# calclavia/tal-asrd

Measured on AMD Instinct MI355X. Metric: audio frames/sec (16 kHz, 10 ms hop) end-to-end log-mel -> TDS encoder -> diarization head, higher is better.
Workload: dtype f32 (dense layers: 3 x f16 MFMA hi/lo split, f32 accumulate); 1 GPU; 1 x 3600 s 16 kHz clip per GPU, each a whole-episode B=1 call (BASELINE.json configs[2]; SDModel path of tal/baseline/reconcile.py:76-85: log-mel -> TDS 80-800-1120-1440 -> 128-d feat + argmax over 6008 speakers); weights=synthetic deterministic, audio_resident_in_hbm=True

## Files before the change

include/tal_asrd.h:

```cpp
#ifndef TAL_ASRD_H
#define TAL_ASRD_H

#include <stddef.h>
#include <stdint.h>

#ifdef __cplusplus
extern "C" {
#endif

#define TAL_OK 0
#define TAL_EINVAL (-1)
#define TAL_ENOMEM (-2)
#define TAL_EHIP (-3)

#define TAL_MAX_STAGES 4
#define TAL_MAX_DEPTH 8

int tal_version(void);
const char* tal_last_error(void);

int tal_set_option(const char* name, int value);
int tal_get_option(const char* name, int* value);
const char* tal_option_name(int index);

int64_t tal_logmel_num_frames(int64_t L);
size_t tal_logmel_plan_bytes(void);
int tal_logmel_plan_init(const float* window, const float* fb, void* plan, void* stream);
size_t tal_logmel_workspace_bytes(int B, int64_t L);
int tal_logmel_fwd(const void* plan, const float* audio, int B, int64_t L, float eps,
                   int subtract_mean, float* out, float* mean_out, double* sum_out,
                   void* workspace, size_t workspace_bytes, void* stream);
int tal_logmel_f16_fwd(const void* plan, const void* audio_f16, int B, int64_t L, float eps,
                       int subtract_mean, float* out, float* mean_out, double* sum_out,
                       void* workspace, size_t workspace_bytes, void* stream);
int tal_subtract_scalar(float* x, int64_t n, const float* mean, void* stream);

int64_t tal_logmel_frames(int64_t L, int hop);
size_t tal_logmel_general_plan_bytes(int n_fft, int n_mels);
int tal_logmel_general_plan_init(const float* window, int n_fft, int hop, const float* fb, int n_mels, void* plan, void* stream);
size_t tal_logmel_general_workspace_bytes(int n_fft, int hop, int B, int64_t L);
int tal_logmel_general_fwd(const void* plan, int n_fft, int hop, int n_mels, const void* audio, int audio_is_f16, int B, int64_t L,
                           float eps, int subtract_mean, float* out, float* mean_out, double* sum_out, void* workspace,
                           size_t workspace_bytes, void* stream);

#define TAL_RESAMPLE_F32 0
#define TAL_RESAMPLE_F16 1
#define TAL_RESAMPLE_I16 2
int64_t tal_resample_num_samples(int64_t n_in, int orig, int new_rate);
size_t tal_resample_plan_bytes(int orig, int new_rate, int width);
int tal_resample_plan_build_host(int orig, int new_rate, int width, float* w, int32_t* first, int* taps);
int tal_resample_plan_init(void* plan, int orig, int new_rate, int width, void* stream);
int tal_resample_fwd(const void* plan, int orig, int new_rate, int width, const void* x, int x_dtype, int B, int64_t L_in,
                     int64_t x_pitch, const int64_t* lengths, float* y, int64_t y_pitch, void* stream);

int tal_linear_fwd(const float* x, const float* w, const float* b, const float* res, float alpha,
                   int mode, int64_t M, int N, int K, float* y, void* stream);
size_t tal_linear_workspace_bytes(int64_t M, int N, int K);
int tal_linear_ws_fwd(const float* x, const float* w, const float* b, const float* res, float alpha,
                      int mode, int64_t M, int N, int K, float* y, void* workspace,
                      size_t workspace_bytes, void* stream);

int tal_split_f16x3_fwd(const float* x, void* out, int64_t rows, int K, void* stream);
int tal_linear_f16x3_fwd(const void* x_split, const void* w_split, const float* b, const float* res, float alpha,
                         int mode, int64_t M, int N, int K, void* y, int out_split, void* workspace,
                         size_t workspace_bytes, void* stream);
int tal_linear_f16x3_guarded_fwd(const void* x_split, const void* w_split, const float* b, const void* res, int res_split,
                                 float alpha, int mode, int64_t M, int N, int K, void* y, int out_split,
                                 int* range_flag, void* workspace, size_t workspace_bytes, void* stream);

#define TAL_GCONV_MAX_K 63
int tal_pack_gconv_weight(const float* w_ref, float* w_packed, int c_out, int c_in_per_group,
                          int ksize, int groups, void* stream);
int tal_gconv_s2_fwd(const float* x, const float* w_packed, const float* bias, int B, int64_t T_in,
                     int C_in, int C_out, int groups, float* y, void* stream);
int tal_gconv_res_fwd(const float* x, const float* w_packed, const float* bias, float alpha, int B,
                      int64_t T, int C, int groups, float* y, void* stream);
int tal_gconv_s2_k_fwd(const float* x, const float* w_packed, const float* bias, int B, int64_t T_in, int C_in, int C_out,
                       int groups, int ksize, float* y, void* stream);
int tal_gconv_res_k_fwd(const float* x, const float* w_packed, const float* bias, float alpha, int B, int64_t T, int C,
                        int groups, int ksize, float* y, void* stream);

size_t tal_gconv_f16x3_weight_bytes(int C_in, int C_out, int groups, int stride);
int tal_pack_gconv_f16x3_weight(const float* w_ref, void* w_frag, int C_in, int C_out, int groups, int stride,
                                void* stream);
int tal_gconv_res_f16x3_fwd(const float* x, const void* w_frag, const float* bias, float alpha, int B,
                            int64_t T, int C, int groups, float* y, void* y_split, void* stream);
int tal_gconv_s2_f16x3_fwd(const float* x, const void* w_frag, const float* bias, int B, int64_t T_in,
                           int C_in, int C_out, int groups, float* y, void* stream);
int tal_gconv_res_split_fwd(const void* x_split, const void* w_frag, const float* bias, float alpha, int B,
                            int64_t T, int C, int groups, void* y_split, void* stream);
int tal_gconv_s2_split_fwd(const void* x, int x_is_split, const void* w_frag, const float* bias, int B,
                           int64_t T_in, int C_in, int C_out, int groups, void* y_split, void* stream);

typedef struct tal_tds_block_w {
    const float* conv_w;
    const float* conv_b;
    const float* fc0_w;
    const float* fc0_b;
    const float* fc3_w;
    const float* fc3_b;
    float resweight;
    int32_t _pad;
    const void* fc0_w_split;
    const void* fc3_w_split;
    const void* conv_w_frag;
} tal_tds_block_w;

typedef struct tal_tds_desc {
    int32_t n_stages;
    int32_t groups;
    int32_t channels[TAL_MAX_STAGES + 1];
    int32_t depths[TAL_MAX_STAGES];
    const float* down_w[TAL_MAX_STAGES];
    const float* down_b[TAL_MAX_STAGES];
    tal_tds_block_w blocks[TAL_MAX_STAGES][TAL_MAX_DEPTH];
    const void* down_w_frag[TAL_MAX_STAGES];
    int32_t flags;
    int32_t ksize;
} tal_tds_desc;
#define TAL_TDS_EXACT_F32 1
#define TAL_TDS_OUT_SPLIT 2

int64_t tal_tds_out_len(const tal_tds_desc* d, int64_t T);
size_t tal_tds_workspace_bytes(const tal_tds_desc* d, int B, int64_t T);
size_t tal_tds_status_offset(const tal_tds_desc* d, int B, int64_t T);
int tal_tds_out_split(const tal_tds_desc* d, int B, int64_t T);
int tal_tds_fwd(const tal_tds_desc* d, const float* x, int B, int64_t T, float* y,
                void* workspace, size_t workspace_bytes, void* stream);
int tal_tds_premean_ok(const tal_tds_desc* d, const float* x);
int tal_tds_premean_fwd(const tal_tds_desc* d, const float* x, const float* x_mean, int B, int64_t T, float* y,
                        void* workspace, size_t workspace_bytes, void* stream);

int tal_tds_halo(const tal_tds_desc* d, int64_t* left, int64_t* right, int64_t* stride);
size_t tal_tds_tiled_workspace_bytes(const tal_tds_desc* d, int64_t T, int64_t out_tile);
size_t tal_tds_tiled_status_offset(const tal_tds_desc* d, int64_t T, int64_t out_tile);
int tal_tds_tiled_fwd(const tal_tds_desc* d, const float* x, int64_t T, float* y, int64_t out_tile,
                      void* workspace, size_t workspace_bytes, void* stream);

size_t tal_sd_head_workspace_bytes(int64_t M, int S);
int tal_sd_head_fwd(const float* x, int64_t M, int C, const float* w_embed, const float* b_embed, int E,
                    const float* w_logit, const float* b_logit, int S, float* feat, float* logits,
                    int32_t* ids, void* workspace, size_t workspace_bytes, void* stream);
int tal_sd_head_split_fwd(const void* x_split, int64_t M, int C, const void* w_embed_split, const float* b_embed, int E,
                          const float* w_logit, const float* b_logit, int S, float* feat, float* logits,
                          int32_t* ids, void* workspace, size_t workspace_bytes, void* stream);
int tal_argmax_rows(const float* x, int64_t M, int N, int32_t* ids, void* stream);

#define TAL_TOPK_MAX 16
size_t tal_spk_topk_workspace_bytes(int64_t M, int S, int E, int k);
int tal_spk_topk_fwd(const float* feat, int64_t M, int E, const float* w_logit, const float* b_logit, int S, int k,
                     int32_t* ids, float* logp, float* lse, void* workspace, size_t workspace_bytes, void* stream);
int tal_topk_lse_rows(const float* x, int64_t M, int N, int k, int32_t* ids, float* logp, float* lse, void* stream);

size_t tal_xent_rows_workspace_bytes(int64_t M, int N, int E);
int tal_xent_rows_fwd(const float* feat, int64_t M, int64_t ldf, int E, const float* w, const float* bias, int N,
                      const int64_t* target, float* nll, float* lse, int32_t* top1, void* workspace, size_t workspace_bytes,
                      void* stream);
int tal_xent_lse_rows(const float* x, int64_t M, int N, const int64_t* target, float* nll, float* lse, int32_t* top1, void* stream);

size_t tal_soft_embed_workspace_bytes(int64_t M, int N, int E, int D);
int tal_soft_embed_fwd(const float* feat, int64_t M, int64_t ldf, int E, const float* w, const float* bias, int N,
                       const float* values, int D, float* out, float* lse, void* workspace, size_t workspace_bytes, void* stream);
size_t tal_soft_embed_rows_workspace_bytes(int64_t M, int N, int D);
int tal_soft_embed_rows(const float* x, int64_t M, int N, const float* values, int D, float* out, float* lse, void* workspace,
                        size_t workspace_bytes, void* stream);

int tal_embed_tokens_fwd(const int64_t* tokens, int B, int U, const float* emb, int V, int E0,
                         const float* proj, int D, const float* pe, int max_len, float* out,
                         void* stream);
int tal_add_positional_fwd(const float* x, int B, int U, int D, const float* pe, int max_len,
                           float* out, void* stream);

typedef struct tal_decoder_layer_w {
    const float* sa_in_w;
    const float* sa_in_b;
    const float* sa_out_w;
    const float* sa_out_b;
    const float* ca_in_w;
    const float* ca_in_b;
    const float* ca_out_w;
    const float* ca_out_b;
    const float* lin1_w;
    const float* lin1_b;
    const float* lin2_w;
    const float* lin2_b;
    float resweight;
    float resweight_src;
    const float* fold_sa_w;
    const float* fold_sa_b;
    const float* fold_ca_w;
    const float* fold_ca_b;
} tal_decoder_layer_w;

int64_t tal_pad4(int64_t n);
int tal_cross_kv_fwd(const tal_decoder_layer_w* w, const float* mem, int B, int S, int E,
                     float* k, float* vt, void* stream);
size_t tal_decoder_layer_workspace_bytes(int B, int U, int S, int E, int H, int FF);
int tal_decoder_layer_fwd(const tal_decoder_layer_w* w, const float* tgt, int B, int U,
                          const float* mem, int S, int E, int H, int FF, const float* tgt_mask,
                          const uint8_t* mem_kpm, const float* k_cache, const float* vt_cache,
                          float* out, float* xattn_avg, void* workspace, size_t workspace_bytes,
                          void* stream);
int tal_decoder_stack_fwd(const tal_decoder_layer_w* layers, int n_layers, const float* tgt, int B,
                          int U, const float* mem, int S, int E, int H, int FF, const float* tgt_mask,
                          const uint8_t* mem_kpm, const float* const* k_cache,
                          const float* const* vt_cache, float* out, float* xattn_avg, void* workspace,
                          size_t workspace_bytes, void* stream);
int tal_lm_head_fwd(const float* h, int64_t M, int64_t ldh, int D, const float* proj_t, int E0,
                    const float* emb, int V, float* logits, void* workspace, size_t workspace_bytes,
                    void* stream);
size_t tal_lm_xent_workspace_bytes(int64_t M, int D, int E0, int V);
int tal_lm_xent_fwd(const float* h, int64_t M, int64_t ldh, int D, const float* proj_t, int E0, const float* emb, int V,
                    const int64_t* target, float* nll, float* lse, int32_t* top1, void* workspace, size_t workspace_bytes,
                    void* stream);
size_t tal_lm_soft_embed_workspace_bytes(int64_t M, int D, int E0, int V, int col_begin);
int tal_lm_soft_embed_fwd(const float* h, int64_t M, int64_t ldh, int D, const float* proj_t, int E0, const float* emb, int V,
                          int col_begin, float* out, float* lse, void* workspace, size_t workspace_bytes, void* stream);
int tal_transpose_fwd(const float* x, int R, int Cc, float* y, void* stream);
int tal_log_softmax_rows(const float* x, int64_t M, int N, float* out, void* stream);
int tal_greedy_pick_fwd(const float* logits, int V, const float* attn_rows, int n_layers,
                        int64_t layer_stride, int S, float* out, int64_t* token_out, void* stream);
typedef struct tal_greedy_ctx {
    const tal_decoder_layer_w* layers;
    int32_t n_layers, E, H, FF, V, E0, S, max_len;
    const float* emb;
    const float* proj;
    const float* proj_t;
    const float* pe;
    const float* const* k_cache;
    const float* const* vt_cache;
    const uint8_t* mem_kpm;
    int64_t* tokens;
    void* workspace;
    size_t workspace_bytes;
    float* picked_dev;
    float* picked_host;
    uint32_t* tickets;
    float* picked_host_dev;
    uint32_t seq;
    uint32_t needs_reset;
    int64_t k_pitch;
    const float* const* kv_all;
    const uint8_t* kpm_all;
    int64_t enc_frames, kv_pitch;
    const float* pick_bias;
    uint32_t no_fold;
    uint32_t _pad2;
} tal_greedy_ctx;
size_t tal_greedy_step_workspace_bytes(int U_max, int S, int E, int H, int FF, int V, int E0, int n_layers);
int tal_greedy_step_fwd(tal_greedy_ctx* c, int64_t history_start, int64_t n_gen, int sync, void* stream);
int tal_greedy_step_poll(tal_greedy_ctx* c, int wait_ms);
int tal_greedy_group_ok(const tal_greedy_ctx* c, int64_t history_start, int64_t n_gen);
int tal_window_vt_fwd(const float* const* kv_all, int n_layers, int64_t frame0, int S, int E, int64_t kv_pitch,
                      float* const* vt, void* stream);
int tal_greedy_set_window(tal_greedy_ctx* c, int64_t frame0, void* stream);
int tal_greedy_step_multi_fwd(tal_greedy_ctx* const* ctxs, const int64_t* history_start, const int64_t* n_gen, int G,
                              void* stream);
typedef struct tal_unaligned_state {
    int64_t* gen;
    int64_t gen_cap, n;
    int64_t history_start;
    int64_t chunk_start;
    int64_t encoder_len;
    int64_t eos, it, max_iters;
    int64_t* rec_chunk_start;
    float* rec_attn;
    int32_t* rec_len;
    int64_t rec_cap, n_rec;
    int32_t rec_stride;
    int32_t chunk_size, max_positions, stall_patience, rep_n;
    int32_t skip_frames;
    int32_t shift_frames;
    float del_prct;
    double thresh_prct;
    double highest_progress;
    int32_t num_no_improve, window_time;
    int32_t flags;
    int32_t gen_pinned;
} tal_unaligned_state;
#define TAL_UNALIGNED_WINDOW_MOVED 1
#define TAL_UNALIGNED_PREFIX_REWRITTEN 2
#define TAL_UNALIGNED_DONE 4
#define TAL_UNALIGNED_GROW 8
#define TAL_UNALIGNED_ALONE 16
int tal_unaligned_consume(tal_unaligned_state* st, int64_t token, const float* attn, int S);
int tal_unaligned_group_run(tal_unaligned_state* const* st, tal_greedy_ctx* const* ctxs, const int64_t* dev_cap, int G,
                            int max_steps, void* stream);
int64_t tal_ngram_repeat_count(const int64_t* row, int64_t len, int n);
int tal_beam_topk(const float* logprobs, const float* row_score, const uint8_t* row_done, int B,
                  int cur_beam, int V, int k, float* out_val, int64_t* out_idx, void* stream);
typedef struct tal_beam_ctx {
    int32_t B, beam, L0, length, V, num_speakers;
    void* workspace;
    size_t workspace_bytes;
    uint32_t* done_host;
    uint32_t* done_host_dev;
    uint32_t* ctl;
    float* scores;
    uint8_t* done;
    int32_t* rec_step;
    float* rec_score;
    int64_t* rec_tokens;
    int64_t* tokens[2];
    float* sel_val;
    int64_t* sel_idx;
    float* part_val;
    int64_t* part_idx;
    float* spk_hist;
    int32_t* parent;
    size_t state_bytes;
    uint32_t seq;
    uint32_t _pad;
} tal_beam_ctx;
size_t tal_beam_workspace_bytes(int B, int beam, int L0, int length, int V, int num_speakers);
int tal_beam_init_fwd(tal_beam_ctx* c, const int64_t* generated, void* stream);
int tal_beam_select_fwd(tal_beam_ctx* c, int step, int cur_beam, const float* logits, const float* bias, int nl, void* stream);
int tal_beam_advance_fwd(tal_beam_ctx* c, int step, int cur_beam, int64_t terminate_token, const float* spk_logits, void* stream);
int tal_beam_gather_spk_fwd(const tal_beam_ctx* c, const int32_t* pairs, int n, float* out, void* stream);

int tal_attn_pool_fwd(const float* attn, const int64_t* chunk_start, const float* feat, int64_t T,
                      int E, int N, int S, int half_mode, float* out, void* stream);
int tal_attn_vote_fwd(const float* attn, const int64_t* chunk_start, const int32_t* ids, int64_t T,
                      int N, int S, int32_t* out_id, float* out_weight, void* stream);
int tal_attn_vote_groups_fwd(const float* attn, const int64_t* chunk_start, const int32_t* ids, int64_t T,
                             int S, const int64_t* group_offsets, int G, int num_ids, int half_mode,
                             int32_t* out_id, double* out_weight, void* stream);
int tal_majority_vote_fwd(const int32_t* ids, int64_t T, const int64_t* ranges, int G, int num_ids,
                          int32_t* out_id, double* out_count, void* stream);

size_t tal_gru_cell_workspace_bytes(int B, int H);
int tal_gru_cell_fwd(const float* x, const float* h, int B, int In, int H, const float* w_ih,
                     const float* w_hh, const float* b_ih, const float* b_hh, float* h_out,
                     void* workspace, size_t workspace_bytes, void* stream);

#define TAL_EDIT_TILE_ROWS 64
#ifndef TAL_EDIT_TILE_COLS
#define TAL_EDIT_TILE_COLS 128
#endif
#define TAL_EDIT_TAG_EQUAL 0
#define TAL_EDIT_TAG_REPLACE 1
#define TAL_EDIT_TAG_INSERT 2
#define TAL_EDIT_TAG_DELETE 3
#define TAL_EDIT_TAG_NONE 255
void tal_edit_align_tile(int* rows, int* cols);
size_t tal_edit_align_workspace_bytes(int P, const int64_t* a_off, const int64_t* b_off, int want_path);
int tal_edit_align_plan(int P, const int64_t* a_off, const int64_t* b_off, int want_path, int64_t* desc,
                        size_t* workspace_bytes, int64_t* path_bytes, int* launches);
int tal_edit_align_fwd(const int64_t* desc_host, const int64_t* desc_dev, int P, const int32_t* a, const int32_t* b,
                       const int32_t* a_lab, const int32_t* b_lab, int Ka, int Kb, int64_t* stats, uint8_t* path,
                       int64_t* counts, void* workspace, size_t workspace_bytes, void* stream);

int tal_prof_enable(int on);
int tal_prof_reset(void);
int tal_prof_collect(int cls, double* total_ms, int64_t* launches, double* total_work);

#ifdef __cplusplus
}
#endif
#endif
```

tal_asrd_amd/_native.py:

```python
import ctypes as C
import os

_HERE = os.path.dirname(os.path.abspath(__file__))
LIB_PATH = os.environ.get("TAL_ASRD_LIB", os.path.join(_HERE, "libtal_asrd_hip.so"))

TAL_MAX_STAGES = 4
TAL_MAX_DEPTH = 8
TAL_TDS_EXACT_F32 = 1
TAL_TDS_OUT_SPLIT = 2
TAL_GCONV_MAX_K = 63
TAL_GROUP_MAX = 16
TAL_TOPK_MAX = 16

c_float_p = C.c_void_p


class TdsBlockW(C.Structure):
    _fields_ = [("conv_w", C.c_void_p), ("conv_b", C.c_void_p), ("fc0_w", C.c_void_p), ("fc0_b", C.c_void_p),
                ("fc3_w", C.c_void_p), ("fc3_b", C.c_void_p), ("resweight", C.c_float), ("_pad", C.c_int32),
                ("fc0_w_split", C.c_void_p), ("fc3_w_split", C.c_void_p), ("conv_w_frag", C.c_void_p)]


class TdsDesc(C.Structure):
    _fields_ = [("n_stages", C.c_int32), ("groups", C.c_int32),
                ("channels", C.c_int32 * (TAL_MAX_STAGES + 1)), ("depths", C.c_int32 * TAL_MAX_STAGES),
                ("down_w", C.c_void_p * TAL_MAX_STAGES), ("down_b", C.c_void_p * TAL_MAX_STAGES),
                ("blocks", (TdsBlockW * TAL_MAX_DEPTH) * TAL_MAX_STAGES),
                ("down_w_frag", C.c_void_p * TAL_MAX_STAGES), ("flags", C.c_int32), ("ksize", C.c_int32)]


class DecoderLayerW(C.Structure):
    _fields_ = [(n, C.c_void_p) for n in ("sa_in_w", "sa_in_b", "sa_out_w", "sa_out_b", "ca_in_w", "ca_in_b",
                                          "ca_out_w", "ca_out_b", "lin1_w", "lin1_b", "lin2_w", "lin2_b")] + \
               [("resweight", C.c_float), ("resweight_src", C.c_float)] + \
               [(n, C.c_void_p) for n in ("fold_sa_w", "fold_sa_b", "fold_ca_w", "fold_ca_b")]


class GreedyCtx(C.Structure):
    _fields_ = [("layers", C.c_void_p), ("n_layers", C.c_int32), ("E", C.c_int32), ("H", C.c_int32), ("FF", C.c_int32),
                ("V", C.c_int32), ("E0", C.c_int32), ("S", C.c_int32), ("max_len", C.c_int32),
                ("emb", C.c_void_p), ("proj", C.c_void_p), ("proj_t", C.c_void_p), ("pe", C.c_void_p),
                ("k_cache", C.c_void_p), ("vt_cache", C.c_void_p), ("mem_kpm", C.c_void_p), ("tokens", C.c_void_p),
                ("workspace", C.c_void_p), ("workspace_bytes", C.c_size_t), ("picked_dev", C.c_void_p),
                ("picked_host", C.c_void_p), ("tickets", C.c_void_p), ("picked_host_dev", C.c_void_p),
                ("seq", C.c_uint32), ("needs_reset", C.c_uint32), ("k_pitch", C.c_int64), ("kv_all", C.c_void_p), ("kpm_all", C.c_void_p),
                ("enc_frames", C.c_int64), ("kv_pitch", C.c_int64), ("pick_bias", C.c_void_p),
                ("no_fold", C.c_uint32), ("_pad2", C.c_uint32)]


class UnalignedState(C.Structure):
    _fields_ = [("gen", C.c_void_p), ("gen_cap", C.c_int64), ("n", C.c_int64), ("history_start", C.c_int64), ("chunk_start", C.c_int64),
                ("encoder_len", C.c_int64), ("eos", C.c_int64), ("it", C.c_int64), ("max_iters", C.c_int64),
                ("rec_chunk_start", C.c_void_p), ("rec_attn", C.c_void_p), ("rec_len", C.c_void_p), ("rec_cap", C.c_int64),
                ("n_rec", C.c_int64), ("rec_stride", C.c_int32), ("chunk_size", C.c_int32), ("max_positions", C.c_int32),
                ("stall_patience", C.c_int32), ("rep_n", C.c_int32), ("skip_frames", C.c_int32), ("shift_frames", C.c_int32),
                ("del_prct", C.c_float), ("thresh_prct", C.c_double), ("highest_progress", C.c_double),
                ("num_no_improve", C.c_int32), ("window_time", C.c_int32), ("flags", C.c_int32), ("gen_pinned", C.c_int32)]


class BeamCtx(C.Structure):
    _fields_ = [(n, C.c_int32) for n in ("B", "beam", "L0", "length", "V", "num_speakers")] + \
               [("workspace", C.c_void_p), ("workspace_bytes", C.c_size_t), ("done_host", C.c_void_p), ("done_host_dev", C.c_void_p)] + \
               [(n, C.c_void_p) for n in ("ctl", "scores", "done", "rec_step", "rec_score", "rec_tokens")] + \
               [("tokens", C.c_void_p * 2)] + \
               [(n, C.c_void_p) for n in ("sel_val", "sel_idx", "part_val", "part_idx", "spk_hist", "parent")] + \
               [("state_bytes", C.c_size_t), ("seq", C.c_uint32), ("_pad", C.c_uint32)]


UNALIGNED_WINDOW_MOVED, UNALIGNED_PREFIX_REWRITTEN, UNALIGNED_DONE, UNALIGNED_GROW, UNALIGNED_ALONE = 1, 2, 4, 8, 16

_i, _i64, _sz, _f, _p = C.c_int, C.c_int64, C.c_size_t, C.c_float, C.c_void_p
SIGNATURES = {
    "tal_version": (_i, []),
    "tal_last_error": (C.c_char_p, []),
    "tal_set_option": (_i, [C.c_char_p, _i]),
    "tal_get_option": (_i, [C.c_char_p, C.POINTER(C.c_int)]),
    "tal_option_name": (C.c_char_p, [_i]),
    "tal_logmel_num_frames": (_i64, [_i64]),
    "tal_logmel_plan_bytes": (_sz, []),
    "tal_logmel_plan_init": (_i, [_p, _p, _p, _p]),
    "tal_logmel_workspace_bytes": (_sz, [_i, _i64]),
    "tal_logmel_fwd": (_i, [_p, _p, _i, _i64, _f, _i, _p, _p, _p, _p, _sz, _p]),
    "tal_logmel_f16_fwd": (_i, [_p, _p, _i, _i64, _f, _i, _p, _p, _p, _p, _sz, _p]),
    "tal_subtract_scalar": (_i, [_p, _i64, _p, _p]),
    "tal_logmel_frames": (_i64, [_i64, _i]),
    "tal_logmel_general_plan_bytes": (_sz, [_i, _i]),
    "tal_logmel_general_plan_init": (_i, [_p, _i, _i, _p, _i, _p, _p]),
    "tal_logmel_general_workspace_bytes": (_sz, [_i, _i, _i, _i64]),
    "tal_logmel_general_fwd": (_i, [_p, _i, _i, _i, _p, _i, _i, _i64, _f, _i, _p, _p, _p, _p, _sz, _p]),
    "tal_resample_num_samples": (_i64, [_i64, _i, _i]),
    "tal_resample_plan_bytes": (_sz, [_i, _i, _i]),
    "tal_resample_plan_build_host": (_i, [_i, _i, _i, _p, _p, C.POINTER(C.c_int)]),
    "tal_resample_plan_init": (_i, [_p, _i, _i, _i, _p]),
    "tal_resample_fwd": (_i, [_p, _i, _i, _i, _p, _i, _i, _i64, _i64, _p, _p, _i64, _p]),
    "tal_linear_fwd": (_i, [_p, _p, _p, _p, _f, _i, _i64, _i, _i, _p, _p]),
    "tal_linear_workspace_bytes": (_sz, [_i64, _i, _i]),
    "tal_split_f16x3_fwd": (_i, [_p, _p, _i64, _i, _p]),
    "tal_linear_f16x3_fwd": (_i, [_p, _p, _p, _p, _f, _i, _i64, _i, _i, _p, _i, _p, _sz, _p]),
    "tal_linear_ws_fwd": (_i, [_p, _p, _p, _p, _f, _i, _i64, _i, _i, _p, _p, _sz, _p]),
    "tal_linear_f16x3_guarded_fwd": (_i, [_p, _p, _p, _p, _i, _f, _i, _i64, _i, _i, _p, _i, _p, _p, _sz, _p]),
    "tal_pack_gconv_weight": (_i, [_p, _p, _i, _i, _i, _i, _p]),
    "tal_gconv_s2_fwd": (_i, [_p, _p, _p, _i, _i64, _i, _i, _i, _p, _p]),
    "tal_gconv_res_fwd": (_i, [_p, _p, _p, _f, _i, _i64, _i, _i, _p, _p]),
    "tal_gconv_s2_k_fwd": (_i, [_p, _p, _p, _i, _i64, _i, _i, _i, _i, _p, _p]),
    "tal_gconv_res_k_fwd": (_i, [_p, _p, _p, _f, _i, _i64, _i, _i, _i, _p, _p]),
    "tal_gconv_f16x3_weight_bytes": (C.c_size_t, [_i, _i, _i, _i]),
    "tal_pack_gconv_f16x3_weight": (_i, [_p, _p, _i, _i, _i, _i, _p]),
    "tal_gconv_s2_f16x3_fwd": (_i, [_p, _p, _p, _i, _i64, _i, _i, _i, _p, _p]),
    "tal_gconv_res_f16x3_fwd": (_i, [_p, _p, _p, _f, _i, _i64, _i, _i, _p, _p, _p]),
    "tal_gconv_res_split_fwd": (_i, [_p, _p, _p, _f, _i, _i64, _i, _i, _p, _p]),
    "tal_gconv_s2_split_fwd": (_i, [_p, _i, _p, _p, _i, _i64, _i, _i, _i, _p, _p]),
    "tal_tds_out_len": (_i64, [C.POINTER(TdsDesc), _i64]),
    "tal_tds_workspace_bytes": (_sz, [C.POINTER(TdsDesc), _i, _i64]),
    "tal_tds_status_offset": (_sz, [C.POINTER(TdsDesc), _i, _i64]),
    "tal_tds_fwd": (_i, [C.POINTER(TdsDesc), _p, _i, _i64, _p, _p, _sz, _p]),
    "tal_tds_out_split": (_i, [C.POINTER(TdsDesc), _i, _i64]),
    "tal_tds_premean_ok": (_i, [C.POINTER(TdsDesc), _p]),
    "tal_tds_premean_fwd": (_i, [C.POINTER(TdsDesc), _p, _p, _i, _i64, _p, _p, _sz, _p]),
    "tal_tds_halo": (_i, [C.POINTER(TdsDesc), C.POINTER(C.c_int64), C.POINTER(C.c_int64), C.POINTER(C.c_int64)]),
    "tal_tds_tiled_workspace_bytes": (_sz, [C.POINTER(TdsDesc), _i64, _i64]),
    "tal_tds_tiled_status_offset": (_sz, [C.POINTER(TdsDesc), _i64, _i64]),
    "tal_tds_tiled_fwd": (_i, [C.POINTER(TdsDesc), _p, _i64, _p, _i64, _p, _sz, _p]),
    "tal_sd_head_workspace_bytes": (_sz, [_i64, _i]),
    "tal_sd_head_fwd": (_i, [_p, _i64, _i, _p, _p, _i, _p, _p, _i, _p, _p, _p, _p, _sz, _p]),
    "tal_sd_head_split_fwd": (_i, [_p, _i64, _i, _p, _p, _i, _p, _p, _i, _p, _p, _p, _p, _sz, _p]),
    "tal_argmax_rows": (_i, [_p, _i64, _i, _p, _p]),
    "tal_spk_topk_workspace_bytes": (_sz, [_i64, _i, _i, _i]),
    "tal_spk_topk_fwd": (_i, [_p, _i64, _i, _p, _p, _i, _i, _p, _p, _p, _p, _sz, _p]),
    "tal_topk_lse_rows": (_i, [_p, _i64, _i, _i, _p, _p, _p, _p]),
    "tal_xent_rows_workspace_bytes": (_sz, [_i64, _i, _i]),
    "tal_xent_rows_fwd": (_i, [_p, _i64, _i64, _i, _p, _p, _i, _p, _p, _p, _p, _p, _sz, _p]),
    "tal_xent_lse_rows": (_i, [_p, _i64, _i, _p, _p, _p, _p, _p]),
    "tal_soft_embed_workspace_bytes": (_sz, [_i64, _i, _i, _i]),
    "tal_soft_embed_fwd": (_i, [_p, _i64, _i64, _i, _p, _p, _i, _p, _i, _p, _p, _p, _sz, _p]),
    "tal_soft_embed_rows_workspace_bytes": (_sz, [_i64, _i, _i]),
    "tal_soft_embed_rows": (_i, [_p, _i64, _i, _p, _i, _p, _p, _p, _sz, _p]),
    "tal_embed_tokens_fwd": (_i, [_p, _i, _i, _p, _i, _i, _p, _i, _p, _i, _p, _p]),
    "tal_add_positional_fwd": (_i, [_p, _i, _i, _i, _p, _i, _p, _p]),
    "tal_pad4": (_i64, [_i64]),
    "tal_cross_kv_fwd": (_i, [C.POINTER(DecoderLayerW), _p, _i, _i, _i, _p, _p, _p]),
    "tal_decoder_layer_workspace_bytes": (_sz, [_i, _i, _i, _i, _i, _i]),
    "tal_decoder_layer_fwd": (_i, [C.POINTER(DecoderLayerW), _p, _i, _i, _p, _i, _i, _i, _i, _p, _p, _p, _p, _p, _p,
                                   _p, _sz, _p]),
    "tal_decoder_stack_fwd": (_i, [_p, _i, _p, _i, _i, _p, _i, _i, _i, _i, _p, _p, _p, _p, _p, _p, _p, _sz, _p]),
    "tal_lm_head_fwd": (_i, [_p, _i64, _i64, _i, _p, _i, _p, _i, _p, _p, _sz, _p]),
    "tal_lm_xent_workspace_bytes": (_sz, [_i64, _i, _i, _i]),
    "tal_lm_xent_fwd": (_i, [_p, _i64, _i64, _i, _p, _i, _p, _i, _p, _p, _p, _p, _p, _sz, _p]),
    "tal_lm_soft_embed_workspace_bytes": (_sz, [_i64, _i, _i, _i, _i]),
    "tal_lm_soft_embed_fwd": (_i, [_p, _i64, _i64, _i, _p, _i, _p, _i, _i, _p, _p, _p, _sz, _p]),
    "tal_transpose_fwd": (_i, [_p, _i, _i, _p, _p]),
    "tal_greedy_step_workspace_bytes": (_sz, [_i, _i, _i, _i, _i, _i, _i, _i]),
    "tal_greedy_step_fwd": (_i, [C.POINTER(GreedyCtx), _i64, _i64, _i, _p]),
    "tal_greedy_step_poll": (_i, [C.POINTER(GreedyCtx), _i]),
    "tal_greedy_group_ok": (_i, [C.POINTER(GreedyCtx), _i64, _i64]),
    "tal_window_vt_fwd": (_i, [_p, _i, _i64, _i, _i, _i64, _p, _p]),
    "tal_greedy_set_window": (_i, [C.POINTER(GreedyCtx), _i64, _p]),
    "tal_greedy_step_multi_fwd": (_i, [C.POINTER(C.POINTER(GreedyCtx)), C.POINTER(C.c_int64), C.POINTER(C.c_int64), _i, _p]),
    "tal_unaligned_consume": (_i, [C.POINTER(UnalignedState), _i64, _p, _i]),
    "tal_unaligned_group_run": (_i, [C.POINTER(C.POINTER(UnalignedState)), C.POINTER(C.POINTER(GreedyCtx)), C.POINTER(C.c_int64), _i, _i, _p]),
    "tal_ngram_repeat_count": (_i64, [_p, _i64, _i]),
    "tal_greedy_pick_fwd": (_i, [_p, _i, _p, _i, _i64, _i, _p, _p, _p]),
    "tal_log_softmax_rows": (_i, [_p, _i64, _i, _p, _p]),
    "tal_beam_topk": (_i, [_p, _p, _p, _i, _i, _i, _i, _p, _p, _p]),
    "tal_beam_workspace_bytes": (_sz, [_i, _i, _i, _i, _i, _i]),
    "tal_beam_init_fwd": (_i, [C.POINTER(BeamCtx), _p, _p]),
    "tal_beam_select_fwd": (_i, [C.POINTER(BeamCtx), _i, _i, _p, _p, _i, _p]),
    "tal_beam_advance_fwd": (_i, [C.POINTER(BeamCtx), _i, _i, _i64, _p, _p]),
    "tal_beam_gather_spk_fwd": (_i, [C.POINTER(BeamCtx), _p, _i, _p, _p]),
    "tal_attn_pool_fwd": (_i, [_p, _p, _p, _i64, _i, _i, _i, _i, _p, _p]),
    "tal_attn_vote_groups_fwd": (_i, [_p, _p, _p, _i64, _i, _p, _i, _i, _i, _p, _p, _p]),
    "tal_majority_vote_fwd": (_i, [_p, _i64, _p, _i, _i, _p, _p, _p]),
    "tal_attn_vote_fwd": (_i, [_p, _p, _p, _i64, _i, _i, _p, _p, _p]),
    "tal_gru_cell_workspace_bytes": (_sz, [_i, _i]),
    "tal_gru_cell_fwd": (_i, [_p, _p, _i, _i, _i, _p, _p, _p, _p, _p, _p, _sz, _p]),
    "tal_edit_align_tile": (None, [C.POINTER(C.c_int), C.POINTER(C.c_int)]),
    "tal_edit_align_workspace_bytes": (_sz, [_i, _p, _p, _i]),
    "tal_edit_align_plan": (_i, [_i, _p, _p, _i, _p, C.POINTER(C.c_size_t), C.POINTER(C.c_int64), C.POINTER(C.c_int)]),
    "tal_edit_align_fwd": (_i, [_p, _p, _i, _p, _p, _p, _p, _i, _i, _p, _p, _p, _p, _sz, _p]),
    "tal_prof_enable": (_i, [_i]),
    "tal_prof_reset": (_i, []),
    "tal_prof_collect": (_i, [_i, C.POINTER(C.c_double), C.POINTER(C.c_int64), C.POINTER(C.c_double)]),
}

_lib = None


class NativeError(RuntimeError):
    pass


def lib():
    global _lib
    if _lib is None:
        if not os.path.exists(LIB_PATH):
            raise NativeError(
                "tal_asrd_amd: %s is missing -- run `python -c 'import __graft_entry__ as g; g.build()'` "
                "(hipcc --offload-arch=gfx950).  There is no CPU/PyTorch fallback for the hot path." % LIB_PATH)
        l = C.CDLL(LIB_PATH)
        for name, (res, args) in SIGNATURES.items():
            fn = getattr(l, name)
            fn.restype = res
            fn.argtypes = args
        pending = []
        for item in filter(None, (x.strip() for x in os.environ.get("TAL_OPTIONS", "").split(","))):
            name, _, val = item.partition("=")
            name = name.strip()
            try:
                value = int(val) if val.strip() else 1
            except ValueError:
                raise NativeError("TAL_OPTIONS: %r is not name=integer" % item) from None
            probe = C.c_int()
            if l.tal_get_option(name.encode(), C.byref(probe)) != 0:
                raise NativeError("TAL_OPTIONS: unknown option %r" % name)
            pending.append((name, value))
        for name, value in pending:
            if l.tal_set_option(name.encode(), value) != 0:
                raise NativeError("TAL_OPTIONS: tal_set_option(%s, %d) failed: %s" % (name, value, l.tal_last_error().decode()))
        _lib = l
    return _lib


def set_option(name, value=1):
    check(lib().tal_set_option(name.encode(), int(value)), "tal_set_option(%s)" % name)


def get_option(name):
    v = C.c_int()
    check(lib().tal_get_option(name.encode(), C.byref(v)), "tal_get_option(%s)" % name)
    return v.value


def check(rc, what=""):
    if rc != 0:
        msg = lib().tal_last_error()
        raise NativeError("%s failed (rc=%d): %s" % (what or "tal call", rc, msg.decode() if msg else ""))


def ptr(t):
    return None if t is None else C.c_void_p(t.data_ptr())


def stream_handle():
    import torch
    return C.c_void_p(torch.cuda.current_stream().cuda_stream)


def require_cuda(t, what):
    if not t.is_cuda:
        raise NativeError("%s: the hot path only runs on the GPU (HIP kernels); got a %s tensor and there is "
                          "deliberately no CPU fallback" % (what, t.device))
```

tal_asrd_amd/csrc/api.hip:

```cpp
#include <string.h>

#include <atomic>

#include "common.h"

namespace tal {

static thread_local char g_err[512] = "";

void set_error(const char* fmt, ...) {
    va_list ap;
    va_start(ap, fmt);
    vsnprintf(g_err, sizeof(g_err), fmt, ap);
    va_end(ap);
}

static const char* const g_opt_names[OPT_COUNT] = {
    "tds_exact_f32", "tds_fp32_activations", "gconv_fuse_split", "gconv_c1_generic", "head_no_astationary", "gemm_global_loads",
    "gemm_no_splitk4", "gemm_no_glds", "gemm_no_splitk_tail", "gemm_no_w64", "logmel_no_fold", "decode_no_small", "decode_small_rows", "gemm_no_row_split", "gemm_no_n96", "gemm_s64_below", "gconv_short_below", "gconv_no_shift18", "gconv_grid_xyz", "gemm_w64_stagger", "gemm_s64_order", "decode_wide_gemm", "gemm_s64_rows", "decode_persist", "decode_persist_wgs", "logmel_mfma", "gru_unfused", "decode_no_fold", "gconv_c1_fuse", "decode_fold_rows", "gconv_long_tt", "logmel_general", "gconv_general", "head_topk_form", "head_topk_grid", "xent_form", "xent_grid", "soft_embed_form", "soft_embed_grid"};
static std::atomic<int> g_opt[OPT_COUNT] = {{0}, {0}, {0}, {0}, {0}, {0}, {0}, {0}, {0}, {0}, {0}, {0}, {256}, {0}, {0}, {2}, {4}, {0}, {0}, {0}, {0}, {0}, {0}, {0}, {32}, {0}, {0}, {0}, {0}, {64}, {0}, {0}, {0}, {0}, {0}, {0}, {0}, {0}, {0}};
int opt(Option o) { return g_opt[o].load(std::memory_order_relaxed); }

int device_cus() {
    static std::atomic<int> table[64];
    int dev = 0;
    if (hipGetDevice(&dev) != hipSuccess || dev < 0 || dev >= 64) dev = 0;
    int cus = table[dev].load(std::memory_order_relaxed);
    if (!cus) {
        hipDeviceProp_t p;
        if (hipGetDeviceProperties(&p, dev) == hipSuccess) cus = p.multiProcessorCount;
        if (cus <= 0) cus = 256;
        table[dev].store(cus, std::memory_order_relaxed);
    }
    return cus;
}

static const int PROF_MAX = 8192;
static std::atomic<bool> g_prof_on{false};
static std::atomic<int> g_prof_n{0};
static hipEvent_t g_prof_ev[PROF_MAX][2];
static std::atomic<int> g_prof_have[PROF_MAX];
static int g_prof_cls[PROF_MAX];
static double g_prof_work[PROF_MAX];

ProfScope::ProfScope(int cls, double work, hipStream_t stream) : slot(-1), s(stream) {
    if (!g_prof_on.load(std::memory_order_relaxed)) return;
    const int mine = g_prof_n.fetch_add(1, std::memory_order_relaxed);
    if (mine >= PROF_MAX) return;
    g_prof_cls[mine] = -1;
    if (!g_prof_have[mine].load(std::memory_order_acquire)) {
        if (hipEventCreate(&g_prof_ev[mine][0]) != hipSuccess || hipEventCreate(&g_prof_ev[mine][1]) != hipSuccess)
            return;
        g_prof_have[mine].store(1, std::memory_order_release);
    }
    slot = mine;
    g_prof_cls[slot] = cls;
    g_prof_work[slot] = work;
    (void)hipEventRecord(g_prof_ev[slot][0], s);
}
ProfScope::~ProfScope() {
    if (slot >= 0) (void)hipEventRecord(g_prof_ev[slot][1], s);
}

__global__ __launch_bounds__(256) void argmax_rows_kernel(const float* __restrict__ x, int64_t M, int N,
                                                         int32_t* __restrict__ ids) {
    const int lane = threadIdx.x & 63;
    const int64_t row = (int64_t)blockIdx.x * 4 + (threadIdx.x >> 6);
    if (row >= M) return;
    const float* xr = x + row * N;
    float best = -INFINITY;
    int bi = 0x7fffffff;
    for (int i = lane; i < N; i += 64) {
        const float v = xr[i];
        if (v > best || (v == best && i < bi)) {
            best = v;
            bi = i;
        }
    }
#pragma unroll
    for (int off = 32; off > 0; off >>= 1) {
        const float ov = __shfl_xor(best, off, 64);
        const int oi = __shfl_xor(bi, off, 64);
        if (ov > best || (ov == best && oi < bi)) {
            best = ov;
            bi = oi;
        }
    }
    if (lane == 0) ids[row] = bi == 0x7fffffff ? 0 : bi;
}

__global__ __launch_bounds__(256) void argmax_partials_kernel(const float* __restrict__ pv,
                                                             const int32_t* __restrict__ pi, int64_t M, int P, int ld,
                                                             int32_t* __restrict__ ids) {
    const int lane = threadIdx.x & 63;
    const int64_t row = (int64_t)blockIdx.x * 4 + (threadIdx.x >> 6);
    if (row >= M) return;
    float best = -INFINITY;
    int bi = 0x7fffffff;
    for (int p = lane; p < P; p += 64) {
        const float v = pv[row * ld + p];
        const int idx = pi[row * ld + p];
        if (v > best || (v == best && idx < bi)) {
            best = v;
            bi = idx;
        }
    }
#pragma unroll
    for (int off = 32; off > 0; off >>= 1) {
        const float ov = __shfl_xor(best, off, 64);
        const int oi = __shfl_xor(bi, off, 64);
        if (ov > best || (ov == best && oi < bi)) {
            best = ov;
            bi = oi;
        }
    }
    if (lane == 0) ids[row] = bi == 0x7fffffff ? 0 : bi;
}

__global__ __launch_bounds__(256) void argmax_row_block_kernel(const float* __restrict__ x, int N,
                                                              int32_t* __restrict__ ids) {
    __shared__ float bv[4];
    __shared__ int bix[4];
    const float* xr = x + (int64_t)blockIdx.x * N;
    const int lane = threadIdx.x & 63, w = threadIdx.x >> 6;
    float best = -INFINITY;
    int bi = 0x7fffffff;
    for (int i = threadIdx.x; i < N; i += 256) {
        const float v = xr[i];
        if (v > best || (v == best && i < bi)) {
            best = v;
            bi = i;
        }
    }
#pragma unroll
    for (int off = 32; off > 0; off >>= 1) {
        const float ov = __shfl_xor(best, off, 64);
        const int oi = __shfl_xor(bi, off, 64);
        if (ov > best || (ov == best && oi < bi)) {
            best = ov;
            bi = oi;
        }
    }
    if (lane == 0) {
        bv[w] = best;
        bix[w] = bi;
    }
    __syncthreads();
    if (threadIdx.x == 0) {
        for (int q = 1; q < 4; ++q)
            if (bv[q] > best || (bv[q] == best && bix[q] < bi)) {
                best = bv[q];
                bi = bix[q];
            }
        ids[blockIdx.x] = bi == 0x7fffffff ? 0 : bi;
    }
}

int launch_argmax_rows(const float* x, int64_t M, int N, int32_t* ids, hipStream_t s) {
    TAL_CHECK_ARG(x && ids && N > 0 && M >= 0, "tal_argmax_rows: bad argument");
    if (M == 0) return TAL_OK;
    ProfScope prof(PROF_OTHER, (double)M * N * 4.0, s);
    if (M <= 512 && N >= 2048)
        hipLaunchKernelGGL(argmax_row_block_kernel, dim3((unsigned)M), dim3(256), 0, s, x, N, ids);
    else
        hipLaunchKernelGGL(argmax_rows_kernel, dim3((unsigned)cdiv(M, 4)), dim3(256), 0, s, x, M, N, ids);
    TAL_CHECK_LAUNCH("tal_argmax_rows");
    return TAL_OK;
}

static int64_t conv_out_len(int64_t t, int k) { return t < k ? 0 : (t - k) / 2 + 1; }

}

using namespace tal;

extern "C" int tal_version(void) { return 501;  }

extern "C" int64_t tal_ngram_repeat_count(const int64_t* row, int64_t len, int n) {
    if (!row || n <= 0 || len - n <= 0) return 0;
    const int64_t starts = len - n;
    int64_t covered_until = 0, count = 0;
    for (int64_t j = 0; j < starts; ++j) {
        bool seen = false;
        for (int64_t i = 0; i < j && !seen; ++i) {
            if (row[i] != row[j]) continue;
            bool eq = true;
            for (int k = 1; k < n && eq; ++k) eq = row[i + k] == row[j + k];
            seen = eq;
        }
        if (seen) {
            const int64_t lo = j > covered_until ? j : covered_until;
            if (j + n > lo) count += j + n - lo;
            covered_until = j + n;
        }
    }
    return count;
}

extern "C" const char* tal_last_error(void) { return g_err; }

static int find_option(const char* name) {
    if (!name) return -1;
    for (int i = 0; i < OPT_COUNT; ++i)
        if (strcmp(name, g_opt_names[i]) == 0) return i;
    return -1;
}

extern "C" int tal_set_option(const char* name, int value) {
    const int i = find_option(name);
    TAL_CHECK_ARG(i >= 0, "tal_set_option: unknown option '%s'", name ? name : "(null)");
    TAL_CHECK_ARG(i != OPT_DECODE_SMALL_ROWS || value >= 0, "tal_set_option: decode_small_rows must be >= 0");
    TAL_CHECK_ARG(i != OPT_HEAD_TOPK_FORM || (value >= 0 && value <= 2), "tal_set_option: head_topk_form is 0 (auto), 1 (generic) or 2 (fused)");
    TAL_CHECK_ARG(i != OPT_HEAD_TOPK_GRID || value >= 0, "tal_set_option: head_topk_grid must be >= 0");
    TAL_CHECK_ARG(i != OPT_XENT_FORM || (value >= 0 && value <= 2), "tal_set_option: xent_form is 0 (auto), 1 (generic) or 2 (fused)");
    TAL_CHECK_ARG(i != OPT_XENT_GRID || value >= 0, "tal_set_option: xent_grid must be >= 0");
    TAL_CHECK_ARG(i != OPT_SOFT_EMBED_FORM || (value >= 0 && value <= 2), "tal_set_option: soft_embed_form is 0 (auto), 1 (generic) or 2 (fused)");
    TAL_CHECK_ARG(i != OPT_SOFT_EMBED_GRID || value >= 0, "tal_set_option: soft_embed_grid must be >= 0");
    g_opt[i].store(value, std::memory_order_relaxed);
    return TAL_OK;
}

extern "C" int tal_get_option(const char* name, int* value) {
    const int i = find_option(name);
    TAL_CHECK_ARG(i >= 0 && value, "tal_get_option: unknown option '%s'", name ? name : "(null)");
    *value = g_opt[i].load(std::memory_order_relaxed);
    return TAL_OK;
}

extern "C" const char* tal_option_name(int index) { return index >= 0 && index < OPT_COUNT ? g_opt_names[index] : nullptr; }

extern "C" int tal_prof_enable(int on) {
    g_prof_on = on != 0;
    return TAL_OK;
}

extern "C" int tal_prof_reset(void) {
    g_prof_n = 0;
    return TAL_OK;
}

extern "C" int tal_prof_collect(int cls, double* total_ms, int64_t* launches, double* total_work) {
    TAL_CHECK_ARG(cls >= 0 && cls < PROF_NCLASS && total_ms && launches && total_work, "tal_prof_collect: bad argument");
    double ms = 0.0, work = 0.0;
    int64_t n = 0;
    const int n_used = g_prof_n.load() < PROF_MAX ? g_prof_n.load() : PROF_MAX;
    for (int i = 0; i < n_used; ++i) {
        if (g_prof_cls[i] != cls) continue;
        if (hipEventSynchronize(g_prof_ev[i][1]) != hipSuccess) {
            set_error("tal_prof_collect: event sync failed");
            return TAL_EHIP;
        }
        float t = 0.f;
        if (hipEventElapsedTime(&t, g_prof_ev[i][0], g_prof_ev[i][1]) != hipSuccess) {
            set_error("tal_prof_collect: cannot read the event pair of launch %d", i);
            return TAL_EHIP;
        }
        ms += t;
        work += g_prof_work[i];
        ++n;
    }
    *total_ms = ms;
    *launches = n;
    *total_work = work;
    return TAL_OK;
}

extern "C" int tal_linear_fwd(const float* x, const float* w, const float* b, const float* res, float alpha, int mode,
                              int64_t M, int N, int K, float* y, void* stream) {
    return launch_linear(x, w, b, res, alpha, mode, M, N, K, y, (hipStream_t)stream);
}

extern "C" size_t tal_linear_workspace_bytes(int64_t M, int N, int K) {
    return gemm_wants_scratch(M, N, K) ? gemm_splitk_ws_bytes() : 0;
}

extern "C" int tal_linear_ws_fwd(const float* x, const float* w, const float* b, const float* res, float alpha, int mode,
                                 int64_t M, int N, int K, float* y, void* workspace, size_t workspace_bytes,
                                 void* stream) {
    TAL_CHECK_ARG(workspace || workspace_bytes == 0, "tal_linear_ws_fwd: null workspace with %zu bytes", workspace_bytes);
    return launch_linear_ws(x, w, b, res, alpha, mode, M, N, K, y, (float*)workspace, workspace_bytes, (hipStream_t)stream);
}

extern "C" int tal_gconv_s2_fwd(const float* x, const float* w_packed, const float* bias, int B, int64_t T_in,
                                int C_in, int C_out, int groups, float* y, void* stream) {
    return launch_gconv_s2(x, w_packed, bias, B, T_in, C_in, C_out, groups, y, (hipStream_t)stream);
}

extern "C" int tal_gconv_res_fwd(const float* x, const float* w_packed, const float* bias, float alpha, int B,
                                 int64_t T, int C, int groups, float* y, void* stream) {
    return launch_gconv_res(x, w_packed, bias, alpha, B, T, C, groups, y, (hipStream_t)stream);
}

extern "C" size_t tal_gconv_f16x3_weight_bytes(int C_in, int C_out, int groups, int stride) {
    return gconv_f16x3_weight_bytes(C_in, C_out, groups, stride);
}

extern "C" int tal_pack_gconv_f16x3_weight(const float* w_ref, void* w_frag, int C_in, int C_out, int groups, int stride, void* stream) {
    return launch_pack_gconv_f16x3(w_ref, w_frag, C_in, C_out, groups, stride, (hipStream_t)stream);
}

extern "C" int tal_gconv_res_f16x3_fwd(const float* x, const void* w_frag, const float* bias, float alpha, int B,
                                       int64_t T, int C, int groups, float* y, void* y_split, void* stream) {
    return launch_gconv_res_f16x3(x, w_frag, bias, alpha, B, T, C, groups, y, y_split, (hipStream_t)stream);
}

extern "C" int tal_gconv_s2_f16x3_fwd(const float* x, const void* w_frag, const float* bias, int B, int64_t T_in, int C_in,
                                      int C_out, int groups, float* y, void* stream) {
    return launch_gconv_s2_f16x3(x, w_frag, bias, B, T_in, C_in, C_out, groups, y, (hipStream_t)stream);
}

extern "C" int tal_gconv_res_split_fwd(const void* x_split, const void* w_frag, const float* bias, float alpha, int B, int64_t T,
                                       int C, int groups, void* y_split, void* stream) {
    TAL_CHECK_ARG(C % 32 == 0, "tal_gconv_res_split_fwd: the split form needs C %% 32 == 0 (C=%d)", C);
    return launch_gconv_res_f16x3(reinterpret_cast<const float*>(x_split), w_frag, bias, alpha, B, T, C, groups, nullptr, y_split,
                                  (hipStream_t)stream, nullptr, true);
}

extern "C" int tal_gconv_s2_split_fwd(const void* x, int x_is_split, const void* w_frag, const float* bias, int B, int64_t T_in,
                                      int C_in, int C_out, int groups, void* y_split, void* stream) {
    TAL_CHECK_ARG(C_out % 32 == 0 && (!x_is_split || C_in % 32 == 0), "tal_gconv_s2_split_fwd: the split form needs channels %% 32 == 0");
    return launch_gconv_s2_f16x3(reinterpret_cast<const float*>(x), w_frag, bias, B, T_in, C_in, C_out, groups, nullptr, (hipStream_t)stream,
                                 nullptr, x_is_split != 0, y_split);
}

extern "C" int tal_argmax_rows(const float* x, int64_t M, int N, int32_t* ids, void* stream) {
    return launch_argmax_rows(x, M, N, ids, (hipStream_t)stream);
}

static int tds_ksize(const tal_tds_desc* d) { return d->ksize == 0 ? 21 : d->ksize; }
static bool tds_general(const tal_tds_desc* d) { return tds_ksize(d) != 21 || opt(OPT_GCONV_GENERAL) != 0; }

static int check_desc(const tal_tds_desc* d) {
    TAL_CHECK_ARG(d, "tal_tds: null descriptor");
    TAL_CHECK_ARG(d->n_stages >= 1 && d->n_stages <= TAL_MAX_STAGES, "tal_tds: n_stages=%d", d->n_stages);
    TAL_CHECK_ARG(d->groups > 0, "tal_tds: groups=%d", d->groups);
    TAL_CHECK_ARG(d->ksize >= 0 && d->ksize <= TAL_GCONV_MAX_K, "tal_tds: ksize=%d outside 1..%d (0: 21)", d->ksize, TAL_GCONV_MAX_K);
    for (int i = 0; i <= d->n_stages; ++i)
        TAL_CHECK_ARG(d->channels[i] > 0 && d->channels[i] % d->groups == 0, "tal_tds: channels[%d]=%d", i, d->channels[i]);
    for (int i = 0; i < d->n_stages; ++i) {
        TAL_CHECK_ARG(d->depths[i] >= 0 && d->depths[i] <= TAL_MAX_DEPTH, "tal_tds: depths[%d]=%d", i, d->depths[i]);
        TAL_CHECK_ARG(d->channels[i + 1] % 4 == 0 || d->depths[i] == 0, "tal_tds: channels[%d]=%d must be a multiple of 4 for the pointwise layers", i + 1, d->channels[i + 1]);
        TAL_CHECK_ARG(tds_ksize(d) % 2 == 1 || d->depths[i] == 0, "tal_tds: ksize=%d is even but depths[%d]=%d: a TDSBlock needs an odd kernel size",
                      d->ksize, i, d->depths[i]);
        if (tds_ksize(d) != 21) {
            TAL_CHECK_ARG(!d->down_w_frag[i], "tal_tds: down_w_frag[%d] set with ksize=%d (fragments exist for k = 21 only)", i, d->ksize);
            for (int j = 0; j < d->depths[i]; ++j)
                TAL_CHECK_ARG(!d->blocks[i][j].conv_w_frag, "tal_tds: blocks[%d][%d].conv_w_frag set with ksize=%d (fragments exist for k = 21 only)",
                              i, j, d->ksize);
        }
    }
    return TAL_OK;
}

extern "C" int64_t tal_tds_out_len(const tal_tds_desc* d, int64_t T) {
    if (!d) return -1;
    const int k = tds_ksize(d);
    for (int i = 0; i < d->n_stages; ++i) T = conv_out_len(T, k);
    return T;
}

static size_t tds_buf_floats(const tal_tds_desc* d, int B, int64_t T) {
    size_t mx = 0;
    for (int i = 0; i < d->n_stages; ++i) {
        T = conv_out_len(T, tds_ksize(d));
        const size_t n = (size_t)B * (size_t)T * (size_t)d->channels[i + 1];
        if (n > mx) mx = n;
    }
    return (mx + 63) & ~(size_t)63;
}

__global__ void clear_status_kernel(int* __restrict__ status, int y_form = 0) { status[threadIdx.x] = threadIdx.x == 1 ? y_form : 0; }

extern "C" size_t tal_tds_status_offset(const tal_tds_desc* d, int B, int64_t T) {
    if (!d || B <= 0 || T <= 0) return 0;
    return 4 * tds_buf_floats(d, B, T) * sizeof(float) + gemm_splitk_ws_bytes();
}

extern "C" size_t tal_tds_workspace_bytes(const tal_tds_desc* d, int B, int64_t T) {
    if (!d || B <= 0 || T <= 0) return 0;
    return tal_tds_status_offset(d, B, T) + 64;
}

static bool tds_s2_mfma_ok(const tal_tds_desc* d, int B, int i, int64_t Tin, int ks, bool general, bool force_f32) {
    return !force_f32 && !general && d->down_w_frag[i] && (int64_t)B * conv_out_len(Tin, ks) > 64 &&
           gconv_has_mfma(d->channels[i], d->channels[i + 1], d->groups, 2) && gconv_f16x3_fits(Tin, d->channels[i]);
}
static bool tds_blocks_split_ok(const tal_tds_desc* d, int B, int i, int64_t Tin, int ks, bool general, bool fp32_only) {
    if (fp32_only || general || d->depths[i] == 0) return false;
    const int c = d->channels[i + 1];
    const int64_t To = conv_out_len(Tin, ks);
    if ((int64_t)B * To <= 128 || c % 160 != 0 || c % 32 != 0 || !gconv_f16x3_fits(To, c) || !gconv_has_mfma(c, c, d->groups, 1)) return false;
    for (int j = 0; j < d->depths[i]; ++j)
        if (!d->blocks[i][j].fc0_w_split || !d->blocks[i][j].fc3_w_split || !d->blocks[i][j].conv_w_frag) return false;
    return true;
}

static int tds_launch_resize(const tal_tds_desc* d, int i, const float* cur, bool cur_split, const float* x_mean, int B, int64_t Tc, int ks, bool general,
                             bool s2_mfma, bool allsplit, float* a, hipStream_t s, int* range_flag) {
    const int cin = d->channels[i], c = d->channels[i + 1];
    if (general) return launch_gconv_s2_k(cur, d->down_w[i], d->down_b[i], B, Tc, cin, c, d->groups, ks, a, s);
    if (s2_mfma)
        return launch_gconv_s2_f16x3(cur, d->down_w_frag[i], d->down_b[i], B, Tc, cin, c, d->groups, allsplit ? nullptr : a, s, range_flag, cur_split,
                                     allsplit ? a : nullptr);
    return launch_gconv_s2(cur, d->down_w[i], d->down_b[i], B, Tc, cin, c, d->groups, allsplit ? nullptr : a, s, allsplit ? a : nullptr,
                           allsplit ? range_flag : nullptr, i == 0 ? x_mean : nullptr);
}

static int tds_launch_dense(const tal_tds_block_w& bw, bool f16x3, bool allsplit, const float* xin, const float* x1, float* h, float* outp, bool out_split,
                            int64_t M, int c, float* skws, hipStream_t s, int* range_flag) {
    const size_t skb = gemm_splitk_ws_bytes();
    int rc;
    if (f16x3) {
        rc = launch_linear_f16x3(xin, bw.fc0_w_split, bw.fc0_b, nullptr, 0.f, 1, M, c, c, h, 1, skws, skb, s, range_flag);
        if (rc) return rc;
        return launch_linear_f16x3(h, bw.fc3_w_split, bw.fc3_b, x1, bw.resweight, 2, M, c, c, outp, out_split ? 1 : 0, skws, skb, s,
                                   allsplit ? range_flag : nullptr, allsplit ? 1 : 0);
    }
    rc = launch_linear_ws(xin, bw.fc0_w, bw.fc0_b, nullptr, 0.f, 1, M, c, c, h, skws, skb, s);
    if (rc) return rc;
    return launch_linear_ws(h, bw.fc3_w, bw.fc3_b, x1, bw.resweight, 2, M, c, c, outp, skws, skb, s);
}

static int tds_walk(const tal_tds_desc* d, const float* x, const float* x_mean, int B, int64_t T, float* y, void* workspace, hipStream_t s,
                    bool launch, bool* y_split) {
    const size_t nf = tds_buf_floats(d, B, T);
    float* buf[4];
    for (int q = 0; q < 4; ++q) buf[q] = reinterpret_cast<float*>(workspace) + q * nf;
    float* skws = reinterpret_cast<float*>(workspace) + 4 * nf;
    int* range_flag = reinterpret_cast<int*>(reinterpret_cast<char*>(workspace) + tal_tds_status_offset(d, B, T));
    const bool force_f32 = opt(OPT_TDS_EXACT_F32) != 0 || (d->flags & TAL_TDS_EXACT_F32) != 0;
    const bool fp32_only = force_f32 || opt(OPT_TDS_FP32_ACTIVATIONS) != 0;
    const int ks = tds_ksize(d);
    const bool general = tds_general(d);
    const float* cur = x;
    bool cur_split = false;
    int ia = -1;
    int64_t Tc = T;
    bool s2_mfma = tds_s2_mfma_ok(d, B, 0, T, ks, general, force_f32), blocks_split = tds_blocks_split_ok(d, B, 0, T, ks, general, fp32_only);
    for (int i = 0; i < d->n_stages; ++i) {
        const int cin = d->channels[i], c = d->channels[i + 1];
        const int64_t To = conv_out_len(Tc, ks);
        const bool last_stage = i == d->n_stages - 1;
        const int64_t M = (int64_t)B * To;
        const bool allsplit = blocks_split && (s2_mfma ? (!cur_split || cin % 32 == 0) : (!cur_split && gconv_s2_can_split(cin, c, d->groups, cur)));
        const bool next_s2_mfma = !last_stage && tds_s2_mfma_ok(d, B, i + 1, To, ks, general, force_f32);
        const bool next_blocks_split = !last_stage && tds_blocks_split_ok(d, B, i + 1, To, ks, general, fp32_only);
        const bool next_split = c % 32 == 0 && next_s2_mfma && next_blocks_split;
        const int io = (ia + 1) % 4;
        float* a = (last_stage && d->depths[i] == 0) ? y : buf[io];
        const bool c1_fused = allsplit && i == 0 && !s2_mfma && opt(OPT_GCONV_C1_FUSE) && !opt(OPT_GCONV_C1_GENERIC) &&
                              gconv_c1_res_fusable(cin, c, d->groups, cur);
        if (launch && !c1_fused) {
            TAL_CHECK_ARG(allsplit || !cur_split, "tal_tds_fwd: internal: stage %d would read a split activation through an fp32 kernel", i);
            const int rc = tds_launch_resize(d, i, cur, cur_split, x_mean, B, Tc, ks, general, s2_mfma, allsplit, a, s, range_flag);
            if (rc) return rc;
        }
        ia = io;
        cur_split = allsplit;
        for (int j = 0; j < d->depths[i]; ++j) {
            const tal_tds_block_w& bw = d->blocks[i][j];
            const bool last_block = j == d->depths[i] - 1;
            float* outp = (last_stage && last_block) ? y : buf[ia];
            const bool out_split = allsplit && (!last_block || next_split || (last_stage && (d->flags & TAL_TDS_OUT_SPLIT) != 0));
            if (launch) {
                TAL_CHECK_ARG(bw.conv_w && bw.conv_b && bw.fc0_w && bw.fc0_b && bw.fc3_w && bw.fc3_b, "tal_tds_fwd: null weight in block %d.%d", i, j);
                float* x1 = buf[(ia + 1) % 4];
                float* h = buf[(ia + 2) % 4];
                float* x1s = buf[(ia + 3) % 4];
                int rc;
                if (allsplit) {
                    if (c1_fused && j == 0)
                        rc = launch_gconv_c1_res_f16x3(cur, d->down_w[i], d->down_b[i], x_mean, bw.conv_w_frag, bw.conv_b, bw.resweight, B, Tc, d->groups, x1, s, range_flag);
                    else
                        rc = launch_gconv_res_f16x3(a, bw.conv_w_frag, bw.conv_b, bw.resweight, B, To, c, d->groups, nullptr, x1, s, range_flag, true);
                    if (!rc) rc = tds_launch_dense(bw, true, true, x1, x1, h, outp, out_split, M, c, skws, s, range_flag);
                } else {
                    const bool f16x3 = !force_f32 && bw.fc0_w_split && bw.fc3_w_split && M > 128 && c % 160 == 0;
                    const bool conv_mfma = !force_f32 && !general && M > 64 && bw.conv_w_frag && gconv_has_mfma(c, c, d->groups, 1) && gconv_f16x3_fits(To, c);
                    const bool fuse_split = opt(OPT_GCONV_FUSE_SPLIT) != 0;
                    if (general)
                        rc = launch_gconv_res_k(a, bw.conv_w, bw.conv_b, bw.resweight, B, To, c, d->groups, ks, x1, s);
                    else if (conv_mfma)
                        rc = launch_gconv_res_f16x3(a, bw.conv_w_frag, bw.conv_b, bw.resweight, B, To, c, d->groups, x1, (fuse_split && f16x3) ? x1s : nullptr, s,
                                                    range_flag);
                    else
                        rc = launch_gconv_res(a, bw.conv_w, bw.conv_b, bw.resweight, B, To, c, d->groups, x1, s);
                    if (!rc && f16x3 && !(conv_mfma && fuse_split)) rc = launch_split_f16x3(x1, x1s, M, c, s, range_flag);
                    if (!rc) rc = tds_launch_dense(bw, f16x3, false, f16x3 ? x1s : x1, x1, h, outp, false, M, c, skws, s, range_flag);
                }
                if (rc) return rc;
            }
            a = outp;
            cur_split = out_split;
        }
        cur = a;
        Tc = To;
        s2_mfma = next_s2_mfma;
        blocks_split = next_blocks_split;
    }
    *y_split = cur_split;
    return TAL_OK;
}

static int tds_fwd_impl(const tal_tds_desc* d, const float* x, const float* x_mean, int B, int64_t T, float* y, void* workspace,
                        size_t workspace_bytes, void* stream) {
    int rc = check_desc(d);
    if (rc) return rc;
    TAL_CHECK_ARG(x && y && workspace, "tal_tds_fwd: null pointer");
    TAL_CHECK_ARG(B > 0 && tal_tds_out_len(d, T) > 0, "tal_tds_fwd: T=%lld too short for %d stride-2 k=%d stages", (long long)T, d->n_stages, tds_ksize(d));
    if (workspace_bytes < tal_tds_workspace_bytes(d, B, T)) {
        set_error("tal_tds_fwd: workspace %zu < %zu bytes", workspace_bytes, tal_tds_workspace_bytes(d, B, T));
        return TAL_ENOMEM;
    }
    hipStream_t s = (hipStream_t)stream;
    bool y_split_out = false;
    if (d->flags & TAL_TDS_OUT_SPLIT) tds_walk(d, x, x_mean, B, T, y, workspace, s, false, &y_split_out);
    int* status = reinterpret_cast<int*>(reinterpret_cast<char*>(workspace) + tal_tds_status_offset(d, B, T));
    clear_status_kernel<<<1, 16, 0, s>>>(status, y_split_out ? 1 : 0);
    if (hipGetLastError() != hipSuccess) {
        set_error("tal_tds_fwd: cannot clear the status word");
        return TAL_EHIP;
    }
    return tds_walk(d, x, x_mean, B, T, y, workspace, s, true, &y_split_out);
}

extern "C" int tal_tds_out_split(const tal_tds_desc* d, int B, int64_t T) {
    if (check_desc(d) || B <= 0 || tal_tds_out_len(d, T) <= 0 || !(d->flags & TAL_TDS_OUT_SPLIT)) return 0;
    float* const aligned = reinterpret_cast<float*>(static_cast<uintptr_t>(16));
    bool y_split = false;
    tds_walk(d, aligned, nullptr, B, T, aligned, aligned, nullptr, false, &y_split);
    return y_split ? 1 : 0;
}

extern "C" int tal_tds_fwd(const tal_tds_desc* d, const float* x, int B, int64_t T, float* y, void* workspace,
                           size_t workspace_bytes, void* stream) {
    return tds_fwd_impl(d, x, nullptr, B, T, y, workspace, workspace_bytes, stream);
}

extern "C" int tal_tds_premean_ok(const tal_tds_desc* d, const float* x) {
    if (check_desc(d) || d->n_stages < 1 || tds_general(d)) return 0;
    return gconv_s2_can_fold_mean(d->channels[0], d->channels[1], d->groups, x) ? 1 : 0;
}

extern "C" int tal_tds_premean_fwd(const tal_tds_desc* d, const float* x, const float* x_mean, int B, int64_t T, float* y, void* workspace,
                                   size_t workspace_bytes, void* stream) {
    int rc = check_desc(d);
    if (rc) return rc;
    TAL_CHECK_ARG(x_mean, "tal_tds_premean_fwd: null mean pointer");
    TAL_CHECK_ARG(tal_tds_premean_ok(d, x), "tal_tds_premean_fwd: the first resize conv of this stack (%d -> %d channels, %d groups) has no mean-folding "
                  "kernel: subtract the mean (tal_subtract_scalar) and call tal_tds_fwd", d->channels[0], d->channels[1], d->groups);
    return tds_fwd_impl(d, x, x_mean, B, T, y, workspace, workspace_bytes, stream);
}

extern "C" int tal_tds_halo(const tal_tds_desc* d, int64_t* left, int64_t* right, int64_t* stride) {
    int rc = check_desc(d);
    if (rc) return rc;
    const int k = tds_ksize(d);
    int64_t lo = 0, hi = 0, st = 1;
    for (int i = d->n_stages - 1; i >= 0; --i) {
        lo -= (int64_t)d->depths[i] * (k / 2);
        hi += (int64_t)d->depths[i] * (k / 2);
        lo = 2 * lo;
        hi = 2 * hi + k - 1;
        st *= 2;
    }
    if (left) *left = -lo;
    if (right) *right = hi;
    if (stride) *stride = st;
    return TAL_OK;
}

namespace {
struct TilePlan { int64_t in_start, in_stop, out_start, out_stop, skip; };
TilePlan plan_tile(int64_t T, int64_t t_out, int64_t out_tile, int64_t k, int64_t left, int64_t right, int64_t stride) {
    TilePlan p;
    p.out_start = k * out_tile;
    p.out_stop = p.out_start + out_tile < t_out ? p.out_start + out_tile : t_out;
    const int64_t a = stride * (p.out_start - (left + stride - 1) / stride);
    p.in_start = a > 0 ? a : 0;
    const int64_t b = stride * (p.out_stop - 1) + right + 1;
    p.in_stop = b < T ? b : T;
    p.skip = p.out_start - p.in_start / stride;
    return p;
}
__global__ void or_status_kernel(const int* __restrict__ tile_flag, int* __restrict__ call_flag) {
    if (threadIdx.x == 0 && *tile_flag) atomicOr(call_flag, *tile_flag);
}
size_t up256(size_t n) { return (n + 255) & ~(size_t)255; }
}

static int tiled_layout(const tal_tds_desc* d, int64_t T, int64_t out_tile, size_t* slice_out_bytes, size_t* tds_bytes, int64_t* max_slice) {
    int64_t left, right, stride;
    int rc = tal_tds_halo(d, &left, &right, &stride);
    if (rc) return rc;
    const int64_t t_out = tal_tds_out_len(d, T);
    TAL_CHECK_ARG(t_out > 0 && out_tile > 0, "tal_tds_tiled: T=%lld too short or out_tile=%lld not positive", (long long)T, (long long)out_tile);
    int64_t longest = 0;
    const int64_t n_tiles = cdiv(t_out, out_tile);
    for (int64_t k = 0; k < n_tiles; ++k) {
        const TilePlan p = plan_tile(T, t_out, out_tile, k, left, right, stride);
        if (p.in_stop - p.in_start > longest) longest = p.in_stop - p.in_start;
    }
    *max_slice = longest;
    *slice_out_bytes = up256((size_t)tal_tds_out_len(d, longest) * d->channels[d->n_stages] * sizeof(float));
    *tds_bytes = up256(tal_tds_workspace_bytes(d, 1, longest));
    return TAL_OK;
}

extern "C" size_t tal_tds_tiled_status_offset(const tal_tds_desc* d, int64_t T, int64_t out_tile) {
    size_t a, b;
    int64_t m;
    if (!d || tiled_layout(d, T, out_tile, &a, &b, &m)) return 0;
    return a + b;
}

extern "C" size_t tal_tds_tiled_workspace_bytes(const tal_tds_desc* d, int64_t T, int64_t out_tile) {
    const size_t off = tal_tds_tiled_status_offset(d, T, out_tile);
    return off ? off + 64 : 0;
}

extern "C" int tal_tds_tiled_fwd(const tal_tds_desc* d, const float* x, int64_t T, float* y, int64_t out_tile, void* workspace,
                                 size_t workspace_bytes, void* stream) {
    TAL_CHECK_ARG(x && y && workspace && d, "tal_tds_tiled_fwd: null pointer");
    tal_tds_desc fp32_out = *d;
    fp32_out.flags &= ~(uint32_t)TAL_TDS_OUT_SPLIT;
    d = &fp32_out;
    size_t so, tb;
    int64_t longest;
    int rc = tiled_layout(d, T, out_tile, &so, &tb, &longest);
    if (rc) return rc;
    if (workspace_bytes < so + tb + 64) {
        set_error("tal_tds_tiled_fwd: workspace %zu < %zu bytes", workspace_bytes, so + tb + 64);
        return TAL_ENOMEM;
    }
    hipStream_t s = (hipStream_t)stream;
    int64_t left, right, stride;
    tal_tds_halo(d, &left, &right, &stride);
    const int64_t t_out = tal_tds_out_len(d, T), n_tiles = cdiv(t_out, out_tile);
    const int c_in = d->channels[0], c_out = d->channels[d->n_stages];
    char* base = reinterpret_cast<char*>(workspace);
    float* slice_out = reinterpret_cast<float*>(base);
    void* tds_ws = base + so;
    int* call_flag = reinterpret_cast<int*>(base + so + tb);
    clear_status_kernel<<<1, 16, 0, s>>>(call_flag);
    if (hipGetLastError() != hipSuccess) {
        set_error("tal_tds_tiled_fwd: cannot clear the status word");
        return TAL_EHIP;
    }
    for (int64_t k = 0; k < n_tiles; ++k) {
        const TilePlan p = plan_tile(T, t_out, out_tile, k, left, right, stride);
        const int64_t Ts = p.in_stop - p.in_start;
        const bool direct = n_tiles == 1;
        rc = tal_tds_fwd(d, x + p.in_start * c_in, 1, Ts, direct ? y : slice_out, tds_ws, tb, stream);
        if (rc) return rc;
        const int* tile_flag = reinterpret_cast<const int*>(reinterpret_cast<char*>(tds_ws) + tal_tds_status_offset(d, 1, Ts));
        hipLaunchKernelGGL(or_status_kernel, dim3(1), dim3(64), 0, s, tile_flag, call_flag);
        TAL_CHECK_LAUNCH("tal_tds_tiled_fwd(status)");
        if (!direct && hipMemcpyAsync(y + p.out_start * c_out, slice_out + p.skip * c_out, (size_t)(p.out_stop - p.out_start) * c_out * sizeof(float),
                                      hipMemcpyDeviceToDevice, s) != hipSuccess) {
            set_error("tal_tds_tiled_fwd: copy of tile %lld failed", (long long)k);
            return TAL_EHIP;
        }
    }
    return TAL_OK;
}

extern "C" int tal_split_f16x3_fwd(const float* x, void* out, int64_t rows, int K, void* stream) {
    return launch_split_f16x3(x, out, rows, K, (hipStream_t)stream);
}

extern "C" int tal_linear_f16x3_fwd(const void* x_split, const void* w_split, const float* b, const float* res, float alpha,
                                    int mode, int64_t M, int N, int K, void* y, int out_split, void* workspace,
                                    size_t workspace_bytes, void* stream) {
    TAL_CHECK_ARG(workspace || workspace_bytes == 0, "tal_linear_f16x3_fwd: null workspace with %zu bytes", workspace_bytes);
    return launch_linear_f16x3(x_split, w_split, b, res, alpha, mode, M, N, K, y, out_split, (float*)workspace, workspace_bytes,
                               (hipStream_t)stream);
}

extern "C" int tal_linear_f16x3_guarded_fwd(const void* x_split, const void* w_split, const float* b, const void* res, int res_split,
                                            float alpha, int mode, int64_t M, int N, int K, void* y, int out_split,
                                            int* range_flag, void* workspace, size_t workspace_bytes, void* stream) {
    TAL_CHECK_ARG(workspace || workspace_bytes == 0, "tal_linear_f16x3_guarded_fwd: null workspace with %zu bytes", workspace_bytes);
    return launch_linear_f16x3(x_split, w_split, b, reinterpret_cast<const float*>(res), alpha, mode, M, N, K, y, out_split,
                               (float*)workspace, workspace_bytes, (hipStream_t)stream, range_flag, res_split);
}

static int sd_head_part_ld(int S) {
    const int64_t a = cdiv(S, 32), b = 4 * cdiv(S, 128);
    return (int)(a > b ? a : b);
}

static size_t sd_head_partials_bytes(int64_t M, int S) { return (size_t)(M > 0 ? M : 1) * (size_t)sd_head_part_ld(S) * 8; }

extern "C" size_t tal_sd_head_workspace_bytes(int64_t M, int S) {
    const size_t partials = ((sd_head_partials_bytes(M, S) + 255) & ~(size_t)255) + (size_t)S * 128 * 4 + 64;
    const int64_t tiles = cdiv(M > 0 ? M : 1, 128);
    const size_t slices = tiles <= 128 ? (size_t)tiles * 8 * 128 * 160 * sizeof(float) : 0;
    return partials > slices ? partials : slices;
}

static int sd_head_after_feat(int64_t M, int E, const float* w_logit, const float* b_logit, int S, float* feat, float* logits,
                              int32_t* ids, void* workspace, size_t workspace_bytes, hipStream_t s);

extern "C" int tal_sd_head_fwd(const float* x, int64_t M, int C, const float* w_embed, const float* b_embed, int E,
                               const float* w_logit, const float* b_logit, int S, float* feat, float* logits,
                               int32_t* ids, void* workspace, size_t workspace_bytes, void* stream) {
    TAL_CHECK_ARG(x && w_embed && w_logit && feat, "tal_sd_head_fwd: null pointer");
    TAL_CHECK_ARG(M >= 0 && C > 0 && E > 0 && S > 0, "tal_sd_head_fwd: bad shape");
    hipStream_t s = (hipStream_t)stream;
    int rc = workspace && workspace_bytes >= tal_sd_head_workspace_bytes(M, S) && M > 512
                 ? launch_linear_ws(x, w_embed, b_embed, nullptr, 0.f, 0, M, E, C, feat, reinterpret_cast<float*>(workspace), workspace_bytes, s)
                 : launch_linear(x, w_embed, b_embed, nullptr, 0.f, 0, M, E, C, feat, s);
    if (rc) return rc;
    return sd_head_after_feat(M, E, w_logit, b_logit, S, feat, logits, ids, workspace, workspace_bytes, s);
}

extern "C" int tal_sd_head_split_fwd(const void* x_split, int64_t M, int C, const void* w_embed_split, const float* b_embed, int E,
                                     const float* w_logit, const float* b_logit, int S, float* feat, float* logits,
                                     int32_t* ids, void* workspace, size_t workspace_bytes, void* stream) {
    TAL_CHECK_ARG(x_split && w_embed_split && w_logit && feat, "tal_sd_head_split_fwd: null pointer");
    TAL_CHECK_ARG(M > 128 && C > 0 && C % 32 == 0 && E > 0 && S > 0, "tal_sd_head_split_fwd: needs M > 128 rows and C %% 32 == 0 (M=%lld, C=%d)", (long long)M, C);
    hipStream_t s = (hipStream_t)stream;
    const bool ws_ok = workspace && workspace_bytes >= tal_sd_head_workspace_bytes(M, S);
    int rc = launch_linear_f16x3(x_split, w_embed_split, b_embed, nullptr, 0.f, 0, M, E, C, feat, 0, ws_ok ? reinterpret_cast<float*>(workspace) : nullptr,
                                 ws_ok ? workspace_bytes : 0, s);
    if (rc) return rc;
    return sd_head_after_feat(M, E, w_logit, b_logit, S, feat, logits, ids, workspace, workspace_bytes, s);
}

static int sd_head_after_feat(int64_t M, int E, const float* w_logit, const float* b_logit, int S, float* feat, float* logits,
                              int32_t* ids, void* workspace, size_t workspace_bytes, hipStream_t s) {
    int rc;
    if (!logits && !ids) return TAL_OK;
    if (logits) {
        rc = launch_linear(feat, w_logit, b_logit, nullptr, 0.f, 0, M, S, E, logits, s);
        if (rc) return rc;
        return ids ? launch_argmax_rows(logits, M, S, ids, s) : TAL_OK;
    }
    TAL_CHECK_ARG(workspace, "tal_sd_head_fwd: ids without logits needs a workspace");
    if (workspace_bytes < sd_head_partials_bytes(M, S)) {
        set_error("tal_sd_head_fwd: workspace %zu < %zu bytes", workspace_bytes, sd_head_partials_bytes(M, S));
        return TAL_ENOMEM;
    }
    if (M == 0) return TAL_OK;
    if (b_logit && head_argmax_applicable(M, S, E)) {
        const int P = head_argmax_partials(M, S);
        float* pv = reinterpret_cast<float*>(workspace);
        int32_t* pi = reinterpret_cast<int32_t*>(pv + (size_t)M * P);
        const bool head_f32 = opt(OPT_TDS_EXACT_F32) != 0;
        void* wsplit = nullptr;
        int* guard = nullptr;
        const size_t used = ((size_t)M * P * 8 + 255) & ~(size_t)255;
        if (!head_f32 && E % 32 == 0 && (reinterpret_cast<uintptr_t>(w_logit) & 15) == 0 && used + (size_t)S * E * 4 + 64 <= workspace_bytes) {
            wsplit = reinterpret_cast<char*>(workspace) + used;
            guard = reinterpret_cast<int*>(reinterpret_cast<char*>(workspace) + used + (size_t)S * E * 4);
            clear_status_kernel<<<1, 16, 0, s>>>(guard);
            TAL_CHECK_LAUNCH("tal_sd_head_fwd(status)");
            rc = launch_split_f16x3(w_logit, wsplit, S, E, s, guard);
            if (rc) return rc;
        }
        rc = launch_head_argmax(feat, w_logit, wsplit, b_logit, M, S, pv, pi, s, guard);
        if (rc) return rc;
        ProfScope prof(PROF_OTHER, (double)M * P * 8.0, s);
        hipLaunchKernelGGL(argmax_partials_kernel, dim3((unsigned)cdiv(M, 4)), dim3(256), 0, s, pv, pi, M, P, P, ids);
        TAL_CHECK_LAUNCH("tal_sd_head_fwd(argmax)");
        return TAL_OK;
    }
    const int ld = sd_head_part_ld(S);
    GemmArgs g = {};
    g.A = feat; g.W = w_logit; g.bias = b_logit;
    g.M = M; g.N = S; g.K = E;
    g.lda = E; g.ldw = E; g.ldy = S; g.nb2 = 1;
    g.part_val = reinterpret_cast<float*>(workspace);
    g.part_idx = reinterpret_cast<int32_t*>(g.part_val + (size_t)M * ld);
    g.part_ld = ld;
    rc = launch_gemm(g, 4, 1, s);
    if (rc) return rc;
    {
        ProfScope prof(PROF_OTHER, (double)M * ld * 8.0, s);
        hipLaunchKernelGGL(argmax_partials_kernel, dim3((unsigned)cdiv(M, 4)), dim3(256), 0, s, g.part_val, g.part_idx, M,
                           gemm_mode4_partials(M, S), ld, ids);
    }
    TAL_CHECK_LAUNCH("tal_sd_head_fwd(argmax)");
    return TAL_OK;
}
```

tal_asrd_amd/csrc/common.h:

```cpp
#pragma once
#include <hip/hip_runtime.h>
#include <stdint.h>
#include <stdio.h>
#include <stdarg.h>
#include <stdlib.h>

#include "../../include/tal_asrd.h"
#include "gemm_plan.h"
#include "gconv_plan.h"

namespace tal {

void set_error(const char* fmt, ...);

#define TAL_CHECK_ARG(cond, ...)                 \
    do {                                         \
        if (!(cond)) {                           \
            tal::set_error(__VA_ARGS__);         \
            return TAL_EINVAL;                   \
        }                                        \
    } while (0)

#define TAL_CHECK_LAUNCH(what)                                                        \
    do {                                                                              \
        hipError_t e__ = hipGetLastError();                                           \
        if (e__ != hipSuccess) {                                                      \
            tal::set_error("%s: launch failed: %s", what, hipGetErrorString(e__));    \
            return TAL_EHIP;                                                          \
        }                                                                             \
    } while (0)

typedef float f32x4 __attribute__((ext_vector_type(4)));
typedef float f32x16 __attribute__((ext_vector_type(16)));
typedef _Float16 f16x8 __attribute__((ext_vector_type(8)));
typedef _Float16 f16x4 __attribute__((ext_vector_type(4)));

__device__ __forceinline__ void split_f16x3(float x, _Float16& hi, _Float16& lo) {
    hi = (_Float16)fminf(fmaxf(x, -65504.f), 65504.f);
    lo = (_Float16)fminf(fmaxf((x - (float)hi) * 2048.f, -65504.f), 65504.f);
}

__device__ __forceinline__ void st_agent(float* p, float v) {
    __hip_atomic_store(reinterpret_cast<unsigned*>(p), __float_as_uint(v), __ATOMIC_RELAXED, __HIP_MEMORY_SCOPE_AGENT);
}
__device__ __forceinline__ float ld_agent(const float* p) {
    return __uint_as_float(__hip_atomic_load(reinterpret_cast<const unsigned*>(p), __ATOMIC_RELAXED, __HIP_MEMORY_SCOPE_AGENT));
}
template <int N>
__device__ __forceinline__ void ld_agent_x4(const float* p, size_t stride, f32x4 (&v)[N]) {
#pragma unroll
    for (int i = 0; i < N; ++i) asm volatile("global_load_dwordx4 %0, %1, off sc1" : "=&v"(v[i]) : "v"(p + i * stride) : "memory");
    asm volatile("s_waitcnt vmcnt(0)" ::: "memory");
#pragma unroll
    for (int i = 0; i < N; ++i) asm volatile("" : "+v"(v[i]));
}
__device__ __forceinline__ unsigned take_ticket(unsigned* word) {
    asm volatile("s_waitcnt vmcnt(0)" ::: "memory");
    return __hip_atomic_fetch_add(word, 1u, __ATOMIC_RELAXED, __HIP_MEMORY_SCOPE_AGENT);
}
__device__ __forceinline__ void reset_ticket(unsigned* word) {
    __hip_atomic_store(word, 0u, __ATOMIC_RELAXED, __HIP_MEMORY_SCOPE_AGENT);
}

__device__ __forceinline__ float amax4(float a, const f32x4& v) {
    return fmaxf(fmaxf(a, fmaxf(fabsf(v.x), fabsf(v.y))), fmaxf(fabsf(v.z), fabsf(v.w)));
}
__device__ __forceinline__ void note_range(float amax, int* flag) {
    if (flag && !(amax <= 65504.f)) atomicOr(flag, 1);
}
__device__ __forceinline__ float amax_nan(float a, float v) {
    const unsigned ua = __float_as_uint(a), uv = __float_as_uint(v) & 0x7fffffffu;
    return __uint_as_float(ua > uv ? ua : uv);
}
__device__ __forceinline__ float amax4_nan(float a, const f32x4& v) {
    return amax_nan(amax_nan(a, v.x), amax_nan(amax_nan(0.f, v.y), amax_nan(amax_nan(0.f, v.z), v.w)));
}

typedef float f32x2p __attribute__((ext_vector_type(2)));
typedef _Float16 f16x2p __attribute__((ext_vector_type(2)));
__device__ __forceinline__ void split_f16x3_pair(float a, float b, f16x2p& hi, f16x2p& lo) {
    const f32x2p x = {a, b};
    hi = __builtin_convertvector(x, f16x2p);
    const f32x2p hf = __builtin_convertvector(hi, f32x2p);
    lo = __builtin_convertvector((x - hf) * 2048.f, f16x2p);
}

enum Option {
    OPT_TDS_EXACT_F32 = 0,
    OPT_TDS_FP32_ACTIVATIONS,
    OPT_GCONV_FUSE_SPLIT,
    OPT_GCONV_C1_GENERIC,
    OPT_HEAD_NO_ASTATIONARY,
    OPT_GEMM_GLOBAL_LOADS,
    OPT_GEMM_NO_SPLITK4,
    OPT_GEMM_NO_GLDS,
    OPT_GEMM_NO_SPLITK_TAIL,
    OPT_GEMM_NO_W64,
    OPT_LOGMEL_NO_FOLD,
    OPT_DECODE_NO_SMALL,
    OPT_DECODE_SMALL_ROWS,
    OPT_GEMM_NO_ROW_SPLIT,
    OPT_GEMM_NO_N96,
    OPT_GEMM_S64_BELOW,
    OPT_GCONV_SHORT_BELOW,
    OPT_GCONV_NO_SHIFT18,
    OPT_GCONV_GRID_XYZ,
    OPT_GEMM_W64_STAGGER,
    OPT_GEMM_S64_ORDER,
    OPT_DECODE_WIDE_GEMM,
    OPT_GEMM_S64_ROWS,
    OPT_DECODE_PERSIST,
    OPT_DECODE_PERSIST_WGS,
    OPT_LOGMEL_MFMA,
    OPT_GRU_UNFUSED,
    OPT_DECODE_NO_FOLD,
    OPT_GCONV_C1_FUSE,
    OPT_DECODE_FOLD_ROWS,
    OPT_GCONV_LONG_TT,
    OPT_LOGMEL_GENERAL,
    OPT_GCONV_GENERAL,
    OPT_HEAD_TOPK_FORM,
    OPT_HEAD_TOPK_GRID,
    OPT_XENT_FORM,
    OPT_XENT_GRID,
    OPT_SOFT_EMBED_FORM,
    OPT_SOFT_EMBED_GRID,
    OPT_COUNT
};
int opt(Option o);
int device_cus();

__device__ __forceinline__ unsigned xcd_logical_block(unsigned nb, unsigned bid) {
    const unsigned xcd = bid & 7u, q = nb >> 3, r = nb & 7u;
    return (xcd < r ? xcd * (q + 1) : r * (q + 1) + (xcd - r) * q) + (bid >> 3);
}

__device__ __forceinline__ int wave_id() { return __builtin_amdgcn_readfirstlane((int)(threadIdx.x >> 6)); }

enum ProfClass { PROF_GEMM = 0, PROF_GCONV_RES = 1, PROF_GCONV_S2 = 2, PROF_LOGMEL = 3, PROF_OTHER = 4, PROF_NCLASS = 5 };
struct ProfScope {
    int slot;
    hipStream_t s;
    ProfScope(int cls, double work, hipStream_t stream);
    ~ProfScope();
};

struct GemmArgs {
    const float* A;
    const float* W;
    const float* bias;
    const float* res;
    float* Y;
    int64_t M;
    int N, K;
    int64_t lda, ldw, ldy, ldres;
    int nb2;
    int64_t a_s1, a_s2, w_s1, w_s2, y_s1, y_s2, r_s1, r_s2, bias_s2;
    float alpha;
    int scale_cols;
    int tiles_n;
    unsigned tiles_n_magic;
    float* part_val;
    int32_t* part_idx;
    int part_ld;
    int tile_base, split, tail_tiles;
    float* splitk_ws;
    size_t splitk_ws_bytes;
    int f16x3, out_split;
    int res_split;
    int* range_flag;
    int stagger_ticks, stagger_blocks;
    int n_major, tiles_m;
    unsigned tiles_m_magic;
};
int launch_gemm(GemmArgs g, int mode, int nbatch, hipStream_t s);
void launch_gemm_w64(const GemmArgs& g, int mode, const GemmStep& st, hipStream_t s);
void launch_gemm_s64(const GemmArgs& g, int mode, const GemmStep& st, hipStream_t s);
int gemm_mode4_partials(int64_t M, int N);
inline int launch_linear_ld(const float* a, int64_t lda, const float* w, const float* bias, int64_t M, int N, int K, float* y, int64_t ldy,
                            hipStream_t s) {
    GemmArgs g = {};
    g.A = a; g.W = w; g.bias = bias; g.Y = y; g.M = M; g.N = N; g.K = K;
    g.lda = lda; g.ldw = K; g.ldy = ldy; g.ldres = ldy; g.nb2 = 1;
    return launch_gemm(g, 0, 1, s);
}

inline size_t lm_proj_bytes(int64_t M, int E0) { return ((size_t)M * E0 * sizeof(float) + 15) & ~(size_t)15; }
template <class Check, class Stage>
int lm_head_project(const char* who, const float* h, int64_t M, int64_t ldh, int D, const float* proj_t, int E0, void* workspace,
                    size_t workspace_bytes, hipStream_t s, Check check, Stage stage) {
    const size_t head = lm_proj_bytes(M, E0);
    if (!workspace || workspace_bytes < head) {
        set_error("%s: workspace %zu < %zu bytes", who, workspace ? workspace_bytes : (size_t)0, head);
        return TAL_ENOMEM;
    }
    float* t = reinterpret_cast<float*>(workspace);
    size_t need = 0;
    int rc = check(t, need);
    if (rc) return rc;
    if (workspace_bytes < head + need) {
        set_error("%s: workspace %zu < %zu bytes", who, workspace_bytes, head + need);
        return TAL_ENOMEM;
    }
    rc = launch_linear_ld(h, ldh, proj_t, nullptr, M, E0, D, t, E0, s);
    if (rc) return rc;
    return stage(t, reinterpret_cast<char*>(workspace) + head, workspace_bytes - head);
}

int launch_linear(const float* x, const float* w, const float* b, const float* res, float alpha, int mode,
                  int64_t M, int N, int K, float* y, hipStream_t s);
int launch_linear_ws(const float* x, const float* w, const float* b, const float* res, float alpha, int mode,
                     int64_t M, int N, int K, float* y, float* ws, size_t ws_bytes, hipStream_t s);
size_t gemm_splitk_ws_bytes();
int launch_split_f16x3(const float* x, void* out, int64_t rows, int K, hipStream_t s, int* range_flag = nullptr);
int launch_linear_f16x3(const void* xs, const void* wsplit, const float* b, const float* res, float alpha, int mode, int64_t M,
                        int N, int K, void* y, int out_split, float* ws, size_t ws_bytes, hipStream_t s, int* range_flag = nullptr,
                        int res_split = 0);
int launch_gconv_s2(const float* x, const float* wp, const float* bias, int B, int64_t T_in, int C_in, int C_out,
                    int groups, float* y, hipStream_t s, void* y_split = nullptr, int* range_flag = nullptr, const float* in_mean = nullptr);
bool gconv_s2_can_split(int C_in, int C_out, int groups, const float* x);
bool gconv_s2_can_fold_mean(int C_in, int C_out, int groups, const float* x);
int launch_gconv_res(const float* x, const float* wp, const float* bias, float alpha, int B, int64_t T, int C,
                     int groups, float* y, hipStream_t s);
int launch_gconv_s2_k(const float* x, const float* wp, const float* bias, int B, int64_t T_in, int C_in, int C_out, int groups,
                      int ks, float* y, hipStream_t s);
int launch_gconv_res_k(const float* x, const float* wp, const float* bias, float alpha, int B, int64_t T, int C, int groups, int ks,
                       float* y, hipStream_t s);
size_t gconv_f16x3_weight_bytes(int C_in, int C_out, int groups, int stride);
GconvCall gconv_call(int entry, int B, int64_t T_in, int C_in, int C_out, int groups, int ks, const void* x);
int gconv_refused(const GconvCall& c, int why);
template <auto KERN, class... Args>
int gconv_launch_planned(const GconvLaunch& p, dim3 grid, const char* what, hipStream_t s, Args... args) {
    static bool reserved = false;
    if (p.lds_reserve > 0 && !reserved) {
        if (hipFuncSetAttribute(reinterpret_cast<const void*>(KERN), hipFuncAttributeMaxDynamicSharedMemorySize, (int)p.lds_reserve) != hipSuccess) {
            set_error("%s: cannot reserve %zu bytes of LDS", what, p.lds_reserve);
            return TAL_EHIP;
        }
        reserved = true;
    }
    if (p.prof == GCP_NONE) {
        hipLaunchKernelGGL(KERN, grid, dim3(p.block), p.lds, s, args...);
    } else {
        ProfScope prof(p.prof, p.work, s);
        hipLaunchKernelGGL(KERN, grid, dim3(p.block), p.lds, s, args...);
    }
    TAL_CHECK_LAUNCH(what);
    return TAL_OK;
}
bool gconv_c1_res_fusable(int C_in, int C_out, int groups, const float* mel);
int launch_gconv_c1_res_f16x3(const float* mel, const float* w1, const float* b1, const float* in_mean, const void* w_frag, const float* bias,
                              float alpha, int B, int64_t T_mel, int groups, void* y_split, hipStream_t s, int* range_flag);
int launch_pack_gconv_f16x3(const float* w_ref, void* w_frag, int C_in, int C_out, int groups, int stride, hipStream_t s);
int launch_gconv_s2_f16x3(const float* x, const void* w_frag, const float* bias, int B, int64_t T_in, int C_in, int C_out, int groups,
                          float* y, hipStream_t s, int* range_flag = nullptr, bool x_split = false, void* y_split = nullptr);
int launch_gconv_res_f16x3(const float* x, const void* w_frag, const float* bias, float alpha, int B, int64_t T, int C, int groups,
                           float* y, void* y_split, hipStream_t s, int* range_flag = nullptr, bool x_split = false);
int launch_argmax_rows(const float* x, int64_t M, int N, int32_t* ids, hipStream_t s);
int launch_logmel_mean(const double* partial, int64_t nparts, double count, float* mean_out, double* sum_out, float* mean_ws,
                       int subtract_mean, float* x, int64_t n, hipStream_t s, const char* what);
bool head_argmax_applicable(int64_t M, int S, int E);
int head_argmax_partials(int64_t M, int S);
int launch_head_argmax(const float* feat, const float* w, const void* w_split, const float* b, int64_t M, int S, float* part_val,
                       int32_t* part_idx, hipStream_t s, int* range_flag = nullptr);

struct SkinnyArgs {
    const float* A;
    const float* W;
    const float* bias;
    const float* res;
    float* Y;
    int M, N, K;
    int64_t lda, ldw, ldy, ldres;
    float alpha;
    int scale_cols;
    float* Yt;
    int vt_begin, U;
    int64_t ldt, vt_bs;
    int ksplit;
    float* sk_part;
    unsigned* sk_tickets;
    const float* A2;
    int64_t lda2;
    int K1;
    int relu_begin;
    int k1_cols;
};

struct AttnArgs {
    const float* q;
    const float* k;
    const float* vt;
    const float* vbias;
    const float* mask;
    const uint8_t* kpm;
    float* ctx;
    float* probs;
    int64_t ldq, q_bs, ldk, k_bs, ldvt, vt_bs, ldc, c_bs;
    int U, S, H, prob_row0;
};

constexpr int TAL_GROUP_MAX = 16;
template <typename T>
struct ArgPack {
    T a[TAL_GROUP_MAX];
    int n;
};

constexpr int TAL_GREEDY_TICKETS = 256;
constexpr int PS_BAR = 252, PS_DONE = 253, PS_ERR = 254;
constexpr int TAL_PS_MAX_SESS = 8, TAL_PS_MAX_LAYERS = 6;
struct PsModel {
    tal_decoder_layer_w layer[TAL_PS_MAX_LAYERS];
    int n_layers, E, H, FF, V, K0;
    float qscale;
    const float *emb, *proj, *proj_t, *pe;
};
struct PsSession {
    const int64_t* tokens;
    int64_t* token_out;
    int U, S;
    float *h0, *h1, *qkv, *vt, *ctx, *x1, *x2, *ff, *probs, *sk_part, *pick_part, *out;
    unsigned* tickets;
    const float* k_cache[TAL_PS_MAX_LAYERS];
    const float* vt_cache[TAL_PS_MAX_LAYERS];
    const uint8_t* kpm;
    int64_t k_pitch;
    unsigned host_seq;
};
struct PsArgs {
    PsModel m;
    PsSession s[TAL_PS_MAX_SESS];
    int n, G;
};
static_assert(sizeof(PsArgs) <= 3800, "the one-launch step's arguments travel by value in the kernel argument segment");
int launch_greedy_persist(const PsArgs& a, hipStream_t s);

bool skinny_gemm_applicable(const SkinnyArgs& g);
int launch_skinny_gemm(const SkinnyArgs& g, int mode, hipStream_t s);
bool attn_small_applicable(int U, int S, int hd);
int launch_attn_small(const AttnArgs& g, int B, int hd, hipStream_t s);
size_t attn_split_scratch_floats(int B, int U, int S, int H, int hd);
int attn_split_tickets(int B, int U, int H);
int launch_attn_split(const AttnArgs& g, int B, int hd, float* scratch, unsigned* tickets, hipStream_t s);
int launch_head_average(const float* probs, float* avg, int B, int H, int U, int S, hipStream_t s);
int launch_skinny_gemm_multi(const SkinnyArgs* g, int G, int mode, hipStream_t s);
int launch_attn_small_multi(const AttnArgs* g, int G, int hd, hipStream_t s);
int launch_attn_split_multi(const AttnArgs* g, float* const* scratch, unsigned* const* tickets, int G, int hd, hipStream_t s);

}
```

tal_asrd_amd/models.py:

```python
import collections
import math

import torch
import torch.nn as nn

from . import _native as N
from . import ops
from . import tiling
from .modules import PositionalEncoding, weight_init

DEFAULT_SR = 16000
KERNEL_SIZE = 21


def _check_kernel_size(who, kernel_size, blocks):
    if isinstance(kernel_size, bool) or not isinstance(kernel_size, int) or not 1 <= kernel_size <= N.TAL_GCONV_MAX_K:
        raise N.NativeError("%s: kernel_size=%r outside 1..%d (the grouped-conv kernels' range)" % (who, kernel_size, N.TAL_GCONV_MAX_K))
    if blocks and kernel_size % 2 == 0:
        raise N.NativeError("%s: kernel_size=%d is even: the reference's TDSBlock residual add fails for it (its conv pads k // 2 "
                            "and returns T + 1 frames)" % (who, kernel_size))


def _htk_filterbank(n_freqs, n_mels, sample_rate, f_min=0.0, f_max=None):
    f_max = float(sample_rate // 2) if f_max is None else float(f_max)
    freqs = torch.linspace(0, sample_rate // 2, n_freqs)
    lo = 2595.0 * math.log10(1.0 + f_min / 700.0)
    hi = 2595.0 * math.log10(1.0 + f_max / 700.0)
    edges_mel = torch.linspace(lo, hi, n_mels + 2)
    edges_hz = 700.0 * (10.0 ** (edges_mel / 2595.0) - 1.0)
    width = edges_hz[1:] - edges_hz[:-1]
    dist = edges_hz.unsqueeze(0) - freqs.unsqueeze(1)
    falling = (-1.0 * dist[:, :-2]) / width[:-1]
    rising = dist[:, 2:] / width[1:]
    return torch.clamp(torch.min(falling, rising), min=0.0)


_EPOCH_ATTR = "_tal_param_epoch"
_hook_installed = [False]


def _note_parameter_registration(module, name, param):
    cell = module.__dict__.get(_EPOCH_ATTR)
    if cell is not None:
        cell[0] += 1


def _note_module_registration(module, name, child):
    cell = module.__dict__.get(_EPOCH_ATTR)
    if cell is not None and child is not None:
        for m in child.modules():
            m.__dict__[_EPOCH_ATTR] = cell
        cell[0] += 1


def _install_hooks():
    if not _hook_installed[0]:
        torch.nn.modules.module.register_module_parameter_registration_hook(_note_parameter_registration)
        torch.nn.modules.module.register_module_module_registration_hook(_note_module_registration)
        _hook_installed[0] = True


def _adopt(root):
    _install_hooks()
    cell = root.__dict__.get(_EPOCH_ATTR)
    if cell is None:
        cell = [0]
    for m in root.modules():
        m.__dict__[_EPOCH_ATTR] = cell
    return cell


def param_epoch(root):
    _install_hooks()
    cell = root.__dict__.get(_EPOCH_ATTR)
    if cell is None:
        cell = _adopt(root)
    return cell[0]


class _Spectrogram(nn.Module):
    def __init__(self, n_fft):
        super().__init__()
        self.register_buffer("window", torch.hann_window(n_fft))


class _MelScale(nn.Module):
    def __init__(self, n_mels, sample_rate, n_freqs):
        super().__init__()
        self.register_buffer("fb", _htk_filterbank(n_freqs, n_mels, sample_rate))


class MelSpectrogram(nn.Module):

    def __init__(self, sample_rate, n_mels, n_fft, win_length, hop_length):
        super().__init__()
        if win_length != n_fft:
            raise N.NativeError("MelSpectrogram: the HIP front-end takes win_length == n_fft (tal/asr/models.py:24-32), got %d and %d"
                                % (win_length, n_fft))
        err = ops.logmel_shape_error(n_fft, hop_length, n_mels)
        if err:
            raise N.NativeError("MelSpectrogram(sample_rate=%s): the HIP front-end limit is violated: %s" % (sample_rate, err))
        self.hop_length = hop_length
        self.spectrogram = _Spectrogram(n_fft)
        self.mel_scale = _MelScale(n_mels, sample_rate, n_fft // 2 + 1)


class LogMelSpec(nn.Module):

    def __init__(self, sr=DEFAULT_SR, n_mels=80, eps=1e-6):
        super().__init__()
        self.mel_transform = MelSpectrogram(sample_rate=sr, n_mels=n_mels, n_fft=int(25 / 1000 * sr),
                                            win_length=int(25 / 1000 * sr), hop_length=int(10 / 1000 * sr))
        self.eps = eps
        self.sample_rate = sr
        self._plan = None
        self._plan_key = None

    def plan(self):
        win, fb = self.mel_transform.spectrogram.window, self.mel_transform.mel_scale.fb
        key = (win.data_ptr(), win._version, fb.data_ptr(), fb._version)
        if self._plan is None or self._plan_key != key:
            self._plan = ops.logmel_plan(win, fb, hop=self.mel_transform.hop_length)
            self._plan_key = key
        return self._plan

    @torch.no_grad()
    def forward(self, audio: torch.Tensor):
        N.require_cuda(audio, "LogMelSpec.forward")
        return ops.logmel(self.plan(), audio, eps=self.eps, subtract_mean=True)

    def forward_unsubtracted(self, audio: torch.Tensor):
        N.require_cuda(audio, "LogMelSpec.forward_unsubtracted")
        out, mean, _ = ops.logmel(self.plan(), audio, eps=self.eps, subtract_mean=False, return_stats=True)
        return out, mean


class Resample(nn.Module):

    def __init__(self, orig_freq=DEFAULT_SR, new_freq=DEFAULT_SR):
        super().__init__()
        ops.resample_plan_bytes(orig_freq, new_freq)
        self.orig_freq, self.new_freq = int(orig_freq), int(new_freq)
        self._plans = {}

    def plan(self, device):
        if device not in self._plans:
            self._plans[device] = ops.resample_plan(self.orig_freq, self.new_freq, device)
        return self._plans[device]

    def num_samples(self, n_in):
        return ops.resample_num_samples(n_in, self.orig_freq, self.new_freq)

    @torch.no_grad()
    def forward(self, waveform: torch.Tensor, lengths=None):
        N.require_cuda(waveform, "Resample.forward")
        return ops.resample(self.plan(waveform.device), waveform, lengths=lengths)

    def extra_repr(self):
        return "orig_freq=%d, new_freq=%d" % (self.orig_freq, self.new_freq)


class _Resampled:

    def _resampler(self, sample_rate):
        own = self.logmelspec.sample_rate
        if sample_rate is None or sample_rate == own:
            return None
        cache = self.__dict__.setdefault("_resamplers", {})
        if sample_rate not in cache:
            cache[sample_rate] = Resample(sample_rate, own)
        return cache[sample_rate]

    def _resample_batch(self, x, audio_lens, sample_rate):
        rs = self._resampler(sample_rate)
        if rs is None:
            return x, audio_lens
        if audio_lens is None:
            return rs(x), None
        return rs(x, lengths=audio_lens), rs.num_samples(audio_lens)


class Linear(nn.Linear):
    def forward(self, x):
        return ops.linear(x, self.weight, self.bias)


class PointwiseConv1d(nn.Conv1d):

    def forward(self, x):
        return ops.linear(x, self.weight, self.bias)


class GroupedConv1d(nn.Conv1d):

    def __init__(self, *a, **kw):
        super().__init__(*a, **kw)
        self._packed = None
        self._packed_key = None

    def packed(self):
        key = (self.weight.data_ptr(), self.weight._version, self.weight.device)
        if self._packed is None or self._packed_key != key:
            self._packed = ops.pack_gconv_weight(self.weight.detach(), self.groups)
            self._packed_key = key
        return self._packed

    def forward(self, x):
        if self.stride[0] != 2 or self.padding[0] != 0:
            raise N.NativeError("GroupedConv1d.forward: only the stride-2 / pad-0 resize conv is exposed directly")
        return ops.gconv_s2(x, self.packed(), self.bias, self.out_channels, self.groups, ksize=self.kernel_size[0])


class TDSBlock(nn.Module):

    def __init__(self, hidden, kernel_size, groups, dropout=0.1):
        super().__init__()
        _check_kernel_size("TDSBlock", kernel_size, True)
        self.conv = nn.Sequential(
            GroupedConv1d(hidden, hidden, kernel_size=kernel_size, stride=1, groups=groups,
                          padding=kernel_size // 2),
            nn.ReLU(), nn.Dropout(dropout))
        self.fc = nn.Sequential(
            PointwiseConv1d(hidden, hidden, kernel_size=1, stride=1), nn.ReLU(), nn.Dropout(dropout),
            PointwiseConv1d(hidden, hidden, kernel_size=1, stride=1), nn.Dropout(dropout))
        self.resweight = nn.Parameter(torch.Tensor([0]))

    def forward_time_major(self, x):
        rw = float(self.resweight.detach())
        g = self.conv[0]
        x = ops.gconv_res(x, g.packed(), g.bias, rw, g.groups, ksize=g.kernel_size[0])
        h = ops.linear(x, self.fc[0].weight, self.fc[0].bias, mode=1)
        return ops.linear(h, self.fc[3].weight, self.fc[3].bias, mode=2, res=x, alpha=rw)

    def forward(self, x):
        return self.forward_time_major(x.permute(0, 2, 1).contiguous()).permute(0, 2, 1).contiguous()


class TDS(nn.Module):

    def __init__(self, input_size, sizes, depths, kernel_size=21, dropout=0.1):
        super().__init__()
        _check_kernel_size("TDS", kernel_size, any(int(d) > 0 for d in depths))
        if len(sizes) - 1 > N.TAL_MAX_STAGES or max(depths) > N.TAL_MAX_DEPTH:
            raise N.NativeError("TDS: at most %d stages of depth %d" % (N.TAL_MAX_STAGES, N.TAL_MAX_DEPTH))
        self.kernel_size = kernel_size
        self.extract_block_id = 1
        self.sizes = sizes
        self.depths = list(depths)
        self.max_item_frames = tiling.max_item_frames(list(sizes))
        self.tile_frames = 32768
        self.input_size = input_size
        self.blocks = nn.Sequential(*[
            nn.Sequential(
                GroupedConv1d(sizes[i - 1], sizes[i], kernel_size=kernel_size, stride=2, groups=input_size),
                nn.Sequential(*[TDSBlock(sizes[i], kernel_size, input_size, dropout=dropout)
                                for _ in range(depths[i - 1])]))
            for i in range(1, len(sizes))])
        self._plist = None
        self._plist_epoch = -1
        _adopt(self)
        self._descs = {}
        self._packs = {}
        self._desc_key = None

    def _apply(self, fn, *a, **kw):
        self._plist = None
        return super()._apply(fn, *a, **kw)


    def _param_key(self):
        epoch = param_epoch(self)
        if self._plist is None or self._plist_epoch != epoch:
            self._plist = list(self.parameters())
            self._plist_epoch = epoch
        return tuple((p.data_ptr(), p._version) for p in self._plist)

    def _stage_pack(self, s):
        if s in self._packs:
            return self._packs[s]
        down, chain = self.blocks[s][0], self.blocks[s][1]
        c = self.sizes[s + 1]
        def in_range(w):
            return bool(torch.isfinite(w).all()) and float(w.abs().max()) <= 65504.0
        frags = self.kernel_size == KERNEL_SIZE
        pack = {"down_w": down.packed(),
                "down_frag": ops.pack_gconv_f16x3_weight(down.weight.detach(), down.groups, stride=2)
                if frags and in_range(down.weight.detach()) else None,
                "blocks": []}
        rws = torch.stack([blk.resweight.detach().reshape(()) for blk in chain]).cpu().tolist() if len(chain) else []
        for blk, rw in zip(chain, rws):
            g = blk.conv[0]
            b = {"conv_w": g.packed(), "rw": float(rw), "fc0_split": None, "fc3_split": None, "conv_frag": None}
            if c % 160 == 0 and in_range(blk.fc[0].weight.detach()) and in_range(blk.fc[3].weight.detach()):
                b["fc0_split"] = ops.split_f16x3(blk.fc[0].weight.detach().reshape(c, c))
                b["fc3_split"] = ops.split_f16x3(blk.fc[3].weight.detach().reshape(c, c))
            if frags and in_range(g.weight.detach()):
                b["conv_frag"] = ops.pack_gconv_f16x3_weight(g.weight.detach(), g.groups)
            pack["blocks"].append(b)
        self._packs[s] = pack
        return pack

    def _descriptor(self, first=0, last=None):
        last = len(self.sizes) - 1 if last is None else last
        key = self._param_key()
        if key != self._desc_key:
            self._descs, self._packs, self._desc_key = {}, {}, key
        if (first, last) in self._descs:
            return self._descs[(first, last)]
        d = N.TdsDesc()
        d.n_stages = last - first
        d.groups = self.input_size
        d.ksize = self.kernel_size
        for s in range(first, last + 1):
            d.channels[s - first] = self.sizes[s]
        for s in range(first, last):
            i = s - first
            down, chain = self.blocks[s][0], self.blocks[s][1]
            pack = self._stage_pack(s)
            d.depths[i] = len(chain)
            d.down_w[i] = pack["down_w"].data_ptr()
            d.down_b[i] = down.bias.data_ptr()
            if pack["down_frag"] is not None:
                d.down_w_frag[i] = pack["down_frag"].data_ptr()
            for j, (blk, b) in enumerate(zip(chain, pack["blocks"])):
                g = blk.conv[0]
                bw = d.blocks[i][j]
                bw.conv_w, bw.conv_b = b["conv_w"].data_ptr(), g.bias.data_ptr()
                bw.fc0_w, bw.fc0_b = blk.fc[0].weight.data_ptr(), blk.fc[0].bias.data_ptr()
                bw.fc3_w, bw.fc3_b = blk.fc[3].weight.data_ptr(), blk.fc[3].bias.data_ptr()
                bw.resweight = b["rw"]
                if b["fc0_split"] is not None:
                    bw.fc0_w_split, bw.fc3_w_split = b["fc0_split"].data_ptr(), b["fc3_split"].data_ptr()
                if b["conv_frag"] is not None:
                    bw.conv_w_frag = b["conv_frag"].data_ptr()
        self._descs[(first, last)] = d
        return d

    def _needs_tiles(self, x, first, last):
        return first == 0 and last == len(self.sizes) - 1 and x.shape[0] == 1 and x.shape[1] > self.max_item_frames

    def forward_time_major(self, x, first=0, last=None):
        N.require_cuda(x, "TDS.forward")
        last = len(self.sizes) - 1 if last is None else last
        if first == last:
            return x
        if self._needs_tiles(x, first, last):
            return ops.tds_forward_tiled(self._descriptor(first, last), x, self.sizes[last], self.tile_frames)
        return ops.tds_forward(self._descriptor(first, last), x, self.sizes[last])

    def forward_then(self, x, tail, x_mean=None, split_ok=False):
        N.require_cuda(x, "TDS.forward")
        desc = self._descriptor(0, len(self.sizes) - 1)
        if x_mean is not None and (self._needs_tiles(x, 0, len(self.sizes) - 1) or not ops.tds_premean_ok(desc, x)):
            x, x_mean = ops.subtract_scalar_(x, x_mean), None
        if self._needs_tiles(x, 0, len(self.sizes) - 1):
            y = self.forward_time_major(x)
            return tail(y, False) if split_ok else tail(y)
        y, chk = ops.tds_forward(desc, x, self.sizes[-1], defer=True, x_mean=x_mean, out_split=split_ok)
        out = tail(y, chk.y_split) if split_ok else tail(y)
        if chk.flagged():
            y = chk.rerun_exact()
            out = tail(y, False) if split_ok else tail(y)
        return out

    def extract(self, x):
        y = self.forward_time_major(x.permute(0, 2, 1).contiguous(), 0, self.extract_block_id)
        return y.permute(0, 2, 1).contiguous()

    def aggregate(self, x):
        y = self.forward_time_major(x.permute(0, 2, 1).contiguous(), self.extract_block_id, len(self.sizes) - 1)
        return y.permute(0, 2, 1).contiguous()

    def forward(self, x):
        return self.forward_time_major(x.permute(0, 2, 1).contiguous()).permute(0, 2, 1).contiguous()


def padding_mask(audio_lens, t_out, device):
    lens = audio_lens.detach().cpu().to(torch.int64)
    scaled = lens // (lens.max() // int(t_out))
    mask = torch.zeros(lens.numel(), int(t_out), dtype=torch.bool)
    for i, l in enumerate(scaled.tolist()):
        mask[i, l:] = 1
    return mask.to(device)


def _check_encoder_mels(n_mels, who):
    if (10 * n_mels) % 4 != 0:
        raise N.NativeError("%s(n_mels=%d): the encoder's pointwise layers need C %% 4 == 0, and C = 10 * n_mels = %d is not "
                            "(n_mels must be even)" % (who, n_mels, 10 * n_mels))


class SDModel(_Resampled, nn.Module):

    def __init__(self, num_speakers=6008, n_mels=80, dropout=0.2, embed_size=128):
        super().__init__()
        self.num_speakers = num_speakers
        _check_encoder_mels(n_mels, "SDModel")
        tds_sizes = [n_mels, 10 * n_mels, 14 * n_mels, 18 * n_mels]
        tds_depths = [2, 3, 6]
        self.logmelspec = LogMelSpec(n_mels=n_mels)
        self.encoder = TDS(n_mels, tds_sizes, tds_depths, dropout=dropout)
        self.dropout = nn.Dropout(dropout)
        self.spk_embed_proj = Linear(tds_sizes[-1], embed_size)
        self.spk_logit_proj = Linear(embed_size, num_speakers)
        self.apply(weight_init())
        self.eval()

    def get_encoder_params(self):
        return list(self.encoder.parameters())

    def extract_features(self, x, specaug=True):
        return self.logmelspec(x)

    def encode_features(self, x: torch.Tensor, audio_lens: torch.LongTensor = None, sample_rate=None):
        rs = self._resampler(sample_rate)
        if rs is not None and audio_lens is not None:
            audio_lens = rs.num_samples(audio_lens)
        x = self.encoder.forward_time_major(x)
        mask = None if audio_lens is None else padding_mask(audio_lens, x.size(1), x.device)
        return {"encoder_out": x, "encoder_padding_mask": mask}

    def encode(self, x: torch.Tensor, audio_lens: torch.LongTensor = None, sample_rate=None):
        x, audio_lens = self._resample_batch(x, audio_lens, sample_rate)
        return self.encode_features(self.extract_features(x), audio_lens)

    def decode(self, encoder_out, past=None, causal_mask=True):
        _, logits, _ = ops.sd_head(encoder_out["encoder_out"], self.spk_embed_proj.weight, self.spk_embed_proj.bias,
                                   self.spk_logit_proj.weight, self.spk_logit_proj.bias,
                                   want_logits=True, want_ids=False)
        return logits

    def forward(self, x, audio_lens):
        encoder_out = self.encode(x, audio_lens)
        return self.decode(encoder_out), encoder_out

    @torch.no_grad()
    def speaker_ids(self, x_wav, want_logits=False, sample_rate=None):
        rs = self._resampler(sample_rate)
        if rs is not None:
            x_wav = rs(x_wav)
        mel, mean = self.logmelspec.forward_unsubtracted(x_wav)
        return self.speaker_ids_from_logmel(mel, mean, want_logits=want_logits)

    @torch.no_grad()
    def speaker_ids_from_logmel(self, mel, mean, want_logits=False):
        def head(enc_out, enc_split=False):
            return ops.sd_head(enc_out, self.spk_embed_proj.weight, self.spk_embed_proj.bias, self.spk_logit_proj.weight,
                               self.spk_logit_proj.bias, want_logits=want_logits, want_ids=True, x_split=enc_split,
                               w_embed_split=self._embed_split() if enc_split else None)
        feat, logits, ids = self.encoder.forward_then(mel, head, x_mean=mean, split_ok=self._embed_split() is not None)
        return (feat, ids, logits) if want_logits else (feat, ids)

    @torch.no_grad()
    def speaker_topk(self, x_wav, k=4, sample_rate=None):
        rs = self._resampler(sample_rate)
        if rs is not None:
            x_wav = rs(x_wav)
        mel, mean = self.logmelspec.forward_unsubtracted(x_wav)
        return self.speaker_topk_from_logmel(mel, mean, k=k)

    @torch.no_grad()
    def speaker_topk_from_logmel(self, mel, mean, k=4):
        def head(enc_out, enc_split=False):
            feat, _, _ = ops.sd_head(enc_out, self.spk_embed_proj.weight, self.spk_embed_proj.bias, self.spk_logit_proj.weight,
                                     self.spk_logit_proj.bias, want_logits=False, want_ids=False, x_split=enc_split,
                                     w_embed_split=self._embed_split() if enc_split else None)
            return (feat,) + ops.spk_topk(feat, self.spk_logit_proj.weight, self.spk_logit_proj.bias, k)
        return self.encoder.forward_then(mel, head, x_mean=mean, split_ok=self._embed_split() is not None)

    @torch.no_grad()
    def speaker_soft_embeds(self, x_wav, sample_rate=None):
        rs = self._resampler(sample_rate)
        if rs is not None:
            x_wav = rs(x_wav)
        mel, mean = self.logmelspec.forward_unsubtracted(x_wav)
        return self.speaker_soft_embeds_from_logmel(mel, mean)

    @torch.no_grad()
    def speaker_soft_embeds_from_logmel(self, mel, mean):
        def head(enc_out, enc_split=False):
            feat, _, _ = ops.sd_head(enc_out, self.spk_embed_proj.weight, self.spk_embed_proj.bias, self.spk_logit_proj.weight,
                                     self.spk_logit_proj.bias, want_logits=False, want_ids=False, x_split=enc_split,
                                     w_embed_split=self._embed_split() if enc_split else None)
            return (feat,) + ops.soft_embed(feat, self.spk_logit_proj.weight, self.spk_logit_proj.bias, None, want_lse=True)
        return self.encoder.forward_then(mel, head, x_mean=mean, split_ok=self._embed_split() is not None)

    def _embed_split(self):
        w = self.spk_embed_proj.weight
        key = (w.data_ptr(), w._version, w.device)
        if getattr(self, "_embed_split_key", None) != key:
            wd = w.detach()
            ok = w.is_cuda and w.shape[1] % 32 == 0 and bool(torch.isfinite(wd).all()) and float(wd.abs().max()) <= 65504.0
            self._embed_split_t = ops.split_f16x3(wd.contiguous()) if ok else None
            self._embed_split_key = key
        return self._embed_split_t

    @torch.no_grad()
    def speaker_ids_stream(self, host_clips, sample_rate=None):
        dev = self.spk_embed_proj.weight.device
        taken = (torch.float32, torch.float16) + ((torch.int16,) if self._resampler(sample_rate) is not None else ())
        copy_stream = torch.cuda.Stream(device=dev)
        compute = torch.cuda.current_stream(dev)
        if not hasattr(self, "_stream_bufs"):
            self._stream_bufs = [None, None]
        bufs, free_ev = self._stream_bufs, [None, None]

        def upload(clip, slot):
            if clip.dtype not in taken:
                raise N.NativeError("speaker_ids_stream: clips must be float32 or float16 waveforms (or int16 PCM together with "
                                    "sample_rate=), got %s" % clip.dtype)
            nbytes = clip.numel() * clip.element_size()
            if bufs[slot] is None or bufs[slot].numel() < nbytes:
                if free_ev[slot] is not None:
                    free_ev[slot].synchronize()
                bufs[slot] = torch.empty(nbytes + nbytes // 8, dtype=torch.uint8, device=dev)
                free_ev[slot] = None
            view = bufs[slot][:nbytes].view(clip.dtype).view(clip.shape)
            if free_ev[slot] is not None:
                copy_stream.wait_event(free_ev[slot])
            else:
                copy_stream.wait_stream(compute)
            with torch.cuda.stream(copy_stream):
                view.copy_(clip, non_blocking=True)
                done = torch.cuda.Event()
                done.record(copy_stream)
            return view, done, slot

        it = iter(host_clips)
        first = next(it, None)
        if first is None:
            return
        pending = upload(first, 0)
        i = 0
        while pending is not None:
            x, done, slot = pending
            nxt = next(it, None)
            pending = upload(nxt, (i + 1) & 1) if nxt is not None else None
            compute.wait_event(done)
            out = self.speaker_ids(x, sample_rate=sample_rate)
            ev = torch.cuda.Event()
            ev.record(compute)
            free_ev[slot] = ev
            i += 1
            yield out


class ModRZTXDecoderLayer(nn.Module):

    def __init__(self, d_model, nhead, dim_feedforward=2048, dropout=0.1, activation="relu"):
        super().__init__()
        if activation != "relu":
            raise N.NativeError("ModRZTXDecoderLayer: only the ReLU FFN is built (tal/asr/models.py:125)")
        self.self_attn = nn.MultiheadAttention(d_model, nhead, dropout=dropout)
        self.multihead_attn = nn.MultiheadAttention(d_model, nhead, dropout=dropout)
        self.linear1 = Linear(d_model, dim_feedforward)
        self.dropout = nn.Dropout(dropout)
        self.linear2 = Linear(dim_feedforward, d_model)
        self.dropout1 = nn.Dropout(dropout)
        self.dropout2 = nn.Dropout(dropout)
        self.dropout3 = nn.Dropout(dropout)
        self.resweight = nn.Parameter(torch.Tensor([0]))
        self.resweight_src = nn.Parameter(torch.Tensor([0]))
        self.nhead = nhead
        self.src_attn_weights = None
        _adopt(self)

    def forward(self, tgt, memory, tgt_mask=None, memory_mask=None, tgt_key_padding_mask=None,
                memory_key_padding_mask=None):
        from .decoder import decoder_layer_forward
        return decoder_layer_forward(self, tgt, memory, tgt_mask, memory_mask, tgt_key_padding_mask,
                                     memory_key_padding_mask)


ScoreResult = collections.namedtuple("ScoreResult", ["lm_nll", "spk_nll", "lm_top1", "spk_top1"])


class ASRModel(_Resampled, nn.Module):

    def __init__(self, model_type="2x", num_speakers=0, n_mels=80, vocab_size=10000, n_head=4, max_positions=512,
                 dropout=0.2, embed_size=64, spk_embed=128, use_speaker_head=False):
        super().__init__()
        self.embed_size = embed_size
        self.num_speakers = num_speakers
        self.max_positions = max_positions
        self.use_speaker_head = use_speaker_head
        self.model_type = model_type
        self.n_head = n_head
        _check_encoder_mels(n_mels, "ASRModel")
        tds_sizes = [n_mels, 10 * n_mels, 14 * n_mels, 18 * n_mels]
        tds_depths = [2, 3, 6]
        if model_type == "1x":
            d_hidden, n_layers = 256, 4
        elif model_type == "2x":
            d_hidden, n_layers = 512, 4
        else:
            raise Exception("Invalid model type")
        self.pos_dec_encoder = PositionalEncoding(d_hidden, max_len=max_positions, dropout=dropout)
        self.logmelspec = LogMelSpec(n_mels=n_mels)
        self.encoder = TDS(n_mels, tds_sizes, tds_depths, dropout=dropout)
        self.dropout = nn.Dropout(dropout)
        self.decoder_proj = Linear(tds_sizes[-1], d_hidden)
        num_tokens = vocab_size if use_speaker_head else vocab_size + num_speakers
        if self.embed_size:
            self.embedding = nn.Embedding(num_tokens, embed_size)
            self.embedding_proj = Linear(embed_size, d_hidden, bias=False)
            self.lm_head = Linear(embed_size, num_tokens, bias=False)
        else:
            self.embedding = nn.Embedding(num_tokens, d_hidden)
            self.lm_head = Linear(d_hidden, num_tokens, bias=False)
        self.lm_head.weight = self.embedding.weight
        self.decoder = _decoder_stack(d_hidden, n_head, dropout, n_layers)
        if self.use_speaker_head:
            self.spk_enc_proj = Linear(tds_sizes[-1], d_hidden)
            self.spk_decoder = _decoder_stack(d_hidden, n_head, dropout, n_layers // 2)
            self.speaker_head = nn.Sequential(Linear(d_hidden, spk_embed), Linear(spk_embed, num_speakers))
        self.apply(weight_init())
        self.eval()

    def get_encoder_params(self):
        return list(self.encoder.parameters())

    def extract_features(self, x, specaug=True):
        return self.logmelspec(x)

    def encode_features(self, x: torch.Tensor, audio_lens: torch.LongTensor = None, sample_rate=None):
        rs = self._resampler(sample_rate)
        if rs is not None and audio_lens is not None:
            audio_lens = rs.num_samples(audio_lens)

        def proj(e):
            spk = ops.linear(e, self.spk_enc_proj.weight, self.spk_enc_proj.bias) if self.use_speaker_head else None
            return spk, ops.linear(e, self.decoder_proj.weight, self.decoder_proj.bias)
        spk_h, x = self.encoder.forward_then(x, proj)
        mask = None if audio_lens is None else padding_mask(audio_lens, x.size(1), x.device)
        return {"speaker_out": spk_h, "encoder_out": x, "encoder_padding_mask": mask}

    def encode(self, x: torch.Tensor, audio_lens: torch.LongTensor = None, sample_rate=None):
        x, audio_lens = self._resample_batch(x, audio_lens, sample_rate)
        return self.encode_features(self.extract_features(x), audio_lens)

    def decode(self, y_prev, encoder_out, past=None, causal_mask=True):
        from .decoder import asr_decode
        return asr_decode(self, y_prev, encoder_out, causal_mask)

    def decode_spk(self, y_prev, encoder_out, causal_mask=True):
        from .decoder import asr_decode_spk
        return asr_decode_spk(self, y_prev, encoder_out, causal_mask)

    def score(self, y_prev, y_target, encoder_out, spk_target=None, want_top1=False):
        from .decoder import asr_score, asr_score_spk
        lm = asr_score(self, y_prev, y_target, encoder_out, want_top1=want_top1)
        lm_nll, lm_top1 = lm if want_top1 else (lm, None)
        spk_nll = spk_top1 = None
        if self.use_speaker_head and spk_target is not None:
            spk = asr_score_spk(self, y_prev, spk_target, encoder_out, want_top1=want_top1)
            spk_nll, spk_top1 = spk if want_top1 else (spk, None)
        return ScoreResult(lm_nll, spk_nll, lm_top1, spk_top1)

    def speaker_token_embeds(self, y_prev, y_target, encoder_out, first_speaker_token):
        from .decoder import asr_speaker_token_embeds
        return asr_speaker_token_embeds(self, y_prev, y_target, encoder_out, first_speaker_token)

    def forward(self, x, y_prev, audio_lens):
        encoder_out = self.encode(x, audio_lens)
        lm_out = self.decode(y_prev, encoder_out)
        spk_out = self.decode_spk(y_prev, encoder_out) if self.use_speaker_head else None
        return (lm_out, spk_out), encoder_out


class TransformerDecoder(nn.Module):

    def __init__(self, layers):
        super().__init__()
        self.layers = nn.ModuleList(layers)
        self.num_layers = len(layers)
        self.norm = None

    def forward(self, tgt, memory, tgt_mask=None, memory_mask=None, tgt_key_padding_mask=None,
                memory_key_padding_mask=None):
        out = tgt
        for layer in self.layers:
            out = layer(out, memory, tgt_mask=tgt_mask, memory_mask=memory_mask,
                        tgt_key_padding_mask=tgt_key_padding_mask,
                        memory_key_padding_mask=memory_key_padding_mask)
        return out


def _decoder_stack(d_model, n_head, dropout, n_layers):
    return TransformerDecoder([ModRZTXDecoderLayer(d_model=d_model, dim_feedforward=d_model * 4, nhead=n_head,
                                                   dropout=dropout, activation="relu") for _ in range(n_layers)])
```

tal_asrd_amd/ops.py:

```python
import ctypes as C

import torch

from . import _native as N


def _ws(nbytes, device):
    return torch.empty(max(int(nbytes), 16), dtype=torch.uint8, device=device)


def _f32c(t, what):
    N.require_cuda(t, what)
    if t.dtype != torch.float32:
        raise N.NativeError("%s: expected float32, got %s (only the waveform may be half precision, as the "
                            "reference's call sites hand it over; everything behind the front-end is fp32)" % (what, t.dtype))
    return t.contiguous()


NFFT_MIN, NFFT_MAX, NMELS_MAX = 32, 2048, 256


class LogmelGeneralPlan:

    def __init__(self, buf, n_fft, hop, n_mels):
        self.buf, self.n_fft, self.hop, self.n_mels = buf, n_fft, hop, n_mels

    @property
    def device(self):
        return self.buf.device


def logmel_shape_error(n_fft, hop, n_mels):
    if not NFFT_MIN <= n_fft <= NFFT_MAX:
        return "n_fft=%d outside %d..%d" % (n_fft, NFFT_MIN, NFFT_MAX)
    if not 1 <= hop <= n_fft:
        return "hop=%d outside 1..n_fft (%d)" % (hop, n_fft)
    if not 1 <= n_mels <= NMELS_MAX:
        return "n_mels=%d outside 1..%d" % (n_mels, NMELS_MAX)
    return None


def logmel_plan(window, fb, hop=160):
    lib = N.lib()
    window = _f32c(window, "logmel_plan(window)")
    fb = _f32c(fb, "logmel_plan(fb)")
    if window.dim() != 1 or fb.dim() != 2 or fb.shape[0] != window.shape[0] // 2 + 1:
        raise N.NativeError("logmel_plan: window/fb must be [n_fft] and [n_fft//2 + 1, n_mels], got %s %s"
                            % (tuple(window.shape), tuple(fb.shape)))
    n_fft, n_mels = int(window.shape[0]), int(fb.shape[1])
    if (n_fft, hop, n_mels) != (400, 160, 80) or N.get_option("logmel_general"):
        err = logmel_shape_error(n_fft, hop, n_mels)
        if err:
            raise N.NativeError("logmel_plan: " + err)
        buf = torch.empty(lib.tal_logmel_general_plan_bytes(n_fft, n_mels), dtype=torch.uint8, device=window.device)
        N.check(lib.tal_logmel_general_plan_init(N.ptr(window), n_fft, hop, N.ptr(fb), n_mels, N.ptr(buf), N.stream_handle()),
                "tal_logmel_general_plan_init")
        return LogmelGeneralPlan(buf, n_fft, hop, n_mels)
    plan = torch.empty(lib.tal_logmel_plan_bytes(), dtype=torch.uint8, device=window.device)
    N.check(lib.tal_logmel_plan_init(N.ptr(window), N.ptr(fb), N.ptr(plan), N.stream_handle()),
            "tal_logmel_plan_init")
    return plan


def _audio(t, what):
    N.require_cuda(t, what)
    if t.dtype not in (torch.float32, torch.float16):
        raise N.NativeError("%s: the waveform must be float32 or float16, got %s%s" % (what, t.dtype, (
            " (16-bit PCM goes through tal_asrd_amd.Resample(orig_freq, new_freq), or the sample_rate= argument of the models' "
            "entry points, which scale it by 2^-15 on the device)") if t.dtype == torch.int16 else ""))
    return t.contiguous()


def logmel(plan, audio, eps=1e-6, subtract_mean=True, return_stats=False):
    lib = N.lib()
    audio = _audio(audio, "logmel")
    if audio.dim() != 2:
        raise N.NativeError("logmel: audio must be [batch, samples]")
    B, L = audio.shape
    if isinstance(plan, LogmelGeneralPlan):
        T = lib.tal_logmel_frames(L - plan.n_fft % 2, plan.hop)
        out = torch.empty(B, T, plan.n_mels, dtype=torch.float32, device=audio.device)
        mean = torch.empty(1, dtype=torch.float32, device=audio.device)
        stats = torch.empty(2, dtype=torch.float64, device=audio.device)
        nws = lib.tal_logmel_general_workspace_bytes(plan.n_fft, plan.hop, B, L)
        ws = _ws(nws, audio.device)
        N.check(lib.tal_logmel_general_fwd(N.ptr(plan.buf), plan.n_fft, plan.hop, plan.n_mels, N.ptr(audio),
                                           1 if audio.dtype == torch.float16 else 0, B, L, eps, 1 if subtract_mean else 0,
                                           N.ptr(out), N.ptr(mean), N.ptr(stats), N.ptr(ws), nws, N.stream_handle()),
                "tal_logmel_general_fwd")
        return (out, mean, stats) if return_stats else out
    T = lib.tal_logmel_num_frames(L)
    out = torch.empty(B, T, 80, dtype=torch.float32, device=audio.device)
    mean = torch.empty(1, dtype=torch.float32, device=audio.device)
    stats = torch.empty(2, dtype=torch.float64, device=audio.device)
    nws = lib.tal_logmel_workspace_bytes(B, L)
    ws = _ws(nws, audio.device)
    fwd = lib.tal_logmel_f16_fwd if audio.dtype == torch.float16 else lib.tal_logmel_fwd
    N.check(fwd(N.ptr(plan), N.ptr(audio), B, L, eps, 1 if subtract_mean else 0, N.ptr(out),
                N.ptr(mean), N.ptr(stats), N.ptr(ws), nws, N.stream_handle()), "tal_logmel_fwd")
    return (out, mean, stats) if return_stats else out


def subtract_scalar_(x, mean):
    lib = N.lib()
    N.check(lib.tal_subtract_scalar(N.ptr(x), x.numel(), N.ptr(mean), N.stream_handle()), "tal_subtract_scalar")
    return x


RESAMPLE_WIDTH = 6
_RESAMPLE_DTYPES = {torch.float32: 0, torch.float16: 1, torch.int16: 2}


class ResamplePlan:

    def __init__(self, buf, orig, new, width):
        self.buf, self.orig, self.new, self.width = buf, orig, new, width

    @property
    def device(self):
        return self.buf.device


def _rate(v, what):
    if isinstance(v, bool) or int(v) != v:
        raise N.NativeError("%s: sample rates are integers (Hz), got %r" % (what, v))
    return int(v)


def resample_plan_bytes(orig, new, width=RESAMPLE_WIDTH):
    lib = N.lib()
    orig, new = _rate(orig, "resample_plan"), _rate(new, "resample_plan")
    if max(abs(orig), abs(new)) >= 2 ** 31:
        raise N.NativeError("resample_plan(%d -> %d): sample rates must be 1..1048576 Hz" % (orig, new))
    nbytes = lib.tal_resample_plan_bytes(orig, new, width)
    if nbytes == 0:
        N.check(lib.tal_resample_plan_build_host(orig, new, width, None, None, None), "resample_plan(%d -> %d)" % (orig, new))
        raise N.NativeError("resample_plan(%d -> %d): outside the plan limits" % (orig, new))
    return nbytes


def resample_plan(orig, new, device, width=RESAMPLE_WIDTH):
    lib = N.lib()
    nbytes = resample_plan_bytes(orig, new, width)
    device = torch.device(device)
    if device.type != "cuda":
        raise N.NativeError("resample_plan: the hot path only runs on the GPU (HIP kernels); got device %s and there is deliberately "
                            "no CPU fallback" % device)
    buf = torch.empty(nbytes, dtype=torch.uint8, device=device)
    with torch.cuda.device(device):
        N.check(lib.tal_resample_plan_init(N.ptr(buf), int(orig), int(new), width, N.stream_handle()), "tal_resample_plan_init")
    return ResamplePlan(buf, int(orig), int(new), width)


def resample_num_samples(n_in, orig, new):
    lib = N.lib()
    orig, new = _rate(orig, "resample_num_samples"), _rate(new, "resample_num_samples")
    if isinstance(n_in, torch.Tensor):
        flat = [lib.tal_resample_num_samples(int(v), orig, new) for v in n_in.detach().cpu().reshape(-1).tolist()]
        return torch.tensor(flat, dtype=torch.int64).reshape(n_in.shape)
    return lib.tal_resample_num_samples(int(n_in), orig, new)


def resample(plan, x, lengths=None):
    lib = N.lib()
    N.require_cuda(x, "resample")
    if x.dtype not in _RESAMPLE_DTYPES:
        raise N.NativeError("resample: the waveform must be float32, float16 or int16, got %s" % x.dtype)
    if x.dim() < 1:
        raise N.NativeError("resample: the waveform must be [..., samples]")
    if x.device != plan.device:
        raise N.NativeError("resample: the plan lives on %s, the waveform on %s" % (plan.device, x.device))
    L = x.shape[-1]
    lead = tuple(x.shape[:-1])
    n = lib.tal_resample_num_samples(L, plan.orig, plan.new)
    if not (x.dim() == 2 and x.stride(1) == 1 and x.stride(0) >= L) and not x.is_contiguous():
        x = x.contiguous()
    B = 1
    for d in lead:
        B *= d
    pitch = x.stride(0) if x.dim() == 2 and B > 1 else L
    y = torch.empty(lead + (n,), dtype=torch.float32, device=x.device)
    if lengths is not None:
        lengths = torch.as_tensor(lengths).to(device=x.device, dtype=torch.int64).contiguous()
        if lengths.numel() != B:
            raise N.NativeError("resample: %d lengths for %d rows" % (lengths.numel(), B))
    if B == 0 or n == 0:
        return y
    N.check(lib.tal_resample_fwd(N.ptr(plan.buf), plan.orig, plan.new, plan.width, N.ptr(x), _RESAMPLE_DTYPES[x.dtype], B, L, pitch,
                                 N.ptr(lengths), N.ptr(y), n, N.stream_handle()), "tal_resample_fwd")
    return y


def linear(x, weight, bias=None, mode=0, res=None, alpha=0.0, out=None):
    lib = N.lib()
    x = _f32c(x, "linear")
    w2 = weight.reshape(weight.shape[0], -1)
    w2 = _f32c(w2, "linear(weight)")
    K = x.shape[-1]
    Nout = w2.shape[0]
    if w2.shape[1] != K:
        raise N.NativeError("linear: x[..., %d] vs weight %s" % (K, tuple(weight.shape)))
    M = x.numel() // K
    y = out if out is not None else torch.empty(*x.shape[:-1], Nout, dtype=torch.float32, device=x.device)
    if res is not None:
        res = _f32c(res, "linear(res)")
    if bias is not None:
        bias = _f32c(bias, "linear(bias)")
    nws = lib.tal_linear_workspace_bytes(M, Nout, K)
    if nws:
        ws = _ws(nws, x.device)
        N.check(lib.tal_linear_ws_fwd(N.ptr(x), N.ptr(w2), N.ptr(bias), N.ptr(res), float(alpha), int(mode), M, Nout, K,
                                      N.ptr(y), N.ptr(ws), nws, N.stream_handle()), "tal_linear_ws_fwd")
    else:
        N.check(lib.tal_linear_fwd(N.ptr(x), N.ptr(w2), N.ptr(bias), N.ptr(res), float(alpha), int(mode), M, Nout, K,
                                   N.ptr(y), N.stream_handle()), "tal_linear_fwd")
    return y


def split_f16x3(x2d):
    lib = N.lib()
    x2d = _f32c(x2d, "split_f16x3")
    rows, K = x2d.shape
    out = torch.empty(rows * K * 4, dtype=torch.uint8, device=x2d.device)
    N.check(lib.tal_split_f16x3_fwd(N.ptr(x2d), N.ptr(out), rows, K, N.stream_handle()), "tal_split_f16x3_fwd")
    return out


def pack_gconv_weight(weight, groups):
    lib = N.lib()
    w = _f32c(weight, "pack_gconv_weight")
    c_out, cig, ks = w.shape
    packed = torch.empty(w.numel(), dtype=torch.float32, device=w.device)
    N.check(lib.tal_pack_gconv_weight(N.ptr(w), N.ptr(packed), c_out, cig, ks, groups, N.stream_handle()),
            "tal_pack_gconv_weight")
    return packed


def gconv_s2(x, w_packed, bias, c_out, groups, ksize=21):
    if ksize != 21:
        return gconv_s2_k(x, w_packed, bias, c_out, groups, ksize)
    lib = N.lib()
    x = _f32c(x, "gconv_s2")
    B, T, c_in = x.shape
    y = torch.empty(B, (T - 21) // 2 + 1, c_out, dtype=torch.float32, device=x.device)
    N.check(lib.tal_gconv_s2_fwd(N.ptr(x), N.ptr(w_packed), N.ptr(bias), B, T, c_in, c_out, groups, N.ptr(y),
                                 N.stream_handle()), "tal_gconv_s2_fwd")
    return y


def gconv_res(x, w_packed, bias, alpha, groups, ksize=21):
    if ksize != 21:
        return gconv_res_k(x, w_packed, bias, alpha, groups, ksize)
    lib = N.lib()
    x = _f32c(x, "gconv_res")
    B, T, c = x.shape
    y = torch.empty_like(x)
    N.check(lib.tal_gconv_res_fwd(N.ptr(x), N.ptr(w_packed), N.ptr(bias), float(alpha), B, T, c, groups, N.ptr(y),
                                  N.stream_handle()), "tal_gconv_res_fwd")
    return y


def gconv_s2_k(x, w_packed, bias, c_out, groups, ksize):
    lib = N.lib()
    x = _f32c(x, "gconv_s2_k")
    B, T, c_in = x.shape
    if T < ksize:
        raise N.NativeError("gconv_s2_k: %d frames are too few for kernel size %d" % (T, ksize))
    y = torch.empty(B, (T - ksize) // 2 + 1, c_out, dtype=torch.float32, device=x.device)
    N.check(lib.tal_gconv_s2_k_fwd(N.ptr(x), N.ptr(w_packed), N.ptr(bias), B, T, c_in, c_out, groups, int(ksize), N.ptr(y),
                                   N.stream_handle()), "tal_gconv_s2_k_fwd")
    return y


def gconv_res_k(x, w_packed, bias, alpha, groups, ksize):
    lib = N.lib()
    x = _f32c(x, "gconv_res_k")
    B, T, c = x.shape
    y = torch.empty_like(x)
    N.check(lib.tal_gconv_res_k_fwd(N.ptr(x), N.ptr(w_packed), N.ptr(bias), float(alpha), B, T, c, groups, int(ksize), N.ptr(y),
                                    N.stream_handle()), "tal_gconv_res_k_fwd")
    return y


def pack_gconv_f16x3_weight(weight, groups, stride=1):
    lib = N.lib()
    w = _f32c(weight, "pack_gconv_f16x3_weight")
    c_out, cig, ks = w.shape
    c_in = cig * groups
    nbytes = lib.tal_gconv_f16x3_weight_bytes(c_in, c_out, groups, stride) if ks == 21 else 0
    if nbytes == 0:
        return None
    frag = torch.empty(nbytes, dtype=torch.uint8, device=w.device)
    N.check(lib.tal_pack_gconv_f16x3_weight(N.ptr(w), N.ptr(frag), c_in, c_out, groups, stride, N.stream_handle()),
            "tal_pack_gconv_f16x3_weight")
    return frag


def gconv_s2_f16x3(x, w_frag, bias, c_out, groups):
    lib = N.lib()
    x = _f32c(x, "gconv_s2_f16x3")
    B, T, c_in = x.shape
    y = torch.empty(B, (T - 21) // 2 + 1, c_out, dtype=torch.float32, device=x.device)
    N.check(lib.tal_gconv_s2_f16x3_fwd(N.ptr(x), N.ptr(w_frag), N.ptr(bias), B, T, c_in, c_out, groups, N.ptr(y),
                                       N.stream_handle()), "tal_gconv_s2_f16x3_fwd")
    return y


def gconv_res_f16x3(x, w_frag, bias, alpha, groups, want_split=False):
    lib = N.lib()
    x = _f32c(x, "gconv_res_f16x3")
    B, T, c = x.shape
    y = torch.empty_like(x)
    ys = torch.empty(B * T * c * 4, dtype=torch.uint8, device=x.device) if want_split else None
    N.check(lib.tal_gconv_res_f16x3_fwd(N.ptr(x), N.ptr(w_frag), N.ptr(bias), float(alpha), B, T, c, groups, N.ptr(y),
                                        N.ptr(ys) if want_split else None, N.stream_handle()), "tal_gconv_res_f16x3_fwd")
    return (y, ys) if want_split else y


def gconv_res_split(x_split, shape, w_frag, bias, alpha, groups):
    lib = N.lib()
    B, T, c = shape
    ys = torch.empty(B * T * c * 4, dtype=torch.uint8, device=x_split.device)
    N.check(lib.tal_gconv_res_split_fwd(N.ptr(x_split), N.ptr(w_frag), N.ptr(bias), float(alpha), B, T, c, groups, N.ptr(ys),
                                        N.stream_handle()), "tal_gconv_res_split_fwd")
    return ys


def gconv_s2_split(x, shape, x_is_split, w_frag, bias, c_out, groups):
    lib = N.lib()
    B, T, c_in = shape
    t_out = (T - 21) // 2 + 1
    ys = torch.empty(B * t_out * c_out * 4, dtype=torch.uint8, device=x.device)
    N.check(lib.tal_gconv_s2_split_fwd(N.ptr(x), 1 if x_is_split else 0, N.ptr(w_frag), N.ptr(bias), B, T, c_in, c_out, groups,
                                       N.ptr(ys), N.stream_handle()), "tal_gconv_s2_split_fwd")
    return ys


range_fallbacks = 0


class RangeCheck:

    def __init__(self, desc, x, y, ws, nws, off, x_mean=None, y_split=False):
        self.desc, self.x, self.y, self.ws, self.nws, self.off, self.x_mean = desc, x, y, ws, nws, off, x_mean
        self.y_split = y_split

    def flagged(self):
        if self.desc.flags & N.TAL_TDS_EXACT_F32 and not self.y_split:
            return False
        flag, form = self.ws[self.off:self.off + 8].view(torch.int32).tolist()
        if bool(form) != bool(self.y_split):
            raise N.NativeError("tal_tds_fwd wrote its output in the %s form but its consumer was enqueued for the %s form "
                                "(a kernel-selection option changed between tal_tds_out_split and the call?)"
                                % ("split" if form else "fp32", "split" if self.y_split else "fp32"))
        return flag != 0 and not (self.desc.flags & N.TAL_TDS_EXACT_F32)

    def rerun_exact(self):
        global range_fallbacks
        range_fallbacks += 1
        lib = N.lib()
        B, T, _ = self.x.shape
        exact = N.TdsDesc.from_buffer_copy(self.desc)
        exact.flags |= N.TAL_TDS_EXACT_F32
        N.check(_tds_call(lib, exact, self.x, self.x_mean, B, T, self.y, self.ws, self.nws), "tal_tds_fwd (exact fp32 re-run)")
        self.y_split = False
        return self.y


def _tds_call(lib, desc, x, x_mean, B, T, y, ws, nws):
    if x_mean is None:
        return lib.tal_tds_fwd(C.byref(desc), N.ptr(x), B, T, N.ptr(y), N.ptr(ws), nws, N.stream_handle())
    return lib.tal_tds_premean_fwd(C.byref(desc), N.ptr(x), N.ptr(x_mean), B, T, N.ptr(y), N.ptr(ws), nws, N.stream_handle())


def tds_premean_ok(desc, x):
    return bool(N.lib().tal_tds_premean_ok(C.byref(desc), N.ptr(x)))


def tds_forward(desc, x, c_out, check_range=True, defer=False, x_mean=None, out_split=False):
    lib = N.lib()
    x = _f32c(x, "tds_forward")
    B, T, _ = x.shape
    t_out = lib.tal_tds_out_len(C.byref(desc), T)
    if t_out <= 0:
        raise N.NativeError("tds_forward: %d frames are too few for the stride-2 k=%d stages" % (T, desc.ksize or 21))
    y = torch.empty(B, t_out, c_out, dtype=torch.float32, device=x.device)
    nws = lib.tal_tds_workspace_bytes(C.byref(desc), B, T)
    ws = _ws(nws, x.device)
    y_split = False
    if out_split:
        if not defer:
            raise N.NativeError("tds_forward: out_split needs defer=True (the caller must look at RangeCheck.y_split)")
        asked = N.TdsDesc.from_buffer_copy(desc)
        asked.flags |= N.TAL_TDS_OUT_SPLIT
        if lib.tal_tds_out_split(C.byref(asked), B, T):
            desc, y_split = asked, True
    N.check(_tds_call(lib, desc, x, x_mean, B, T, y, ws, nws), "tal_tds_fwd")
    chk = RangeCheck(desc, x, y, ws, nws, lib.tal_tds_status_offset(C.byref(desc), B, T), x_mean, y_split)
    if defer:
        return y, chk
    if check_range and chk.flagged():
        chk.rerun_exact()
    return y


def tds_forward_tiled(desc, x, c_out, out_tile, check_range=True):
    lib = N.lib()
    x = _f32c(x, "tds_forward_tiled")
    if x.dim() != 3 or x.shape[0] != 1:
        raise N.NativeError("tds_forward_tiled: x must be [1, T, C]")
    T = x.shape[1]
    t_out = lib.tal_tds_out_len(C.byref(desc), T)
    if t_out <= 0:
        raise N.NativeError("tds_forward_tiled: %d frames are too few for the stride-2 k=%d stages" % (T, desc.ksize or 21))
    y = torch.empty(1, t_out, c_out, dtype=torch.float32, device=x.device)
    nws = lib.tal_tds_tiled_workspace_bytes(C.byref(desc), T, int(out_tile))
    ws = _ws(nws, x.device)

    def run(d):
        N.check(lib.tal_tds_tiled_fwd(C.byref(d), N.ptr(x), T, N.ptr(y), int(out_tile), N.ptr(ws), nws, N.stream_handle()),
                "tal_tds_tiled_fwd")
    run(desc)
    if check_range and not (desc.flags & N.TAL_TDS_EXACT_F32):
        off = lib.tal_tds_tiled_status_offset(C.byref(desc), T, int(out_tile))
        if int(ws[off:off + 4].view(torch.int32)[0]) != 0:
            global range_fallbacks
            range_fallbacks += 1
            exact = N.TdsDesc.from_buffer_copy(desc)
            exact.flags |= N.TAL_TDS_EXACT_F32
            run(exact)
    return y


def sd_head(x, w_embed, b_embed, w_logit, b_logit, want_logits=True, want_ids=True, x_split=False, w_embed_split=None):
    lib = N.lib()
    x = _f32c(x, "sd_head")
    Cc = x.shape[-1]
    M = x.numel() // Cc
    E, S = w_embed.shape[0], w_logit.shape[0]
    dev = x.device
    feat = torch.empty(*x.shape[:-1], E, dtype=torch.float32, device=dev)
    logits = torch.empty(*x.shape[:-1], S, dtype=torch.float32, device=dev) if want_logits else None
    ids = torch.empty(x.shape[:-1], dtype=torch.int32, device=dev) if want_ids else None
    nws = lib.tal_sd_head_workspace_bytes(M, S) if not want_logits else 0
    ws = _ws(nws, dev)
    if x_split:
        if w_embed_split is None:
            raise N.NativeError("sd_head: x_split needs w_embed_split (ops.split_f16x3 of the embedding weight)")
        if not nws:
            nws = lib.tal_sd_head_workspace_bytes(M, S)
            ws = _ws(nws, dev)
        N.check(lib.tal_sd_head_split_fwd(N.ptr(x), M, Cc, N.ptr(w_embed_split), N.ptr(b_embed), E,
                                          N.ptr(_f32c(w_logit, "w")), N.ptr(b_logit), S, N.ptr(feat), N.ptr(logits),
                                          N.ptr(ids), N.ptr(ws), nws, N.stream_handle()), "tal_sd_head_split_fwd")
        return feat, logits, ids
    N.check(lib.tal_sd_head_fwd(N.ptr(x), M, Cc, N.ptr(_f32c(w_embed, "w")), N.ptr(b_embed), E,
                                N.ptr(_f32c(w_logit, "w")), N.ptr(b_logit), S, N.ptr(feat), N.ptr(logits),
                                N.ptr(ids), N.ptr(ws), nws, N.stream_handle()), "tal_sd_head_fwd")
    return feat, logits, ids


def argmax_rows(x):
    lib = N.lib()
    x = _f32c(x, "argmax_rows")
    Nn = x.shape[-1]
    M = x.numel() // Nn
    ids = torch.empty(x.shape[:-1], dtype=torch.int32, device=x.device)
    N.check(lib.tal_argmax_rows(N.ptr(x), M, Nn, N.ptr(ids), N.stream_handle()), "tal_argmax_rows")
    return ids


def _check_k(k, n, what):
    if isinstance(k, bool) or int(k) != k or not 1 <= int(k) <= min(N.TAL_TOPK_MAX, n):
        raise N.NativeError("%s: k=%r outside 1..min(%d, %d columns)" % (what, k, N.TAL_TOPK_MAX, n))
    return int(k)


def spk_topk(feat, w_logit, b_logit, k):
    lib = N.lib()
    feat = _f32c(feat, "spk_topk")
    w = _f32c(w_logit, "spk_topk(w_logit)")
    b = None if b_logit is None else _f32c(b_logit, "spk_topk(b_logit)")
    E, S = feat.shape[-1], w.shape[0]
    if w.dim() != 2 or w.shape[1] != E or (b is not None and b.numel() != S):
        raise N.NativeError("spk_topk: feat [..., %d] vs w_logit %s, b_logit %s"
                            % (E, tuple(w.shape), None if b is None else tuple(b.shape)))
    k = _check_k(k, S, "spk_topk")
    M = feat.numel() // E
    lead, dev = tuple(feat.shape[:-1]), feat.device
    ids = torch.empty(lead + (k,), dtype=torch.int32, device=dev)
    logp = torch.empty(lead + (k,), dtype=torch.float32, device=dev)
    lse = torch.empty(lead, dtype=torch.float32, device=dev)
    nws = lib.tal_spk_topk_workspace_bytes(M, S, E, k)
    ws = _ws(nws, dev)
    N.check(lib.tal_spk_topk_fwd(N.ptr(feat), M, E, N.ptr(w), N.ptr(b), S, k, N.ptr(ids), N.ptr(logp), N.ptr(lse), N.ptr(ws), nws,
                                 N.stream_handle()), "tal_spk_topk_fwd")
    return ids, logp, lse


def topk_lse_rows(x, k):
    lib = N.lib()
    x = _f32c(x, "topk_lse_rows")
    Nn = x.shape[-1]
    k = _check_k(k, Nn, "topk_lse_rows")
    M = x.numel() // Nn
    lead = tuple(x.shape[:-1])
    ids = torch.empty(lead + (k,), dtype=torch.int32, device=x.device)
    logp = torch.empty(lead + (k,), dtype=torch.float32, device=x.device)
    lse = torch.empty(lead, dtype=torch.float32, device=x.device)
    N.check(lib.tal_topk_lse_rows(N.ptr(x), M, Nn, k, N.ptr(ids), N.ptr(logp), N.ptr(lse), N.stream_handle()), "tal_topk_lse_rows")
    return ids, logp, lse


def _targets(target, lead, what):
    N.require_cuda(target, what)
    if target.dtype.is_floating_point or target.dtype == torch.bool or tuple(target.shape) != tuple(lead):
        raise N.NativeError("%s: targets must be integers of shape %s, got %s %s" % (what, tuple(lead), target.dtype, tuple(target.shape)))
    return target.to(torch.int64).contiguous()


def xent_rows(feat, w, bias, target, want_lse=False, want_top1=False):
    lib = N.lib()
    feat = _f32c(feat, "xent_rows")
    w = _f32c(w, "xent_rows(w)")
    b = None if bias is None else _f32c(bias, "xent_rows(bias)")
    E, S = feat.shape[-1], w.shape[0]
    if w.dim() != 2 or w.shape[1] != E or (b is not None and b.numel() != S):
        raise N.NativeError("xent_rows: feat [..., %d] vs w %s, bias %s" % (E, tuple(w.shape), None if b is None else tuple(b.shape)))
    lead, dev = tuple(feat.shape[:-1]), feat.device
    t = _targets(target, lead, "xent_rows(target)")
    M = feat.numel() // E
    nll = torch.empty(lead, dtype=torch.float32, device=dev)
    lse = torch.empty(lead, dtype=torch.float32, device=dev) if want_lse else None
    top1 = torch.empty(lead, dtype=torch.int32, device=dev) if want_top1 else None
    nws = lib.tal_xent_rows_workspace_bytes(M, S, E)
    ws = _ws(nws, dev)
    N.check(lib.tal_xent_rows_fwd(N.ptr(feat), M, E, E, N.ptr(w), N.ptr(b), S, N.ptr(t), N.ptr(nll), N.ptr(lse), N.ptr(top1), N.ptr(ws),
                                  nws, N.stream_handle()), "tal_xent_rows_fwd")
    return (nll,) + ((lse,) if want_lse else ()) + ((top1,) if want_top1 else ()) if want_lse or want_top1 else nll


def xent_lse_rows(x, target, want_lse=False, want_top1=False):
    lib = N.lib()
    x = _f32c(x, "xent_lse_rows")
    Nn = x.shape[-1]
    lead = tuple(x.shape[:-1])
    t = _targets(target, lead, "xent_lse_rows(target)")
    M = x.numel() // Nn
    nll = torch.empty(lead, dtype=torch.float32, device=x.device)
    lse = torch.empty(lead, dtype=torch.float32, device=x.device) if want_lse else None
    top1 = torch.empty(lead, dtype=torch.int32, device=x.device) if want_top1 else None
    N.check(lib.tal_xent_lse_rows(N.ptr(x), M, Nn, N.ptr(t), N.ptr(nll), N.ptr(lse), N.ptr(top1), N.stream_handle()), "tal_xent_lse_rows")
    return (nll,) + ((lse,) if want_lse else ()) + ((top1,) if want_top1 else ()) if want_lse or want_top1 else nll


def soft_embed(feat, w, bias, values=None, want_lse=False):
    lib = N.lib()
    feat = _f32c(feat, "soft_embed")
    w = _f32c(w, "soft_embed(w)")
    b = None if bias is None else _f32c(bias, "soft_embed(bias)")
    v = None if values is None else _f32c(values, "soft_embed(values)")
    E, S = feat.shape[-1], w.shape[0]
    if w.dim() != 2 or w.shape[1] != E or (b is not None and b.numel() != S) or (v is not None and (v.dim() != 2 or v.shape[0] != S)):
        raise N.NativeError("soft_embed: feat [..., %d] vs w %s, bias %s, values %s"
                            % (E, tuple(w.shape), None if b is None else tuple(b.shape), None if v is None else tuple(v.shape)))
    D = E if v is None else v.shape[1]
    lead, dev = tuple(feat.shape[:-1]), feat.device
    M = feat.numel() // E
    out = torch.empty(lead + (D,), dtype=torch.float32, device=dev)
    lse = torch.empty(lead, dtype=torch.float32, device=dev) if want_lse else None
    nws = lib.tal_soft_embed_workspace_bytes(M, S, E, D)
    ws = _ws(nws, dev)
    N.check(lib.tal_soft_embed_fwd(N.ptr(feat), M, E, E, N.ptr(w), N.ptr(b), S, N.ptr(v), D, N.ptr(out), N.ptr(lse), N.ptr(ws), nws,
                                   N.stream_handle()), "tal_soft_embed_fwd")
    return (out, lse) if want_lse else out


def soft_embed_rows(x, values, want_lse=False):
    lib = N.lib()
    x = _f32c(x, "soft_embed_rows")
    v = _f32c(values, "soft_embed_rows(values)")
    Nn = x.shape[-1]
    if v.dim() != 2 or v.shape[0] != Nn:
        raise N.NativeError("soft_embed_rows: x [..., %d] vs values %s" % (Nn, tuple(v.shape)))
    D = v.shape[1]
    lead = tuple(x.shape[:-1])
    M = x.numel() // Nn
    out = torch.empty(lead + (D,), dtype=torch.float32, device=x.device)
    lse = torch.empty(lead, dtype=torch.float32, device=x.device) if want_lse else None
    nws = lib.tal_soft_embed_rows_workspace_bytes(M, Nn, D)
    ws = _ws(nws, x.device)
    N.check(lib.tal_soft_embed_rows(N.ptr(x), M, Nn, N.ptr(v), D, N.ptr(out), N.ptr(lse), N.ptr(ws), nws, N.stream_handle()),
            "tal_soft_embed_rows")
    return (out, lse) if want_lse else out


def add_positional(x, pe):
    lib = N.lib()
    x = _f32c(x, "add_positional")
    B, U, D = x.shape
    out = torch.empty_like(x)
    N.check(lib.tal_add_positional_fwd(N.ptr(x), B, U, D, N.ptr(_f32c(pe, "pe")), pe.shape[0], N.ptr(out),
                                       N.stream_handle()), "tal_add_positional_fwd")
    return out


EDIT_TAGS = ("equal", "replace", "insert", "delete")
EDIT_TAG_NONE = 255
EDIT_BUDGET_FRACTION = 0.25
EDIT_MAX_PAIRS = 65535


def edit_align_tile():
    r, c = C.c_int(), C.c_int()
    N.lib().tal_edit_align_tile(C.byref(r), C.byref(c))
    return r.value, c.value


class EditAlignment:

    def __init__(self, stats, path, path_offsets, counts, launches, workspace_bytes):
        self.stats, self.path, self.path_offsets, self.counts = stats, path, path_offsets, counts
        self.launches, self.workspace_bytes = launches, workspace_bytes

    @property
    def dist(self):
        return self.stats[:, 0]

    def tags(self):
        if self.path is None:
            raise N.NativeError("edit_align: the call was made with want_path=False")
        steps = self.stats[:, 1].cpu().numpy()
        flat = self.path.cpu().numpy()
        return [flat[o:o + int(k)] for o, k in zip(self.path_offsets[:-1], steps)]


def _edit_is_batch(x):
    import numpy as np
    if isinstance(x, (torch.Tensor, np.ndarray)):
        return x.ndim > 1
    return len(x) > 0 and isinstance(x[0], (list, tuple, torch.Tensor, np.ndarray))


def _edit_cat(seqs, dev, what, upper=None):
    import numpy as np
    lens = [int(s.numel()) if isinstance(s, torch.Tensor) else len(s) for s in seqs]
    off = np.zeros(len(seqs) + 1, dtype=np.int64)
    np.cumsum(lens, out=off[1:])
    if seqs and all(isinstance(s, torch.Tensor) and s.is_cuda for s in seqs):
        for s in seqs:
            if s.dtype.is_floating_point or s.dtype == torch.bool or s.dim() != 1:
                raise N.NativeError("%s: expected 1-D integer tensors, got %s %s" % (what, s.dtype, tuple(s.shape)))
        return torch.cat([s.to(device=dev, dtype=torch.int32) for s in seqs]).contiguous(), off
    host = np.zeros(int(off[-1]), dtype=np.int64)
    for s, o, k in zip(seqs, off[:-1], lens):
        if k:
            v = np.asarray(s.cpu() if isinstance(s, torch.Tensor) else s)
            if v.ndim != 1 or v.dtype.kind not in "iu":
                raise N.NativeError("%s: expected 1-D integer sequences, got %s %s" % (what, v.dtype, v.shape))
            host[o:o + k] = v
    if host.size and (host.min() < (0 if upper is not None else -2 ** 31) or host.max() >= (upper if upper is not None else 2 ** 31)):
        raise N.NativeError("%s: values outside [%d, %d)" % (what, 0 if upper is not None else -2 ** 31, upper if upper is not None else 2 ** 31))
    return torch.from_numpy(host.astype(np.int32)).to(dev), off


def edit_align(a, b, a_labels=None, b_labels=None, n_labels=None, want_path=True, budget_bytes=None, device=None):
    import numpy as np
    lib = N.lib()
    dev = torch.device(device) if device is not None else next((x.device for x in (a, b) if isinstance(x, torch.Tensor)), torch.device("cuda:0"))
    if not _edit_is_batch(a) and not _edit_is_batch(b):
        a, b = [a], [b]
        a_labels = None if a_labels is None else [a_labels]
        b_labels = None if b_labels is None else [b_labels]
    a, b = list(a), list(b)
    if len(a) != len(b):
        raise N.NativeError("edit_align: %d reference sequences vs %d hypothesis sequences" % (len(a), len(b)))
    if dev.type != "cuda":
        raise N.NativeError("edit_align: the hot path only runs on the GPU (HIP kernels); got device %s and there is deliberately no "
                            "CPU fallback (wder.levenshtein / wder.align_opcodes are the host routines)" % dev)
    if (a_labels is None) != (b_labels is None):
        raise N.NativeError("edit_align: labels are needed for both sides or for neither")
    labels = a_labels is not None
    if labels and not want_path:
        raise N.NativeError("edit_align: counts need the path (want_path=True)")
    P = len(a)
    Ka = Kb = 0
    if labels:
        if isinstance(n_labels, (tuple, list)):
            Ka, Kb = int(n_labels[0]), int(n_labels[1])
        elif n_labels is not None:
            Ka = Kb = int(n_labels)
    ids_a, a_off = _edit_cat(a, dev, "edit_align(a)")
    ids_b, b_off = _edit_cat(b, dev, "edit_align(b)")
    lab_a = lab_b = None
    if labels:
        a_labels, b_labels = list(a_labels), list(b_labels)
        if n_labels is None:
            if any(isinstance(s, torch.Tensor) and s.is_cuda for s in a_labels + b_labels):
                raise N.NativeError("edit_align: n_labels is needed with device labels")
            Ka = 1 + max([int(np.max(s)) for s in a_labels if len(s)] or [0])
            Kb = 1 + max([int(np.max(s)) for s in b_labels if len(s)] or [0])
        if Ka <= 0 or Kb <= 0 or Ka * Kb > 1 << 24:
            raise N.NativeError("edit_align: n_labels = (%d, %d): both must be positive and their product at most 2^24" % (Ka, Kb))
        lab_a, la_off = _edit_cat(a_labels, dev, "edit_align(a_labels)", Ka)
        lab_b, lb_off = _edit_cat(b_labels, dev, "edit_align(b_labels)", Kb)
        if not np.array_equal(la_off, a_off) or not np.array_equal(lb_off, b_off):
            raise N.NativeError("edit_align: every label sequence must be as long as its id sequence")
    m, n = np.diff(a_off), np.diff(b_off)
    path_off = np.zeros(P + 1, dtype=np.int64)
    np.cumsum(m + n, out=path_off[1:])
    need = []
    for p in range(P):
        oa, ob = np.array([0, m[p]], dtype=np.int64), np.array([0, n[p]], dtype=np.int64)
        need.append(int(lib.tal_edit_align_workspace_bytes(1, oa.ctypes.data, ob.ctypes.data, int(want_path))))
    if budget_bytes is None:
        free, _ = torch.cuda.mem_get_info(dev)
        budget_bytes = EDIT_BUDGET_FRACTION * (free + torch.cuda.memory_reserved(dev) - torch.cuda.memory_allocated(dev))
    for p in range(P):
        if need[p] > budget_bytes:
            raise N.NativeError("edit_align: pair %d (m=%d, n=%d) needs a workspace of %d bytes, the budget is %d bytes; there is no host "
                                "fallback (backend=\"host\" of wder.py is the host route)" % (p, m[p], n[p], need[p], int(budget_bytes)))
    calls, p0, acc = [], 0, 0
    for p in range(P):
        if p > p0 and (acc + need[p] > budget_bytes or p - p0 == EDIT_MAX_PAIRS):
            calls.append((p0, p))
            p0, acc = p, 0
        acc += need[p]
    if P:
        calls.append((p0, P))
    stats = torch.empty((P, 4), dtype=torch.int64, device=dev)
    path = torch.empty(max(int(path_off[-1]), 1), dtype=torch.uint8, device=dev)[:int(path_off[-1])] if want_path else None
    counts = torch.empty((P, Ka, Kb), dtype=torch.int64, device=dev) if labels else None
    launches, ws_max = 0, 0
    with torch.cuda.device(dev):
        for p0, p1 in calls:
            k = p1 - p0
            oa, ob = np.ascontiguousarray(a_off[p0:p1 + 1]), np.ascontiguousarray(b_off[p0:p1 + 1])
            desc = np.zeros((k, 8), dtype=np.int64)
            nws, npath, nl = C.c_size_t(), C.c_int64(), C.c_int()
            N.check(lib.tal_edit_align_plan(k, oa.ctypes.data, ob.ctypes.data, int(want_path), desc.ctypes.data, C.byref(nws), C.byref(npath),
                                            C.byref(nl)), "tal_edit_align_plan")
            desc_dev = torch.from_numpy(desc).to(dev)
            ws = _ws(nws.value, dev)
            N.check(lib.tal_edit_align_fwd(desc.ctypes.data, N.ptr(desc_dev), k, N.ptr(ids_a), N.ptr(ids_b), N.ptr(lab_a), N.ptr(lab_b), Ka, Kb,
                                           C.c_void_p(stats.data_ptr() + 32 * p0),
                                           C.c_void_p(path.data_ptr() + int(path_off[p0])) if want_path else None,
                                           C.c_void_p(counts.data_ptr() + 8 * Ka * Kb * p0) if labels else None,
                                           N.ptr(ws), nws.value, N.stream_handle()), "tal_edit_align_fwd")
            launches += nl.value
            ws_max = max(ws_max, nws.value)
    return EditAlignment(stats, path, path_off, counts, launches, ws_max)
```

Baseline: 22.02 million frames/s.

## Fold last TDS block fc3 into speaker embedding projection

Adds a pre-head output form in which the final TDS block stops after fc0 and exposes its residual input and hidden activation. The SD head then computes the embedding as x1·Wf plus h·(rw·Wf·W3) with a folded bias. This replaces the large square fc3 GEMM with a narrow one. The folded weights are precomputed in float64 and cached, with finiteness and f16 range checks. The change risks slightly different rounding, and the fp32 fallback path is kept.

```diff
diff --git a/include/tal_asrd.h b/include/tal_asrd.h
--- a/include/tal_asrd.h
+++ b/include/tal_asrd.h
@@ -120,11 +120,13 @@
 } tal_tds_desc;
 #define TAL_TDS_EXACT_F32 1
 #define TAL_TDS_OUT_SPLIT 2
+#define TAL_TDS_OUT_PREHEAD 4
 
 int64_t tal_tds_out_len(const tal_tds_desc* d, int64_t T);
 size_t tal_tds_workspace_bytes(const tal_tds_desc* d, int B, int64_t T);
 size_t tal_tds_status_offset(const tal_tds_desc* d, int B, int64_t T);
 int tal_tds_out_split(const tal_tds_desc* d, int B, int64_t T);
+int tal_tds_out_prehead(const tal_tds_desc* d, int B, int64_t T, size_t* x1_offset, size_t* h_offset);
 int tal_tds_fwd(const tal_tds_desc* d, const float* x, int B, int64_t T, float* y,
                 void* workspace, size_t workspace_bytes, void* stream);
 int tal_tds_premean_ok(const tal_tds_desc* d, const float* x);
@@ -144,6 +146,9 @@
 int tal_sd_head_split_fwd(const void* x_split, int64_t M, int C, const void* w_embed_split, const float* b_embed, int E,
                           const float* w_logit, const float* b_logit, int S, float* feat, float* logits,
                           int32_t* ids, void* workspace, size_t workspace_bytes, void* stream);
+int tal_sd_head_prehead_fwd(const void* x1_split, const void* h_split, int64_t M, int C, const void* w_embed_split,
+                            const void* w_fold_split, const float* b_fold, int E, const float* w_logit, const float* b_logit, int S,
+                            float* feat, float* logits, int32_t* ids, void* workspace, size_t workspace_bytes, void* stream);
 int tal_argmax_rows(const float* x, int64_t M, int N, int32_t* ids, void* stream);
 
 #define TAL_TOPK_MAX 16
diff --git a/tal_asrd_amd/_native.py b/tal_asrd_amd/_native.py
--- a/tal_asrd_amd/_native.py
+++ b/tal_asrd_amd/_native.py
@@ -8,6 +8,7 @@
 TAL_MAX_DEPTH = 8
 TAL_TDS_EXACT_F32 = 1
 TAL_TDS_OUT_SPLIT = 2
+TAL_TDS_OUT_PREHEAD = 4
 TAL_GCONV_MAX_K = 63
 TAL_GROUP_MAX = 16
 TAL_TOPK_MAX = 16
@@ -115,6 +116,7 @@
     "tal_tds_status_offset": (_sz, [C.POINTER(TdsDesc), _i, _i64]),
     "tal_tds_fwd": (_i, [C.POINTER(TdsDesc), _p, _i, _i64, _p, _p, _sz, _p]),
     "tal_tds_out_split": (_i, [C.POINTER(TdsDesc), _i, _i64]),
+    "tal_tds_out_prehead": (_i, [C.POINTER(TdsDesc), _i, _i64, C.POINTER(C.c_size_t), C.POINTER(C.c_size_t)]),
     "tal_tds_premean_ok": (_i, [C.POINTER(TdsDesc), _p]),
     "tal_tds_premean_fwd": (_i, [C.POINTER(TdsDesc), _p, _p, _i, _i64, _p, _p, _sz, _p]),
     "tal_tds_halo": (_i, [C.POINTER(TdsDesc), C.POINTER(C.c_int64), C.POINTER(C.c_int64), C.POINTER(C.c_int64)]),
@@ -124,6 +126,7 @@
     "tal_sd_head_workspace_bytes": (_sz, [_i64, _i]),
     "tal_sd_head_fwd": (_i, [_p, _i64, _i, _p, _p, _i, _p, _p, _i, _p, _p, _p, _p, _sz, _p]),
     "tal_sd_head_split_fwd": (_i, [_p, _i64, _i, _p, _p, _i, _p, _p, _i, _p, _p, _p, _p, _sz, _p]),
+    "tal_sd_head_prehead_fwd": (_i, [_p, _p, _i64, _i, _p, _p, _p, _i, _p, _p, _i, _p, _p, _p, _p, _sz, _p]),
     "tal_argmax_rows": (_i, [_p, _i64, _i, _p, _p]),
     "tal_spk_topk_workspace_bytes": (_sz, [_i64, _i, _i, _i]),
     "tal_spk_topk_fwd": (_i, [_p, _i64, _i, _p, _p, _i, _i, _p, _p, _p, _p, _sz, _p]),
diff --git a/tal_asrd_amd/csrc/api.hip b/tal_asrd_amd/csrc/api.hip
--- a/tal_asrd_amd/csrc/api.hip
+++ b/tal_asrd_amd/csrc/api.hip
@@ -17,8 +17,8 @@
 
 static const char* const g_opt_names[OPT_COUNT] = {
     "tds_exact_f32", "tds_fp32_activations", "gconv_fuse_split", "gconv_c1_generic", "head_no_astationary", "gemm_global_loads",
-    "gemm_no_splitk4", "gemm_no_glds", "gemm_no_splitk_tail", "gemm_no_w64", "logmel_no_fold", "decode_no_small", "decode_small_rows", "gemm_no_row_split", "gemm_no_n96", "gemm_s64_below", "gconv_short_below", "gconv_no_shift18", "gconv_grid_xyz", "gemm_w64_stagger", "gemm_s64_order", "decode_wide_gemm", "gemm_s64_rows", "decode_persist", "decode_persist_wgs", "logmel_mfma", "gru_unfused", "decode_no_fold", "gconv_c1_fuse", "decode_fold_rows", "gconv_long_tt", "logmel_general", "gconv_general", "head_topk_form", "head_topk_grid", "xent_form", "xent_grid", "soft_embed_form", "soft_embed_grid"};
-static std::atomic<int> g_opt[OPT_COUNT] = {{0}, {0}, {0}, {0}, {0}, {0}, {0}, {0}, {0}, {0}, {0}, {0}, {256}, {0}, {0}, {2}, {4}, {0}, {0}, {0}, {0}, {0}, {0}, {0}, {32}, {0}, {0}, {0}, {0}, {64}, {0}, {0}, {0}, {0}, {0}, {0}, {0}, {0}, {0}};
+    "gemm_no_splitk4", "gemm_no_glds", "gemm_no_splitk_tail", "gemm_no_w64", "logmel_no_fold", "decode_no_small", "decode_small_rows", "gemm_no_row_split", "gemm_no_n96", "gemm_s64_below", "gconv_short_below", "gconv_no_shift18", "gconv_grid_xyz", "gemm_w64_stagger", "gemm_s64_order", "decode_wide_gemm", "gemm_s64_rows", "decode_persist", "decode_persist_wgs", "logmel_mfma", "gru_unfused", "decode_no_fold", "gconv_c1_fuse", "decode_fold_rows", "gconv_long_tt", "logmel_general", "gconv_general", "head_topk_form", "head_topk_grid", "xent_form", "xent_grid", "soft_embed_form", "soft_embed_grid", "sd_head_nofold", "sd_head_fold_rows"};
+static std::atomic<int> g_opt[OPT_COUNT] = {{0}, {0}, {0}, {0}, {0}, {0}, {0}, {0}, {0}, {0}, {0}, {0}, {256}, {0}, {0}, {2}, {4}, {0}, {0}, {0}, {0}, {0}, {0}, {0}, {32}, {0}, {0}, {0}, {0}, {64}, {0}, {0}, {0}, {0}, {0}, {0}, {0}, {0}, {0}, {0}, {16384}};
 int opt(Option o) { return g_opt[o].load(std::memory_order_relaxed); }
 
 int device_cus() {
@@ -216,6 +216,7 @@
     TAL_CHECK_ARG(i != OPT_XENT_GRID || value >= 0, "tal_set_option: xent_grid must be >= 0");
     TAL_CHECK_ARG(i != OPT_SOFT_EMBED_FORM || (value >= 0 && value <= 2), "tal_set_option: soft_embed_form is 0 (auto), 1 (generic) or 2 (fused)");
     TAL_CHECK_ARG(i != OPT_SOFT_EMBED_GRID || value >= 0, "tal_set_option: soft_embed_grid must be >= 0");
+    TAL_CHECK_ARG(i != OPT_SD_HEAD_FOLD_ROWS || value >= 0, "tal_set_option: sd_head_fold_rows must be >= 0");
     g_opt[i].store(value, std::memory_order_relaxed);
     return TAL_OK;
 }
@@ -407,12 +408,12 @@
 }
 
 static int tds_launch_dense(const tal_tds_block_w& bw, bool f16x3, bool allsplit, const float* xin, const float* x1, float* h, float* outp, bool out_split,
-                            int64_t M, int c, float* skws, hipStream_t s, int* range_flag) {
+                            int64_t M, int c, float* skws, hipStream_t s, int* range_flag, bool no_fc3 = false) {
     const size_t skb = gemm_splitk_ws_bytes();
     int rc;
     if (f16x3) {
         rc = launch_linear_f16x3(xin, bw.fc0_w_split, bw.fc0_b, nullptr, 0.f, 1, M, c, c, h, 1, skws, skb, s, range_flag);
-        if (rc) return rc;
+        if (rc || no_fc3) return rc;
         return launch_linear_f16x3(h, bw.fc3_w_split, bw.fc3_b, x1, bw.resweight, 2, M, c, c, outp, out_split ? 1 : 0, skws, skb, s,
                                    allsplit ? range_flag : nullptr, allsplit ? 1 : 0);
     }
@@ -421,8 +422,14 @@
     return launch_linear_ws(h, bw.fc3_w, bw.fc3_b, x1, bw.resweight, 2, M, c, c, outp, skws, skb, s);
 }
 
+enum { TDS_FORM_F32 = 0, TDS_FORM_SPLIT = 1, TDS_FORM_PREHEAD = 2 };
+struct TdsOut {
+    int form;
+    size_t x1_off, h_off;
+};
+
 static int tds_walk(const tal_tds_desc* d, const float* x, const float* x_mean, int B, int64_t T, float* y, void* workspace, hipStream_t s,
-                    bool launch, bool* y_split) {
+                    bool launch, TdsOut* out) {
     const size_t nf = tds_buf_floats(d, B, T);
     float* buf[4];
     for (int q = 0; q < 4; ++q) buf[q] = reinterpret_cast<float*>(workspace) + q * nf;
@@ -434,6 +441,7 @@
     const bool general = tds_general(d);
     const float* cur = x;
     bool cur_split = false;
+    bool prehead = false;
     int ia = -1;
     int64_t Tc = T;
     bool s2_mfma = tds_s2_mfma_ok(d, B, 0, T, ks, general, force_f32), blocks_split = tds_blocks_split_ok(d, B, 0, T, ks, general, fp32_only);
@@ -462,6 +470,12 @@
             const bool last_block = j == d->depths[i] - 1;
             float* outp = (last_stage && last_block) ? y : buf[ia];
             const bool out_split = allsplit && (!last_block || next_split || (last_stage && (d->flags & TAL_TDS_OUT_SPLIT) != 0));
+            prehead = allsplit && last_stage && last_block && (d->flags & TAL_TDS_OUT_PREHEAD) != 0 && !opt(OPT_SD_HEAD_NOFOLD) &&
+                      M > (int64_t)opt(OPT_SD_HEAD_FOLD_ROWS);
+            if (prehead) {
+                out->x1_off = (size_t)((ia + 1) % 4) * nf * sizeof(float);
+                out->h_off = (size_t)((ia + 2) % 4) * nf * sizeof(float);
+            }
             if (launch) {
                 TAL_CHECK_ARG(bw.conv_w && bw.conv_b && bw.fc0_w && bw.fc0_b && bw.fc3_w && bw.fc3_b, "tal_tds_fwd: null weight in block %d.%d", i, j);
                 float* x1 = buf[(ia + 1) % 4];
@@ -473,7 +487,7 @@
                         rc = launch_gconv_c1_res_f16x3(cur, d->down_w[i], d->down_b[i], x_mean, bw.conv_w_frag, bw.conv_b, bw.resweight, B, Tc, d->groups, x1, s, range_flag);
                     else
                         rc = launch_gconv_res_f16x3(a, bw.conv_w_frag, bw.conv_b, bw.resweight, B, To, c, d->groups, nullptr, x1, s, range_flag, true);
-                    if (!rc) rc = tds_launch_dense(bw, true, true, x1, x1, h, outp, out_split, M, c, skws, s, range_flag);
+                    if (!rc) rc = tds_launch_dense(bw, true, true, x1, x1, h, outp, out_split, M, c, skws, s, range_flag, prehead);
                 } else {
                     const bool f16x3 = !force_f32 && bw.fc0_w_split && bw.fc3_w_split && M > 128 && c % 160 == 0;
                     const bool conv_mfma = !force_f32 && !general && M > 64 && bw.conv_w_frag && gconv_has_mfma(c, c, d->groups, 1) && gconv_f16x3_fits(To, c);
@@ -498,7 +512,7 @@
         s2_mfma = next_s2_mfma;
         blocks_split = next_blocks_split;
     }
-    *y_split = cur_split;
+    out->form = prehead ? TDS_FORM_PREHEAD : cur_split ? TDS_FORM_SPLIT : TDS_FORM_F32;
     return TAL_OK;
 }
 
@@ -513,23 +527,34 @@
         return TAL_ENOMEM;
     }
     hipStream_t s = (hipStream_t)stream;
-    bool y_split_out = false;
-    if (d->flags & TAL_TDS_OUT_SPLIT) tds_walk(d, x, x_mean, B, T, y, workspace, s, false, &y_split_out);
+    TdsOut out = {};
+    if (d->flags & (TAL_TDS_OUT_SPLIT | TAL_TDS_OUT_PREHEAD)) tds_walk(d, x, x_mean, B, T, y, workspace, s, false, &out);
     int* status = reinterpret_cast<int*>(reinterpret_cast<char*>(workspace) + tal_tds_status_offset(d, B, T));
-    clear_status_kernel<<<1, 16, 0, s>>>(status, y_split_out ? 1 : 0);
+    clear_status_kernel<<<1, 16, 0, s>>>(status, out.form);
     if (hipGetLastError() != hipSuccess) {
         set_error("tal_tds_fwd: cannot clear the status word");
         return TAL_EHIP;
     }
-    return tds_walk(d, x, x_mean, B, T, y, workspace, s, true, &y_split_out);
+    return tds_walk(d, x, x_mean, B, T, y, workspace, s, true, &out);
 }
 
 extern "C" int tal_tds_out_split(const tal_tds_desc* d, int B, int64_t T) {
     if (check_desc(d) || B <= 0 || tal_tds_out_len(d, T) <= 0 || !(d->flags & TAL_TDS_OUT_SPLIT)) return 0;
     float* const aligned = reinterpret_cast<float*>(static_cast<uintptr_t>(16));
-    bool y_split = false;
-    tds_walk(d, aligned, nullptr, B, T, aligned, aligned, nullptr, false, &y_split);
-    return y_split ? 1 : 0;
+    TdsOut out = {};
+    tds_walk(d, aligned, nullptr, B, T, aligned, aligned, nullptr, false, &out);
+    return out.form == TDS_FORM_SPLIT ? 1 : 0;
+}
+
+extern "C" int tal_tds_out_prehead(const tal_tds_desc* d, int B, int64_t T, size_t* x1_offset, size_t* h_offset) {
+    if (check_desc(d) || B <= 0 || tal_tds_out_len(d, T) <= 0 || !(d->flags & TAL_TDS_OUT_PREHEAD)) return 0;
+    float* const aligned = reinterpret_cast<float*>(static_cast<uintptr_t>(16));
+    TdsOut out = {};
+    tds_walk(d, aligned, nullptr, B, T, aligned, aligned, nullptr, false, &out);
+    if (out.form != TDS_FORM_PREHEAD) return 0;
+    if (x1_offset) *x1_offset = out.x1_off;
+    if (h_offset) *h_offset = out.h_off;
+    return 1;
 }
 
 extern "C" int tal_tds_fwd(const tal_tds_desc* d, const float* x, int B, int64_t T, float* y, void* workspace,
@@ -623,7 +648,7 @@
                                  size_t workspace_bytes, void* stream) {
     TAL_CHECK_ARG(x && y && workspace && d, "tal_tds_tiled_fwd: null pointer");
     tal_tds_desc fp32_out = *d;
-    fp32_out.flags &= ~(uint32_t)TAL_TDS_OUT_SPLIT;
+    fp32_out.flags &= ~(uint32_t)(TAL_TDS_OUT_SPLIT | TAL_TDS_OUT_PREHEAD);
     d = &fp32_out;
     size_t so, tb;
     int64_t longest;
@@ -724,6 +749,22 @@
     const bool ws_ok = workspace && workspace_bytes >= tal_sd_head_workspace_bytes(M, S);
     int rc = launch_linear_f16x3(x_split, w_embed_split, b_embed, nullptr, 0.f, 0, M, E, C, feat, 0, ws_ok ? reinterpret_cast<float*>(workspace) : nullptr,
                                  ws_ok ? workspace_bytes : 0, s);
+    if (rc) return rc;
+    return sd_head_after_feat(M, E, w_logit, b_logit, S, feat, logits, ids, workspace, workspace_bytes, s);
+}
+
+extern "C" int tal_sd_head_prehead_fwd(const void* x1_split, const void* h_split, int64_t M, int C, const void* w_embed_split,
+                                       const void* w_fold_split, const float* b_fold, int E, const float* w_logit, const float* b_logit, int S,
+                                       float* feat, float* logits, int32_t* ids, void* workspace, size_t workspace_bytes, void* stream) {
+    TAL_CHECK_ARG(x1_split && h_split && w_embed_split && w_fold_split && w_logit && feat, "tal_sd_head_prehead_fwd: null pointer");
+    TAL_CHECK_ARG(M > 128 && C > 0 && C % 32 == 0 && E > 0 && S > 0, "tal_sd_head_prehead_fwd: needs M > 128 rows and C %% 32 == 0 (M=%lld, C=%d)", (long long)M, C);
+    hipStream_t s = (hipStream_t)stream;
+    const bool ws_ok = workspace && workspace_bytes >= tal_sd_head_workspace_bytes(M, S);
+    float* skws = ws_ok ? reinterpret_cast<float*>(workspace) : nullptr;
+    const size_t skb = ws_ok ? workspace_bytes : 0;
+    int rc = launch_linear_f16x3(x1_split, w_embed_split, b_fold, nullptr, 0.f, 0, M, E, C, feat, 0, skws, skb, s);
+    if (rc) return rc;
+    rc = launch_linear_f16x3(h_split, w_fold_split, nullptr, feat, 1.f, 2, M, E, C, feat, 0, skws, skb, s);
     if (rc) return rc;
     return sd_head_after_feat(M, E, w_logit, b_logit, S, feat, logits, ids, workspace, workspace_bytes, s);
 }
diff --git a/tal_asrd_amd/csrc/common.h b/tal_asrd_amd/csrc/common.h
--- a/tal_asrd_amd/csrc/common.h
+++ b/tal_asrd_amd/csrc/common.h
@@ -125,6 +125,8 @@
     OPT_XENT_GRID,
     OPT_SOFT_EMBED_FORM,
     OPT_SOFT_EMBED_GRID,
+    OPT_SD_HEAD_NOFOLD,
+    OPT_SD_HEAD_FOLD_ROWS,
     OPT_COUNT
 };
 int opt(Option o);
diff --git a/tal_asrd_amd/models.py b/tal_asrd_amd/models.py
--- a/tal_asrd_amd/models.py
+++ b/tal_asrd_amd/models.py
@@ -348,7 +348,7 @@
             return ops.tds_forward_tiled(self._descriptor(first, last), x, self.sizes[last], self.tile_frames)
         return ops.tds_forward(self._descriptor(first, last), x, self.sizes[last])
 
-    def forward_then(self, x, tail, x_mean=None, split_ok=False):
+    def forward_then(self, x, tail, x_mean=None, split_ok=False, pre_tail=None):
         N.require_cuda(x, "TDS.forward")
         desc = self._descriptor(0, len(self.sizes) - 1)
         if x_mean is not None and (self._needs_tiles(x, 0, len(self.sizes) - 1) or not ops.tds_premean_ok(desc, x)):
@@ -356,8 +356,12 @@
         if self._needs_tiles(x, 0, len(self.sizes) - 1):
             y = self.forward_time_major(x)
             return tail(y, False) if split_ok else tail(y)
-        y, chk = ops.tds_forward(desc, x, self.sizes[-1], defer=True, x_mean=x_mean, out_split=split_ok)
-        out = tail(y, chk.y_split) if split_ok else tail(y)
+        y, chk = ops.tds_forward(desc, x, self.sizes[-1], defer=True, x_mean=x_mean, out_split=split_ok,
+                                 prehead=split_ok and pre_tail is not None)
+        if chk.prehead is not None:
+            out = pre_tail(*chk.prehead)
+        else:
+            out = tail(y, chk.y_split) if split_ok else tail(y)
         if chk.flagged():
             y = chk.rerun_exact()
             out = tail(y, False) if split_ok else tail(y)
@@ -388,6 +392,11 @@
     if (10 * n_mels) % 4 != 0:
         raise N.NativeError("%s(n_mels=%d): the encoder's pointwise layers need C %% 4 == 0, and C = 10 * n_mels = %d is not "
                             "(n_mels must be even)" % (who, n_mels, 10 * n_mels))
+
+
+def fold_head_weights(wf, bf, w3, b3, rw):
+    rw = rw.reshape(())
+    return rw * (wf @ w3), bf + rw * (wf @ b3)
 
 
 class SDModel(_Resampled, nn.Module):
@@ -444,12 +453,21 @@
 
     @torch.no_grad()
     def speaker_ids_from_logmel(self, mel, mean, want_logits=False):
+        feat, logits, ids = self._encode_then_head(mel, mean, want_logits, True, lambda out: out)
+        return (feat, ids, logits) if want_logits else (feat, ids)
+
+    def _encode_then_head(self, mel, mean, want_logits, want_ids, after):
+        wl, bl = self.spk_logit_proj.weight, self.spk_logit_proj.bias
+        split = self._embed_split()
+        fold = self._head_fold()
+
         def head(enc_out, enc_split=False):
-            return ops.sd_head(enc_out, self.spk_embed_proj.weight, self.spk_embed_proj.bias, self.spk_logit_proj.weight,
-                               self.spk_logit_proj.bias, want_logits=want_logits, want_ids=True, x_split=enc_split,
-                               w_embed_split=self._embed_split() if enc_split else None)
-        feat, logits, ids = self.encoder.forward_then(mel, head, x_mean=mean, split_ok=self._embed_split() is not None)
-        return (feat, ids, logits) if want_logits else (feat, ids)
+            return after(ops.sd_head(enc_out, self.spk_embed_proj.weight, self.spk_embed_proj.bias, wl, bl, want_logits=want_logits,
+                                     want_ids=want_ids, x_split=enc_split, w_embed_split=split if enc_split else None))
+
+        def head_pre(x1, h):
+            return after(ops.sd_head_prehead(x1, h, split, fold[0], fold[1], wl, bl, want_logits=want_logits, want_ids=want_ids))
+        return self.encoder.forward_then(mel, head, x_mean=mean, split_ok=split is not None, pre_tail=head_pre if fold is not None else None)
 
     @torch.no_grad()
     def speaker_topk(self, x_wav, k=4, sample_rate=None):
@@ -461,12 +479,8 @@
 
     @torch.no_grad()
     def speaker_topk_from_logmel(self, mel, mean, k=4):
-        def head(enc_out, enc_split=False):
-            feat, _, _ = ops.sd_head(enc_out, self.spk_embed_proj.weight, self.spk_embed_proj.bias, self.spk_logit_proj.weight,
-                                     self.spk_logit_proj.bias, want_logits=False, want_ids=False, x_split=enc_split,
-                                     w_embed_split=self._embed_split() if enc_split else None)
-            return (feat,) + ops.spk_topk(feat, self.spk_logit_proj.weight, self.spk_logit_proj.bias, k)
-        return self.encoder.forward_then(mel, head, x_mean=mean, split_ok=self._embed_split() is not None)
+        return self._encode_then_head(mel, mean, False, False, lambda out: (out[0],) + ops.spk_topk(
+            out[0], self.spk_logit_proj.weight, self.spk_logit_proj.bias, k))
 
     @torch.no_grad()
     def speaker_soft_embeds(self, x_wav, sample_rate=None):
@@ -478,12 +492,8 @@
 
     @torch.no_grad()
     def speaker_soft_embeds_from_logmel(self, mel, mean):
-        def head(enc_out, enc_split=False):
-            feat, _, _ = ops.sd_head(enc_out, self.spk_embed_proj.weight, self.spk_embed_proj.bias, self.spk_logit_proj.weight,
-                                     self.spk_logit_proj.bias, want_logits=False, want_ids=False, x_split=enc_split,
-                                     w_embed_split=self._embed_split() if enc_split else None)
-            return (feat,) + ops.soft_embed(feat, self.spk_logit_proj.weight, self.spk_logit_proj.bias, None, want_lse=True)
-        return self.encoder.forward_then(mel, head, x_mean=mean, split_ok=self._embed_split() is not None)
+        return self._encode_then_head(mel, mean, False, False, lambda out: (out[0],) + ops.soft_embed(
+            out[0], self.spk_logit_proj.weight, self.spk_logit_proj.bias, None, want_lse=True))
 
     def _embed_split(self):
         w = self.spk_embed_proj.weight
@@ -494,6 +504,33 @@
             self._embed_split_t = ops.split_f16x3(wd.contiguous()) if ok else None
             self._embed_split_key = key
         return self._embed_split_t
+
+    def _head_fold_terms(self):
+        chain = self.encoder.blocks[-1][1]
+        if len(chain) == 0:
+            return None
+        blk, proj = chain[-1], self.spk_embed_proj
+        src = (proj.weight, proj.bias, blk.fc[3].weight, blk.fc[3].bias, blk.resweight)
+        key = tuple((t.data_ptr(), t._version, t.device) for t in src)
+        if getattr(self, "_head_fold_key", None) != key:
+            wf, bf, w3, b3, rw = (t.detach().to(torch.float64) for t in src)
+            wc, b = fold_head_weights(wf, bf, w3.reshape(w3.shape[0], -1), b3, rw)
+            wc, b = wc.to(torch.float32).contiguous(), b.to(torch.float32).contiguous()
+            ok = bool(torch.isfinite(wc).all()) and float(wc.abs().max()) <= 65504.0 and bool(torch.isfinite(b).all())
+            self._head_fold_t = (wc, b) if ok else None
+            self._head_fold_split_t = None
+            self._head_fold_key = key
+        return self._head_fold_t
+
+    def _head_fold(self):
+        if self._embed_split() is None:
+            return None
+        terms = self._head_fold_terms()
+        if terms is None:
+            return None
+        if self._head_fold_split_t is None:
+            self._head_fold_split_t = ops.split_f16x3(terms[0])
+        return self._head_fold_split_t, terms[1]
 
     @torch.no_grad()
     def speaker_ids_stream(self, host_clips, sample_rate=None):
diff --git a/tal_asrd_amd/ops.py b/tal_asrd_amd/ops.py
--- a/tal_asrd_amd/ops.py
+++ b/tal_asrd_amd/ops.py
@@ -341,18 +341,21 @@
 
 class RangeCheck:
 
-    def __init__(self, desc, x, y, ws, nws, off, x_mean=None, y_split=False):
+    def __init__(self, desc, x, y, ws, nws, off, x_mean=None, y_split=False, prehead=None):
         self.desc, self.x, self.y, self.ws, self.nws, self.off, self.x_mean = desc, x, y, ws, nws, off, x_mean
         self.y_split = y_split
+        self.prehead = prehead
 
     def flagged(self):
-        if self.desc.flags & N.TAL_TDS_EXACT_F32 and not self.y_split:
+        want = 2 if self.prehead is not None else 1 if self.y_split else 0
+        if self.desc.flags & N.TAL_TDS_EXACT_F32 and not want:
             return False
         flag, form = self.ws[self.off:self.off + 8].view(torch.int32).tolist()
-        if bool(form) != bool(self.y_split):
+        if form != want:
+            names = ("fp32", "split", "pre-head (x1, h)")
             raise N.NativeError("tal_tds_fwd wrote its output in the %s form but its consumer was enqueued for the %s form "
-                                "(a kernel-selection option changed between tal_tds_out_split and the call?)"
-                                % ("split" if form else "fp32", "split" if self.y_split else "fp32"))
+                                "(a kernel-selection option changed between tal_tds_out_split / tal_tds_out_prehead and the call?)"
+                                % (names[form] if 0 <= form < 3 else form, names[want]))
         return flag != 0 and not (self.desc.flags & N.TAL_TDS_EXACT_F32)
 
     def rerun_exact(self):
@@ -363,7 +366,7 @@
         exact = N.TdsDesc.from_buffer_copy(self.desc)
         exact.flags |= N.TAL_TDS_EXACT_F32
         N.check(_tds_call(lib, exact, self.x, self.x_mean, B, T, self.y, self.ws, self.nws), "tal_tds_fwd (exact fp32 re-run)")
-        self.y_split = False
+        self.y_split, self.prehead = False, None
         return self.y
 
 
@@ -377,7 +380,7 @@
     return bool(N.lib().tal_tds_premean_ok(C.byref(desc), N.ptr(x)))
 
 
-def tds_forward(desc, x, c_out, check_range=True, defer=False, x_mean=None, out_split=False):
+def tds_forward(desc, x, c_out, check_range=True, defer=False, x_mean=None, out_split=False, prehead=False):
     lib = N.lib()
     x = _f32c(x, "tds_forward")
     B, T, _ = x.shape
@@ -387,16 +390,23 @@
     y = torch.empty(B, t_out, c_out, dtype=torch.float32, device=x.device)
     nws = lib.tal_tds_workspace_bytes(C.byref(desc), B, T)
     ws = _ws(nws, x.device)
-    y_split = False
-    if out_split:
-        if not defer:
-            raise N.NativeError("tds_forward: out_split needs defer=True (the caller must look at RangeCheck.y_split)")
+    y_split, pre = False, None
+    if (out_split or prehead) and not defer:
+        raise N.NativeError("tds_forward: out_split / prehead need defer=True (the caller must look at RangeCheck.y_split / .prehead)")
+    if prehead:
+        asked = N.TdsDesc.from_buffer_copy(desc)
+        asked.flags |= N.TAL_TDS_OUT_PREHEAD
+        x1_off, h_off = C.c_size_t(), C.c_size_t()
+        if lib.tal_tds_out_prehead(C.byref(asked), B, T, C.byref(x1_off), C.byref(h_off)):
+            nb = B * t_out * c_out * 4
+            desc, pre = asked, tuple(ws[o.value:o.value + nb].view(torch.float32).view(B, t_out, c_out) for o in (x1_off, h_off))
+    if out_split and pre is None:
         asked = N.TdsDesc.from_buffer_copy(desc)
         asked.flags |= N.TAL_TDS_OUT_SPLIT
         if lib.tal_tds_out_split(C.byref(asked), B, T):
             desc, y_split = asked, True
     N.check(_tds_call(lib, desc, x, x_mean, B, T, y, ws, nws), "tal_tds_fwd")
-    chk = RangeCheck(desc, x, y, ws, nws, lib.tal_tds_status_offset(C.byref(desc), B, T), x_mean, y_split)
+    chk = RangeCheck(desc, x, y, ws, nws, lib.tal_tds_status_offset(C.byref(desc), B, T), x_mean, y_split, pre)
     if defer:
         return y, chk
     if check_range and chk.flagged():
@@ -457,6 +467,24 @@
     N.check(lib.tal_sd_head_fwd(N.ptr(x), M, Cc, N.ptr(_f32c(w_embed, "w")), N.ptr(b_embed), E,
                                 N.ptr(_f32c(w_logit, "w")), N.ptr(b_logit), S, N.ptr(feat), N.ptr(logits),
                                 N.ptr(ids), N.ptr(ws), nws, N.stream_handle()), "tal_sd_head_fwd")
+    return feat, logits, ids
+
+
+def sd_head_prehead(x1, h, w_embed_split, w_fold_split, b_fold, w_logit, b_logit, want_logits=True, want_ids=True):
+    lib = N.lib()
+    x1, h = _f32c(x1, "sd_head_prehead"), _f32c(h, "sd_head_prehead")
+    Cc = x1.shape[-1]
+    M = x1.numel() // Cc
+    E, S = b_fold.numel(), w_logit.shape[0]
+    dev = x1.device
+    feat = torch.empty(*x1.shape[:-1], E, dtype=torch.float32, device=dev)
+    logits = torch.empty(*x1.shape[:-1], S, dtype=torch.float32, device=dev) if want_logits else None
+    ids = torch.empty(x1.shape[:-1], dtype=torch.int32, device=dev) if want_ids else None
+    nws = lib.tal_sd_head_workspace_bytes(M, S)
+    ws = _ws(nws, dev)
+    N.check(lib.tal_sd_head_prehead_fwd(N.ptr(x1), N.ptr(h), M, Cc, N.ptr(w_embed_split), N.ptr(w_fold_split), N.ptr(b_fold), E,
+                                        N.ptr(_f32c(w_logit, "w")), N.ptr(b_logit), S, N.ptr(feat), N.ptr(logits), N.ptr(ids),
+                                        N.ptr(ws), nws, N.stream_handle()), "tal_sd_head_prehead_fwd")
     return feat, logits, ids
 
 
```

New measurement: 21.82 million frames/s. No clear change (-0.9%).
